# knights-lab/BURST

Hardware: AMD Instinct MI355X
Metric: aligned reads/sec (node), 100-bp synthetic reads @0.98 id vs RefSeq stand-in .edx/.acx (DB15), -m BEST; 1 GPU (higher is better)
Workload: dtype u32 bit-vectors (u8 edit distances)

## Files before the change

### burst_amd/capi.py

```python
import ctypes as C
import os

import numpy as np

_HERE = os.path.dirname(os.path.abspath(__file__))
LIB_PATH = os.path.join(os.environ.get("BURST_AMD_LIBDIR") or _HERE, "libburst_hip.so")

BHIP_OK, BHIP_E_ARG, BHIP_E_DEVICE, BHIP_E_CAPACITY, BHIP_E_QUERYLEN, BHIP_E_INTERNAL, BHIP_E_RESCORE = 0, -1, -2, -3, -4, -5, -6
BHIP_Q_PREFILTER, BHIP_Q_EXHAUSTIVE = 0, 1
BHIP_MAX_QLEN = 4095

HIT_DTYPE = np.dtype([("q", "<u4"), ("refIx", "<u4"), ("finalPos", "<u4"), ("score", "<f4"),
                      ("ed", "u1"), ("gapR", "u1"), ("gapQ", "u1"), ("rc", "u1")])
assert HIT_DTYPE.itemsize == 20


class BhipStats(C.Structure):
    _fields_ = [("n_queries", C.c_uint64), ("n_pairs", C.c_uint64), ("n_columns", C.c_uint64),
                ("n_raw_hits", C.c_uint64), ("n_hits", C.c_uint64), ("acx_entries_read", C.c_uint64),
                ("bytes_algorithmic", C.c_uint64), ("n_windows", C.c_uint64), ("n_window_columns", C.c_uint64),
                ("n_lane_tasks", C.c_uint64), ("n_task_columns", C.c_uint64), ("n_seed_words", C.c_uint64),
                ("ms_h2d", C.c_float), ("ms_prefilter", C.c_float), ("ms_peq", C.c_float), ("ms_myers", C.c_float),
                ("ms_rescore", C.c_float), ("ms_d2h", C.c_float), ("ms_total", C.c_float),
                ("ms_myers_prefix", C.c_float), ("ms_myers_window", C.c_float), ("ms_prefilter_hash", C.c_float), ("ms_seed", C.c_float),
                ("ms_stage_copy", C.c_float), ("ms_stage_route", C.c_float),
                ("myers_launches", C.c_uint32), ("prefix_words", C.c_uint32), ("prefilter_launches", C.c_uint32), ("prefilter_algo", C.c_uint32)]

    def as_dict(self):
        return {n: getattr(self, n) for n, _ in self._fields_}


class BhipQuerySpan(C.Structure):
    _fields_ = [("codes", C.c_void_p), ("codes4", C.c_void_p), ("off", C.c_void_p), ("emac", C.c_void_p), ("rc", C.c_void_p), ("flags", C.c_void_p),
                ("n", C.c_uint32), ("q_base", C.c_uint32), ("codes2", C.c_void_p), ("len", C.c_void_p)]


EXPORTS = ["bhip_init", "bhip_stage_queries", "bhip_align_staged", "bhip_align_batch", "bhip_align_pairs", "bhip_prefilter", "bhip_set_option", "bhip_get_stats",
           "bhip_device_info", "bhip_destroy", "bhip_last_error", "bhip_abi_version", "bhip_set_ref_order", "bhip_copy_hits_device", "bhip_sync_hits",
           "bhip_comm_create", "bhip_comm_unique_id", "bhip_comm_create_rank", "bhip_comm_allreduce_min", "bhip_comm_fetch_gathered", "bhip_comm_gather_hits", "bhip_comm_stage_device", "bhip_comm_gather_staged", "bhip_comm_stage_reset", "bhip_comm_destroy", "bhip_acx_export", "bhip_reserve", "bhip_reserve_symbols", "bhip_sort_queries", "bhip_stage_spans", "bhip_alloc_host", "bhip_free_host", "bhip_host_register", "bhip_host_unregister", "bhip_set_enqueued_hook", "bhip_acx_export_entries",
           "bhip_build_accelerator_shared", "bhip_comm_share", "bhip_team_create", "bhip_team_destroy", "bhip_team_share", "bhip_device_copy", "bhip_dna_marks",
           "bhip_cov_begin", "bhip_cov_add", "bhip_cov_sample_stats", "bhip_cov_dataset_stats", "bhip_cov_info", "bhip_cov_end", "bhip_lane_extents"]

COV_LINE_DTYPE = np.dtype([("ref", "<u4"), ("st", "<u4"), ("ed", "<u4"), ("w", "<u4")])
assert COV_LINE_DTYPE.itemsize == 16


class BurstHipError(RuntimeError):
    def __init__(self, code, msg):
        super().__init__("libburst_hip error %d: %s" % (code, msg))
        self.code = code


LOAD_LEGACY_PREFILTERS = False


def _load():
    if not os.path.exists(LIB_PATH):
        raise ImportError("%s is missing: the HIP extension has not been built (run __graft_entry__.build()); "
                          "burst_amd has no CPU fallback" % LIB_PATH)
    legacy = os.path.join(os.path.dirname(LIB_PATH), "libburst_hip_legacy.so")
    if LOAD_LEGACY_PREFILTERS and os.path.exists(legacy):
        globals()["_legacy_lib"] = C.CDLL(legacy, mode=C.RTLD_GLOBAL)
    lib = C.CDLL(LIB_PATH)
    vp, u32, u64, i32 = C.c_void_p, C.c_uint32, C.c_uint64, C.c_int
    lib.bhip_init.argtypes = [i32, vp, vp, u32, u32, vp, vp, i32, i32, vp, u32, vp, i32, C.POINTER(vp)]
    lib.bhip_init.restype = i32
    lib.bhip_dna_marks.argtypes = [i32, vp, u64, vp, vp, u64, u32, C.POINTER(u64), C.POINTER(u64), vp, vp]
    lib.bhip_dna_marks.restype = i32
    lib.bhip_align_batch.argtypes = [vp, vp, vp, vp, vp, vp, vp, u32, u32, i32, vp, u64, C.POINTER(u64)]
    lib.bhip_align_batch.restype = i32
    lib.bhip_stage_queries.argtypes = [vp, vp, vp, vp, vp, vp, vp, u32, u32]
    lib.bhip_stage_queries.restype = i32
    lib.bhip_align_staged.argtypes = [vp, i32, vp, u64, C.POINTER(u64)]
    lib.bhip_align_staged.restype = i32
    lib.bhip_align_pairs.argtypes = [vp, vp, vp, vp, u32, vp, vp, u64, vp]
    lib.bhip_align_pairs.restype = i32
    lib.bhip_prefilter.argtypes = [vp, vp, vp, vp, u32, vp, vp, vp, u64, C.POINTER(u64)]
    lib.bhip_prefilter.restype = i32
    lib.bhip_set_option.argtypes = [vp, C.c_char_p, C.c_longlong]
    lib.bhip_set_option.restype = i32
    lib.bhip_get_stats.argtypes = [vp, C.POINTER(BhipStats)]
    lib.bhip_get_stats.restype = i32
    lib.bhip_device_info.argtypes = [vp, C.c_char_p, i32, C.POINTER(i32), C.POINTER(u64)]
    lib.bhip_device_info.restype = i32
    lib.bhip_copy_hits_device.argtypes = [vp, vp, u64, C.POINTER(u64)]
    lib.bhip_copy_hits_device.restype = i32
    lib.bhip_sync_hits.argtypes = [vp]
    lib.bhip_sync_hits.restype = i32
    lib.bhip_destroy.argtypes = [vp]
    lib.bhip_destroy.restype = None
    lib.bhip_last_error.argtypes = []
    lib.bhip_last_error.restype = C.c_char_p
    lib.bhip_set_ref_order.argtypes = [vp, vp, u32]
    lib.bhip_set_ref_order.restype = i32
    lib.bhip_abi_version.argtypes = []
    lib.bhip_abi_version.restype = i32
    lib.bhip_stage_spans.argtypes = [vp, C.POINTER(BhipQuerySpan), u32, u32, u32]
    lib.bhip_reserve.argtypes = [vp, u32, u32]
    lib.bhip_reserve.restype = i32
    lib.bhip_stage_spans.restype = i32
    lib.bhip_reserve_symbols.argtypes = [vp, u32, u32, u64]
    lib.bhip_reserve_symbols.restype = i32
    lib.bhip_alloc_host.argtypes = [u64]
    lib.bhip_alloc_host.restype = vp
    lib.bhip_free_host.argtypes = [vp]
    lib.bhip_free_host.restype = None
    lib.bhip_host_register.argtypes = [vp, u64]
    lib.bhip_host_register.restype = i32
    lib.bhip_host_unregister.argtypes = [vp]
    lib.bhip_host_unregister.restype = i32
    lib.bhip_comm_unique_id.argtypes = [vp]
    lib.bhip_comm_unique_id.restype = i32
    lib.bhip_comm_create_rank.argtypes = [i32, i32, i32, vp, C.POINTER(vp)]
    lib.bhip_comm_create_rank.restype = i32
    lib.bhip_comm_destroy.argtypes = [vp]
    lib.bhip_comm_destroy.restype = None
    lib.bhip_acx_export.argtypes = [vp, vp, vp, vp, u64, C.POINTER(u64), vp, u32, C.POINTER(u32)]
    lib.bhip_acx_export.restype = i32
    lib.bhip_build_accelerator_shared.argtypes = [vp, i32, i32, i32, vp, vp]
    lib.bhip_build_accelerator_shared.restype = i32
    lib.bhip_team_create.argtypes = [i32, C.POINTER(vp)]
    lib.bhip_team_create.restype = i32
    lib.bhip_team_destroy.argtypes = [vp]
    lib.bhip_team_destroy.restype = None
    lib.bhip_device_copy.argtypes = [vp, vp, u64, i32]
    lib.bhip_device_copy.restype = i32
    lib.bhip_cov_begin.argtypes = [vp, u32, vp, u32]
    lib.bhip_cov_add.argtypes = [vp, u32, vp, u64]
    lib.bhip_cov_sample_stats.argtypes = [vp, u32, vp, vp]
    lib.bhip_cov_dataset_stats.argtypes = [vp, vp, vp]
    lib.bhip_cov_info.argtypes = [vp, vp]
    lib.bhip_cov_end.argtypes = [vp]
    lib.bhip_lane_extents.argtypes = [vp, vp]
    for f in (lib.bhip_cov_begin, lib.bhip_cov_add, lib.bhip_cov_sample_stats, lib.bhip_cov_dataset_stats, lib.bhip_cov_info, lib.bhip_cov_end, lib.bhip_lane_extents):
        f.restype = i32
    return lib


_lib = None


def _hits_mode(all_hits):
    return 2 if all_hits in (2, "best") else int(bool(all_hits))


def lib():
    global _lib
    if _lib is None:
        _lib = _load()
    return _lib


def _ptr(a):
    return None if a is None else a.ctypes.data_as(C.c_void_p)


def _chk(rc):
    if rc != BHIP_OK:
        raise BurstHipError(rc, lib().bhip_last_error().decode("utf-8", "replace"))


# ... 208 lines not shown
```

### burst_amd/csrc/bhip_align.hip

```cpp
#include "bhip_handle.h"
#include "bhip_pf_select.h"

__global__ void k_hit_count(const BhipHit *__restrict__ hits, uint32_t n, const uint32_t *__restrict__ n_dev, uint32_t *__restrict__ cnt, uint32_t *__restrict__ rank) {
	if (n_dev) n = *n_dev < n ? *n_dev : n;
	for (uint32_t i = blockIdx.x * blockDim.x + threadIdx.x; i < n; i += gridDim.x * blockDim.x) rank[i] = atomicAdd(&cnt[hits[i].q], 1u);
}
__global__ void k_hit_scatter(const BhipHit *__restrict__ in, uint32_t n, const uint32_t *__restrict__ n_dev, const uint32_t *__restrict__ off, const uint32_t *__restrict__ rank,
                              BhipHit *__restrict__ out, const uint32_t *__restrict__ qmap) {
	if (n_dev) n = *n_dev < n ? *n_dev : n;
	for (uint32_t i = blockIdx.x * blockDim.x + threadIdx.x; i < n; i += gridDim.x * blockDim.x) {
		BhipHit h = in[i];
		const uint32_t dst = off[h.q] + rank[i];
		if (qmap) h.q = qmap[h.q];
		out[dst] = h;
	}
}
__global__ void k_junk_adjust_raw(BhipRawHit *__restrict__ raw, const uint32_t *__restrict__ n_raw_dev, uint32_t raw_cap, const uint8_t *__restrict__ nx) {
	uint32_t n = *n_raw_dev;
	if (n > raw_cap) n = raw_cap;
	for (uint32_t i = blockIdx.x * blockDim.x + threadIdx.x; i < n; i += gridDim.x * blockDim.x) { const uint32_t x = nx[raw[i].q]; raw[i].ed += x; raw[i].m += x; }
}
__global__ void k_junk_adjust_best(uint32_t *__restrict__ best, const uint8_t *__restrict__ nx_six, uint32_t s0, uint32_t s1) {
	for (uint32_t s = s0 + blockIdx.x * blockDim.x + threadIdx.x; s < s1; s += gridDim.x * blockDim.x)
		if (nx_six[s] && best[s] != 0xFFFFFFFFu) best[s] += nx_six[s];
// ... 216 lines not shown
struct PfOverflow {
	uint32_t *fb1 = nullptr, *n_fb1 = nullptr;
	uint32_t *fb2 = nullptr, *n_fb2 = nullptr;
	int begin(Lane *L, Counters *dc, hipStream_t st, uint32_t n_list, bool lane_resolved) {
		int rc;
		if ((rc = L->fb_list.reserve(lane_resolved ? (size_t)n_list * 8 + 64 : (size_t)n_list * 4 + 16))) return rc;
		fb1 = L->fb_list.as<uint32_t>(); n_fb1 = &dc->n_fb;
		if (lane_resolved) {
			fb2 = fb1 + n_list + 8; n_fb2 = &dc->n_fb2;
			if (L->pf_launches || L->fb_dirty) HIPCHK(hipMemsetAsync(&dc->n_fb, 0, 8, st));
			L->fb_dirty = false;
		} else {
			HIPCHK(hipMemsetAsync(&dc->n_fb, 0, 4, st));
			L->fb_dirty = true;
		}
		return 0;
	}
};

static int launch_dense_fallback(Handle *h, Lane *L, hipStream_t st, const uint32_t *d_qlist, uint32_t n_list, const uint32_t *bad, uint32_t n_bad,
                                 uint2 *cand, uint32_t *candcnt, uint32_t *n_cand_dev, uint32_t cand_cap, Counters *dc, const uint32_t *fb, const uint32_t *n_fb) {
	const uint32_t *plan = h->cur->plan.as<uint32_t>();
	const bool narrow = h->cur->st_maxlen < 255u + (uint32_t)h->K;
	const size_t lds_w = ((size_t)(h->n_clumps + (narrow ? 3 : 1)) / (narrow ? 4 : 2)) * 4 + 1536u * 4 + 512u * 8 + 512u * 4 + 16;
	const uint32_t nw32 = (h->n_clumps + 1) / 2;
	if (lds_w <= 64 * 1024) {
		const uint32_t per_cu = (uint32_t)std::max<size_t>(1, std::min<size_t>(16, (160 * 1024) / lds_w));
		const uint32_t grid = std::min<uint32_t>(n_list, (uint32_t)h->n_cu * per_cu);
		if (narrow) hipLaunchKernelGGL(k_prefilter_wave<uint8_t>, dim3(grid), dim3(64), lds_w, st, h->s_codes(), h->s_off(),
			h->s_emac(), d_qlist, n_list, h->acx_view(), h->K, h->n_clumps, bad, n_bad, cand, candcnt,
			n_cand_dev, cand_cap, &dc->ent_read, plan, fb, n_fb);
		else hipLaunchKernelGGL(k_prefilter_wave<uint16_t>, dim3(grid), dim3(64), lds_w, st, h->s_codes(), h->s_off(),
			h->s_emac(), d_qlist, n_list, h->acx_view(), h->K, h->n_clumps, bad, n_bad, cand, candcnt,
			n_cand_dev, cand_cap, &dc->ent_read, plan, fb, n_fb);
	} else {
		int rc;
		const uint32_t grid = std::min<uint32_t>(n_list, (uint32_t)h->n_cu * 2);
		if ((rc = L->gcnt.reserve((size_t)grid * nw32 * 4))) return rc;
		hipLaunchKernelGGL(k_prefilter<false>, dim3(grid), dim3(256), 0, st, h->s_codes(), h->s_off(),
			h->s_emac(), d_qlist, n_list, h->acx_view(), h->K, h->n_clumps,
			L->gcnt.as<uint32_t>(), bad, n_bad, cand, candcnt, n_cand_dev, cand_cap, &dc->ent_read, fb, n_fb, plan);
	}
	HIPCHK(hipGetLastError());
	return 0;
}

static int launch_prefilter(Handle *h, Lane *L, hipStream_t st, const uint32_t *d_qlist, uint32_t n_list, uint2 *cand, uint32_t *candcnt, uint32_t cand_cap,
                            bool with_bad, uint32_t *n_cand_dev, Counters *dc) {
	const uint32_t *bad = with_bad ? h->bad.as<uint32_t>() : nullptr;
	const uint32_t n_bad = with_bad ? h->n_bad : 0;
	int rc;
	PfOverflow ov;
	if ((rc = ov.begin(L, dc, st, n_list, false))) return rc;
	{
		const uint32_t n_quads = (n_list + 3) / 4;
		const uint32_t grid = std::min<uint32_t>(n_quads, (uint32_t)h->n_cu * 6);
		hipLaunchKernelGGL(k_prefilter_hash, dim3(grid), dim3(64), 0, st, h->s_codes(), h->s_off(), h->s_emac(),
			d_qlist, n_list, h->acx_view(), h->K, bad, n_bad, cand, candcnt, n_cand_dev, cand_cap, &dc->ent_read,
			h->cur->plan.as<uint32_t>(), ov.fb1, ov.n_fb1);
		HIPCHK(hipGetLastError());
	}
	return launch_dense_fallback(h, L, st, d_qlist, n_list, bad, n_bad, cand, candcnt, n_cand_dev, cand_cap, dc, ov.fb1, ov.n_fb1);
}

static uint32_t seed_row_words(uint32_t maxwords) { return maxwords <= 8 ? 8u : std::max<uint32_t>(16u, (maxwords + 15u) & ~15u); }
static int class_prefix_words(const Handle *h, uint32_t maxE, int NW) {
	if (!h->opt_two_stage || NW > 32) return 0;
	const uint32_t want = (6 * maxE + 31) / 32;
	int NWP = want <= 1 ? 1 : (want <= 2 ? 2 : (want <= 3 ? 3 : (want <= 4 ? 4 : (want <= 6 ? 6 : 0))));
	if (NWP >= NW) NWP = 0;
	return NWP;
}
static int launch_peq(Handle *h, hipStream_t st, StageSlot *S, const uint32_t *d_qlist, uint32_t n_list, int NW, int NWP, DBuf &peq, DBuf &peqp, uint32_t blocks_per_cu = 16) {
	int rc;
	if ((rc = peq.reserve((size_t)n_list * 16 * NW * 4))) return rc;
	if ((rc = peqp.reserve((size_t)n_list * 16 * 6 * 4))) return rc;
	const bool junk = S->st_has_junk;
	const uint8_t *codes = junk ? S->qcodes_s.as<uint8_t>() : S->qcodes.as<uint8_t>();
	const uint64_t *off = junk ? S->qoff_s.as<uint64_t>() : S->qoff.as<uint64_t>();
	const uint32_t *pack = junk ? S->qpack_s.as<uint32_t>() : S->qpack.as<uint32_t>();
	{
		const uint32_t qb = 256u / (uint32_t)NW;
		const uint32_t grid = (uint32_t)std::min<uint64_t>(((uint64_t)n_list + qb - 1) / qb, (uint64_t)h->n_cu * blocks_per_cu);
		hipLaunchKernelGGL(k_build_peq, dim3(grid), dim3(256), 0, st, codes, off, d_qlist, n_list, NW, 0, h->mm, peq.as<uint32_t>(), pack, (S->st_maxlen + 7) / 8, h->peq_rows);
		HIPCHK(hipGetLastError());
	}
	if (NWP) {
		const uint32_t qb = 256u / (uint32_t)NWP;
		const uint32_t grid = (uint32_t)std::min<uint64_t>(((uint64_t)n_list + qb - 1) / qb, (uint64_t)h->n_cu * blocks_per_cu);
		hipLaunchKernelGGL(k_build_peq, dim3(grid), dim3(256), 0, st, codes, off, d_qlist, n_list, NWP, 32 * NWP, h->mm, peqp.as<uint32_t>(), pack, (S->st_maxlen + 7) / 8, h->peq_rows);
		HIPCHK(hipGetLastError());
	}
	return 0;
}
static uint32_t seed_min_need_for(const Handle *h, double mean_words, uint32_t W16) {
	return bhip_seed_min_need(h->opt_seed_min_need, h->opt_pf_cw, h->opt_pf_table, h->opt_pf_bytes, h->acx_wmean, mean_words, W16);
}
static int launch_seed(Handle *h, Lane *L, hipStream_t st, StageSlot *S, int cls, const uint32_t *d_qlist, uint32_t n_list, uint32_t maxwords, double mean_words, bool ahead = false) {
	int rc;
	const uint32_t W16 = seed_row_words(maxwords);
	L->seeded_ok[cls] = false;
	if ((rc = L->ranges_c[cls].reserve((size_t)n_list * W16 * 8 + 16))) return rc;
	if ((rc = L->hdr_c[cls].reserve((size_t)n_list * 8 + 16))) return rc;
	DBuf &qm = L->qmeta_c[S->seq & 1][cls];
	if ((rc = qm.reserve((size_t)n_list * 16 + 16))) return rc;
	L->qmeta_seq[S->seq & 1][cls] = 0;
	const uint64_t n_thr = (uint64_t)n_list * W16;
	hipEvent_t *ev = L->ev_seed[S->seq & 1][cls];
	const bool junk = S->st_has_junk;
	HIPCHK(hipEventRecord(ev[SPAN_START], st));
	const uint64_t full = (n_thr + 255) / 256;
	const uint32_t grid = (uint32_t)(ahead && h->opt_seed_ahead_blocks > 0 ? std::min<uint64_t>(full, (uint64_t)h->n_cu * (uint64_t)h->opt_seed_ahead_blocks) : full);
	hipLaunchKernelGGL(k_seed_ranges, dim3(grid), dim3(256), 0, st,
		junk ? S->qcodes_s.as<uint8_t>() : S->qcodes.as<uint8_t>(), junk ? S->qoff_s.as<uint64_t>() : S->qoff.as<uint64_t>(), d_qlist, n_list,
		h->acx_view(), h->K, S->plan.as<uint32_t>(), W16, L->ranges_c[cls].as<uint2>(), L->hdr_c[cls].as<uint2>(),
		junk ? S->qpack_s.as<uint32_t>() : S->qpack.as<uint32_t>(), (S->st_maxlen + 7) / 8, junk ? S->qemac_s.as<uint16_t>() : S->qemac.as<uint16_t>(), qm.as<uint4>(), S->st_has_six ? S->qsix.as<uint32_t>() : nullptr,
		seed_min_need_for(h, mean_words, W16), (uint32_t)h->opt_seed_drop_len, h->alt);
	HIPCHK(hipGetLastError());
	HIPCHK(hipEventRecord(ev[SPAN_DONE], st));
	L->qmeta_seq[S->seq & 1][cls] = S->seq + 1;
	L->seeded_ok[cls] = true; L->seeded_seq[cls] = S->seq; L->seeded_n[cls] = n_list; L->seeded_W16[cls] = W16;
	return 0;
}

static bhip_pf_kernel_t pf_kernel(const BhipPfChoice &c, int big) {
	if (c.legacy) return bhip_legacy_pf_kernel ? bhip_legacy_pf_kernel(c.kind, big ? 11 : c.htb, big ? 4 : c.rb, c.cw_mode, big) : nullptr;
	if (c.kind == BHIP_PF_CQ) return c.cw_mode == 0 ? (big ? k_prefilter_cq<0, 1> : k_prefilter_cq<0, 0>) : (big ? k_prefilter_cq<1, 1> : k_prefilter_cq<1, 0>);
	return big ? k_prefilter_cw<2, 1> : k_prefilter_cw<2, 0>;
}

static int launch_prefilter_mask(Handle *h, Lane *L, hipStream_t st, int cls, const uint32_t *d_qlist, uint32_t n_list, uint32_t maxwords, uint32_t *n_tasks_dev,
                                 uint32_t *n_cand_dev, Counters *dc, int algo, int prune) {
	int rc;
	PfOverflow ov;
	if ((rc = ov.begin(L, dc, st, n_list, true))) return rc;
	const uint32_t W16 = seed_row_words(maxwords);
	const double mean_words = n_list ? (double)L->seed_words[cls] / (double)n_list : (double)maxwords;
	if (!(L->seeded_ok[cls] && L->seeded_seq[cls] == h->cur->seq && L->seeded_n[cls] == n_list && L->seeded_W16[cls] == W16))
		if ((rc = launch_seed(h, L, st, h->cur, cls, d_qlist, n_list, maxwords, mean_words))) return rc;
	const BhipPfChoice c = bhip_pf_choose(algo, h->opt_pf_cw, h->opt_pf_table, h->opt_pf_rb, W16, mean_words * h->acx_wmean);
	const bool filter = c.kind != BHIP_PF_MASK, cw = c.kind == BHIP_PF_CW || c.kind == BHIP_PF_CQ;
	const bhip_pf_kernel_t fp = filter ? pf_kernel(c, 0) : nullptr, fp2 = filter && c.two_pass ? pf_kernel(c, 1) : nullptr;
	if (filter && (!fp || (c.two_pass && !fp2)))
		return fail(BHIP_E_ARG, "option prefilter_cw = %d selects a superseded prefilter kernel that is not part of libburst_hip.so (tests: libburst_hip_legacy.so is loaded first)", h->opt_pf_cw);
	hipFuncAttributes fa;
	const void *fn = filter ? (const void *)fp : c.htb == 9 ? (const void *)k_prefilter_mask<9> : c.htb == 10 ? (const void *)k_prefilter_mask<10> : (const void *)k_prefilter_mask<11>;
	const uint32_t fit = std::min<uint32_t>(cw ? 32u : 12u, blocks_per_cu(fn, 64u, 0, &fa));
	if (getenv("BHIP_DEBUG")) {
		if (cw) fprintf(stderr, "[bhip] prefilter kernel: %s, slot mode %d, %zu B LDS, %d VGPRs -> %u blocks per CU\n", c.kind == BHIP_PF_CQ ? "four queries per wave, streams by the whole wave" : "one query per wave", c.cw_mode, fa.sharedSizeBytes, fa.numRegs, fit);
		else fprintf(stderr, "[bhip] prefilter kernel: table 2^%d, %d record blocks in registers, %zu B LDS, %d VGPRs -> %u blocks per CU\n", c.htb, c.rb, fa.sharedSizeBytes, fa.numRegs, fit);
	}
	const uint32_t waves = h->opt_pf_waves ? std::min<uint32_t>((uint32_t)h->opt_pf_waves, fit) : fit;
	const uint32_t grid = std::min<uint32_t>(c.kind == BHIP_PF_CW ? n_list : (n_list + 3) / 4, (uint32_t)h->n_cu * waves);
	HIPCHK(hipEventRecord(L->ev_pf[cls][PF_HASH_START], st));
	const uint32_t *fb_dense = ov.fb1, *n_fb_dense = ov.n_fb1;
	if (filter) {
		auto launch = [&](bhip_pf_kernel_t k, uint32_t g, uint32_t *fb, uint32_t *n_fb, const uint32_t *sel, const uint32_t *n_sel) {
			hipLaunchKernelGGL(k, dim3(g), dim3(64), 0, st, L->ranges_c[cls].as<uint2>(), L->hdr_c[cls].as<uint2>(), W16, n_list,
				h->acx_view().rec, h->bad.as<uint32_t>(), h->n_bad,
				h->clump_len.as<uint32_t>(), h->tot_refs, L->tasks.as<uint2>(), n_tasks_dev, (uint32_t)L->task_cap, &dc->ent_read,
				fb, n_fb, &dc->unit_sum, &dc->col_sum, &dc->qlen_sum, &dc->surv_sum,
				L->tasks2.as<uint2>(), &dc->n_tasks2_cls[cls], prune, sel, n_sel, c.kind == BHIP_PF_CF ? h->opt_pf_bytes : 0);
		};
		launch(fp, grid, ov.fb1, ov.n_fb1, nullptr, nullptr);
		if (c.two_pass) {
			HIPCHK(hipGetLastError());
			const uint32_t g2 = (uint32_t)h->n_cu * (c.kind == BHIP_PF_CQ ? std::min<uint32_t>(4u, blocks_per_cu((const void *)fp2, 64u, 0)) : 1u);
			launch(fp2, g2, ov.fb2, ov.n_fb2, ov.fb1, ov.n_fb1);
			fb_dense = ov.fb2; n_fb_dense = ov.n_fb2;
		}
	} else {
		dispatch_int(HtbList{}, c.htb, [&](auto htb) {
			hipLaunchKernelGGL(k_prefilter_mask<decltype(htb)::value>, dim3(grid), dim3(64), 0, st, L->ranges_c[cls].as<uint2>(), L->hdr_c[cls].as<uint2>(), W16, n_list,
				h->acx_view().rec, h->bad.as<uint32_t>(), h->n_bad,
				h->clump_len.as<uint32_t>(), h->tot_refs, L->tasks.as<uint2>(), n_tasks_dev, (uint32_t)L->task_cap, &dc->ent_read,
				ov.fb1, ov.n_fb1, &dc->unit_sum, &dc->col_sum, &dc->qlen_sum, L->cand.as<uint2>(), n_cand_dev, (uint32_t)L->cand_cap);
		});
	}
	HIPCHK(hipGetLastError());
	HIPCHK(hipEventRecord(L->ev_pf[cls][PF_HASH_DONE], st));
	++L->pf_launches;
	L->pf_algo_used = c.kind;
	return launch_dense_fallback(h, L, st, d_qlist, n_list, h->bad.as<uint32_t>(), h->n_bad, L->cand.as<uint2>(), nullptr, n_cand_dev, (uint32_t)L->cand_cap, dc, fb_dense, n_fb_dense);
}

static int lane_reserve_work(Lane *L) {
	int rc;
	if ((rc = L->cand.reserve(L->cand_cap * sizeof(uint2))) || (rc = L->raw.reserve(L->raw_cap * sizeof(BhipRawHit))) || (rc = L->wide.reserve(L->raw_cap * sizeof(uint32_t))) ||
	    (rc = L->rs_lists.reserve(L->raw_cap * sizeof(uint32_t) * 10)) || (rc = L->scratch.reserve(L->scratch_cap * sizeof(uint32_t))) || (rc = L->wins.reserve(L->win_cap * sizeof(BhipWin))) ||
	    (rc = L->tasks.reserve(L->task_cap * sizeof(uint2))) || (rc = L->tasks2.reserve(L->task_cap * sizeof(uint2))) || (rc = L->tasks2k.reserve(L->task_cap * sizeof(uint2))) ||
	    (rc = L->wins2.reserve(L->win_cap * sizeof(BhipWin)))) return rc;
	return 0;
}
extern "C" int bhip_reserve(void *handle, uint32_t n_entries, uint32_t max_len) { return bhip_reserve_symbols(handle, n_entries, max_len, 0); }
extern "C" int bhip_reserve_symbols(void *handle, uint32_t n_entries, uint32_t max_len, uint64_t total_symbols) {
	Handle *h = (Handle *)handle;
	if (!h) return fail(BHIP_E_ARG, "null handle");
	if (!n_entries) return BHIP_OK;
	if (!max_len || max_len > BHIP_MAX_QLEN) max_len = BHIP_MAX_QLEN;
	HIPCHK(hipSetDevice(h->device));
	int rc;
	if (getenv("BHIP_DEBUG")) { size_t f_ = 0, t_ = 0; if (hipMemGetInfo(&f_, &t_) == hipSuccess) fprintf(stderr, "[bhip] reserve for %u entries of up to %u symbols: %.2f GB of the device's %.2f free\n", n_entries, max_len, f_ / 1e9, t_ / 1e9); }
	const size_t n = n_entries, nb = total_symbols ? (size_t)std::min<uint64_t>(total_symbols + 64, (uint64_t)n * max_len) : n * max_len, qw = (max_len + 7) / 8;
	const size_t cw = (size_t)class_words(class_of_len(max_len), max_len);
	const size_t peq_words = total_symbols ? std::min<size_t>(n * cw, 2 * (nb / 32 + n)) : n * cw;
	for (StageSlot &S : h->slots) {
		if ((rc = slot_init(&S))) return rc;
		if ((rc = S.qcodes4.reserve(nb / 2 + 128)) || (rc = S.qcodes.reserve(nb + 128)) || (rc = S.qoff.reserve((n + 1) * 8)) || (rc = S.qemac.reserve((n + 1) * 2)) ||
		    (rc = S.qsix.reserve((n + 1) * 4)) || (rc = S.qrc.reserve(n + 1)) || (rc = S.qflags.reserve(n + 1)) || (rc = S.qmap.reserve((n + 1) * 4)) ||
		    (rc = S.off_raw.reserve((n + 8) * 8)) || (rc = S.plan.reserve(n * 4 + 16)) || (rc = S.qpack.reserve(n * qw * 4 + 64)) || (rc = S.key.reserve(n + 16)) ||
		    (rc = S.key_sorted.reserve(n + 16)) || (rc = S.idx.reserve(n * 4 + 16)) || (rc = S.idx_sorted.reserve(n * 4 + 16))) return rc;
		size_t tb = 0;
		HIPCHK(hipcub::DeviceRadixSort::SortPairs(nullptr, tb, S.key.as<uint8_t>(), S.key_sorted.as<uint8_t>(), S.idx.as<uint32_t>(), S.idx_sorted.as<uint32_t>(), (int)n, 0, 8, h->stage_stream));
		if ((rc = S.sort_tmp.reserve(tb + 16))) return rc;
	}
	if (getenv("BHIP_DEBUG")) { size_t f_ = 0, t_ = 0; if (hipMemGetInfo(&f_, &t_) == hipSuccess) fprintf(stderr, "[bhip] ... staging slots reserved: %.2f GB free\n", f_ / 1e9); }
	if ((rc = ensure_lanes(h, 1))) return rc;
	Lane *L = h->lanes[0];
	lane_capacity_floor(h, L, n);
	const int cls = class_of_len(max_len);
	if ((rc = lane_reserve_work(L)) || (rc = L->peq.reserve(peq_words * 16 * 4)) || (rc = L->peqp.reserve(n * 16 * 6 * 4)) ||
	    (rc = L->peq_alt.reserve(peq_words * 16 * 4)) || (rc = L->peqp_alt.reserve(n * 16 * 6 * 4)) ||
	    (rc = L->fb_list.reserve(n * 8 + 64)) || (rc = L->ranges_c[cls].reserve(n * 16 * 8 + 16)) || (rc = L->hdr_c[cls].reserve(n * 8 + 16))) return rc;
	if (h->n_order) { if ((rc = h->best_key.reserve((n + 1) * 8)) || (rc = h->sort_idx.reserve(std::max<size_t>((size_t)h->out_cap, n + 1) * 4))) return rc; if (!h->nsel_pinned) HIPCHK(hipHostMalloc((void **)&h->nsel_pinned, 64, hipHostMallocDefault)); }
	if ((rc = h->best.reserve((n + 1) * 4)) || (rc = h->out.reserve(h->out_cap * sizeof(BhipHit))) || (rc = h->shared_ctr.reserve(sizeof(SharedCtr))) ||
	    (rc = h->sort_idx.reserve(h->out_cap * 4)) || (rc = h->sort_keys.reserve((n + 1) * 4)) || (rc = h->sort_keys2.reserve((n + 1) * 4)) ||
	    (rc = h->out_sorted.reserve(h->out_cap * sizeof(BhipHit))) || (rc = h->out_sorted2.reserve(h->out_cap * sizeof(BhipHit)))) return rc;
	{
		size_t tb = 0;
		HIPCHK(hipcub::DeviceScan::ExclusiveSum(nullptr, tb, h->sort_keys.as<uint32_t>(), h->sort_keys2.as<uint32_t>(), (int)(n + 1), h->stream));
		if ((rc = h->sort_tmp.reserve(tb))) return rc;
	}
	if (getenv("BHIP_DEBUG")) { size_t f_ = 0, t_ = 0; if (hipMemGetInfo(&f_, &t_) == hipSuccess) fprintf(stderr, "[bhip] ... lane and record buffers reserved: %.2f GB free\n", f_ / 1e9); }
	if (!h->copy_stream) { HIPCHK(hipStreamCreateWithFlags(&h->copy_stream, hipStreamNonBlocking)); HIPCHK(hipEventCreateWithFlags(&h->ev_sorted, hipEventDisableTiming));
		for (auto &e : h->ev_copied) HIPCHK(hipEventCreateWithFlags(&e, hipEventDisableTiming)); }
	{
		const uint32_t nw = std::min<uint32_t>(n_entries, 1u << 17), len = std::min<uint32_t>(max_len, 100u);
		const size_t nb_w = (size_t)nw * len + 16;
		uint8_t *pin = nullptr;
		const size_t bytes = nb_w + nb_w / 2 + 16 + ((size_t)nw + 1) * 8 + (size_t)nw * 2 + 64 + (size_t)nw * 4 * sizeof(BhipHit);
		HIPCHK(hipHostMalloc((void **)&pin, bytes, hipHostMallocPortable));
		uint8_t *codes = pin, *codes4 = pin + nb_w;
		uint64_t *off = (uint64_t *)(pin + ((nb_w + nb_w / 2 + 16 + 7) & ~(size_t)7));
		uint16_t *emac = (uint16_t *)(off + nw + 1);
		BhipHit *hbuf = (BhipHit *)(((uintptr_t)(emac + nw) + 63) & ~(uintptr_t)63);
		uint64_t x = 88172645463325252ull;
		for (size_t i = 0; i < nb_w; ++i) { x ^= x << 13; x ^= x >> 7; x ^= x << 17; codes[i] = (uint8_t)(1 + (x & 3)); }
		for (size_t i = 0; i < nb_w / 2; ++i) codes4[i] = (uint8_t)(codes[2 * i] | codes[2 * i + 1] << 4);
		for (uint32_t i = 0; i <= nw; ++i) off[i] = (uint64_t)i * len;
		for (uint32_t i = 0; i < nw; ++i) emac[i] = (uint16_t)(len / 40);
		BhipQuerySpan sp;
		memset(&sp, 0, sizeof sp);
		sp.codes = codes; sp.codes4 = codes4; sp.off = off; sp.emac = emac; sp.n = nw;
		uint64_t n_out = 0;
		const int async = h->opt_async_d2h;
		h->opt_async_d2h = 1;
		for (StageSlot &S : h->slots) { S.state = 0; S.st_valid = false; }
		rc = 0;
		for (int rep = 0; rep < 4 && !rc; ++rep) {
			rc = bhip_stage_spans(h, &sp, 1, nw, len);
			if (!rc) rc = bhip_align_staged(h, 0, hbuf, (uint64_t)nw * 4, &n_out);
		}
		(void)bhip_sync_hits(h);
		{
			const size_t big = std::min<size_t>(64u << 20, std::min(h->out_sorted.cap, h->out_sorted2.cap));
			void *tmp = nullptr;
			if (big && hipHostMalloc(&tmp, 2 * big, hipHostMallocPortable) == hipSuccess) {
				(void)hipMemcpyAsync(tmp, h->out_sorted.p, big, hipMemcpyDeviceToHost, h->copy_stream);
				(void)hipMemcpyAsync((char *)tmp + big, h->out_sorted2.p, big, hipMemcpyDeviceToHost, h->copy_stream);
				(void)hipMemcpyAsync(tmp, h->out_sorted.p, big, hipMemcpyDeviceToHost, h->copy_stream);
				(void)hipStreamSynchronize(h->copy_stream);
				(void)hipMemcpyAsync(h->out_sorted.p, tmp, big, hipMemcpyHostToDevice, h->stage_stream);
				(void)hipMemcpyAsync(h->out_sorted2.p, (char *)tmp + big, big, hipMemcpyHostToDevice, h->stage_stream);
				(void)hipMemcpyAsync(h->out_sorted.p, tmp, big, hipMemcpyHostToDevice, h->stage_stream);
				(void)hipStreamSynchronize(h->stage_stream);
				const size_t piece = big / 16;
				if (piece) {
					for (int i = 0; i < 12; ++i) (void)hipMemcpyAsync((char *)h->out_sorted.p + (size_t)i * piece, (char *)tmp + (size_t)i * piece, piece, hipMemcpyHostToDevice, h->stage_stream);
					(void)hipMemcpyAsync((char *)tmp + big, h->out_sorted2.p, big, hipMemcpyDeviceToHost, h->copy_stream);
					(void)hipStreamSynchronize(h->copy_stream);
					(void)hipStreamSynchronize(h->stage_stream);
				}
				(void)hipHostFree(tmp);
			}
			(void)hipGetLastError();
		}
// ... 17 lines not shown
	SharedCtr hsc = {};
	uint32_t n_deliver = 0;
	bool sorted_ahead = false; int o_ahead = 0;
	size_t tmp_bytes = 0;
	std::chrono::steady_clock::time_point t0; double t_host[4] = {0, 0, 0, 0};
	void mark(int i) { t_host[i] = std::chrono::duration<double, std::milli>(std::chrono::steady_clock::now() - t0).count(); }
};

static int enqueue_class(Handle *h, Lane *L, int cls, int all_hits) {
	int rc;
	hipStream_t pf = h->pf_stream, sw = h->sweep_stream, po = h->post_stream;
	Counters *dc = L->counters.as<Counters>();
	const uint32_t n_pf = L->npf[cls], n_ex = L->nex[cls], n_list = n_pf + n_ex;
	const uint32_t grid_my = (uint32_t)h->n_cu * (uint32_t)h->opt_sweep_blocks;
	const uint32_t grid_task = (uint32_t)h->n_cu * 4u * (uint32_t)h->opt_sweep_blocks * (uint32_t)h->opt_oversub;
	const int NW = class_words(cls, L->maxlen);
	const uint32_t *qlist = L->qlist[cls];
	hipEvent_t *ce = L->ev_cls[cls];
	if (L->launches) { HIPCHK(hipStreamWaitEvent(pf, L->ev_rs[RS_START], 0)); HIPCHK(hipStreamWaitEvent(sw, L->ev_rs[RS_START], 0)); }
	const int NWP = class_prefix_words(h, L->maxE[cls], NW);
	HIPCHK(hipEventRecord(ce[CE_START], sw));
	L->peq_ahead[cls] = false;
	if (L->alt_ok && L->alt_seq == h->cur->seq && L->alt_cls == cls && L->alt_n == n_list && L->alt_nwp == NWP && !L->launches) {
		std::swap(L->peq, L->peq_alt); std::swap(L->peqp, L->peqp_alt);
		std::swap(L->ev_peq_cur[SPAN_START], L->ev_peq_alt[SPAN_START]); std::swap(L->ev_peq_cur[SPAN_DONE], L->ev_peq_alt[SPAN_DONE]);
		L->alt_ok = false; L->peq_ahead[cls] = true;
	} else if ((rc = launch_peq(h, sw, h->cur, qlist, n_list, NW, NWP, L->peq, L->peqp))) return rc;
	L->prefix_words = (uint32_t)NWP;
	HIPCHK(hipEventRecord(ce[CE_PEQ_DONE], sw));
	HIPCHK(hipEventRecord(ce[CE_PF_START], pf));
	const bool masked = NWP && n_pf && h->has_masks && h->opt_lane_masks;
	const int pf_algo = bhip_pf_algo(h->opt_pf_algo, L->pf_algo);
	const int prune = masked && !all_hits && h->opt_prune && n_list < (1u << 24) && pf_algo == 0;
	if (n_pf) {
		if (masked) { if ((rc = launch_prefilter_mask(h, L, pf, cls, qlist, n_pf, L->maxwords[cls], &dc->n_tasks_cls[cls], &dc->n_cand_cls[cls], dc, pf_algo, prune))) return rc; }
		else if ((rc = launch_prefilter(h, L, pf, qlist, n_pf, L->cand.as<uint2>(), nullptr, (uint32_t)L->cand_cap, true, &dc->n_cand_cls[cls], dc))) return rc;
	}
	const uint4 *qmeta_cls = (masked && L->qmeta_seq[h->cur->seq & 1][cls] == h->cur->seq + 1) ? L->qmeta_c[h->cur->seq & 1][cls].as<uint4>() : nullptr;
	L->masked = masked;
	L->pf_masked[cls] = masked && n_pf;
	HIPCHK(hipEventRecord(ce[CE_PF_DONE], pf));
	HIPCHK(hipStreamWaitEvent(sw, ce[CE_PF_DONE], 0));
	HIPCHK(hipEventRecord(ce[CE_SWEEP_START], sw));
	if (n_pf) {
		if (masked) launch_prefix_task(h, L, sw, NWP, grid_task, L->tasks.as<uint2>(), &dc->n_tasks_cls[cls], qlist, L->wins.as<BhipWin>(), &dc->n_wins_cls[cls], dc, qmeta_cls);
		if (NWP) launch_prefix(h, L, sw, NWP, masked ? std::min<uint32_t>(grid_my, (uint32_t)h->n_cu) : grid_my, L->cand.as<uint2>(), &dc->n_cand_cls[cls], L->cand_cap, 0, qlist, &dc->n_wins_cls[cls], dc);
		else launch_myers(h, L, sw, NW, grid_my, L->cand.as<uint2>(), &dc->n_cand_cls[cls], L->cand_cap, 0, qlist, L->raw.as<BhipRawHit>(),
			&dc->n_raw, (uint32_t)L->raw_cap, h->best.as<uint32_t>(), nullptr, dc);
		HIPCHK(hipGetLastError());
		++L->launches;
	}
	HIPCHK(hipEventRecord(ce[CE_SWEEP_PF_DONE], sw));
	if (n_ex) {
		const uint64_t np = (uint64_t)n_ex * h->n_clumps;
		const uint32_t g = (uint32_t)std::min<uint64_t>((np + 15) / 16, grid_my);
		if (NWP) launch_prefix(h, L, sw, NWP, g, nullptr, nullptr, np, n_pf, qlist, &dc->n_wins_cls[cls], dc);
		else launch_myers(h, L, sw, NW, g, nullptr, nullptr, np, n_pf, qlist, L->raw.as<BhipRawHit>(), &dc->n_raw, (uint32_t)L->raw_cap,
			h->best.as<uint32_t>(), nullptr, dc);
		HIPCHK(hipGetLastError());
		++L->launches;
		L->n_pairs_ex += np;
	}
	HIPCHK(hipEventRecord(ce[CE_SWEEP_EX_DONE], sw));
	HIPCHK(hipStreamWaitEvent(po, ce[CE_SWEEP_EX_DONE], 0));
	if (NWP) { launch_window(h, L, po, cls, NWP, grid_my, L->wins.as<BhipWin>(), &dc->n_wins_cls[cls], dc); HIPCHK(hipGetLastError()); }
	L->pruned[cls] = masked && prune && n_pf;
	if (L->pruned[cls]) {
		HIPCHK(hipEventRecord(L->ev_ph[cls][PH_WIN_DONE], po));
		HIPCHK(hipStreamWaitEvent(sw, L->ev_ph[cls][PH_WIN_DONE], 0));
		hipLaunchKernelGGL(k_task_filter, dim3((uint32_t)h->n_cu * 8), dim3(256), 0, sw, L->tasks2.as<uint2>(), &dc->n_tasks2_cls[cls], (uint32_t)L->task_cap, qlist,
			six_or_null(h), h->best.as<uint32_t>(), L->tasks2k.as<uint2>(), &dc->n_tasks2k_cls[cls]);
		launch_prefix_task(h, L, sw, NWP, grid_task, L->tasks2k.as<uint2>(), &dc->n_tasks2k_cls[cls], qlist, L->wins2.as<BhipWin>(), &dc->n_wins2_cls[cls], dc, qmeta_cls);
		HIPCHK(hipGetLastError());
		HIPCHK(hipEventRecord(L->ev_ph[cls][PH_SWEEP2_DONE], sw));
		HIPCHK(hipStreamWaitEvent(po, L->ev_ph[cls][PH_SWEEP2_DONE], 0));
		launch_window(h, L, po, cls, NWP, grid_my, L->wins2.as<BhipWin>(), &dc->n_wins2_cls[cls], dc);
		HIPCHK(hipGetLastError());
	}
	HIPCHK(hipEventRecord(ce[CE_WIN_DONE], po));
	HIPCHK(hipEventRecord(L->ev_rs[RS_START], po));
	return 0;
}

static int enqueue_rescore(Handle *h, Lane *L, const BatchCall &b) {
	hipStream_t po = h->post_stream;
	Counters *dc = L->counters.as<Counters>();
	SharedCtr *sc = h->shared_ctr.as<SharedCtr>();
	const RefArgs R = ref_args(h);
	HIPCHK(hipEventRecord(L->ev_rs[RS_START], po));
	if (h->cur->st_has_junk) {
		const uint32_t nl_ = h->cur->st_lanes, nsh_ = h->cur->st_nshared;
		uint32_t li_ = 0;
		for (uint32_t l = 0; l < nl_; ++l) if (h->lanes[l] == L) li_ = l;
		const uint32_t s0 = (uint32_t)(((uint64_t)li_ * nsh_ + nl_ - 1) / nl_), s1 = (uint32_t)(((uint64_t)(li_ + 1) * nsh_ + nl_ - 1) / nl_);
		hipLaunchKernelGGL(k_junk_adjust_raw, dim3((uint32_t)h->n_cu * 4), dim3(256), 0, po, L->raw.as<BhipRawHit>(), &dc->n_raw, (uint32_t)L->raw_cap, h->cur->nx.as<uint8_t>());
		if (s1 > s0) hipLaunchKernelGGL(k_junk_adjust_best, dim3(std::min<uint32_t>((s1 - s0 + 255) / 256, (uint32_t)h->n_cu * 4)), dim3(256), 0, po, h->best.as<uint32_t>(), h->cur->nx_six.as<uint8_t>(), s0, s1);
		HIPCHK(hipGetLastError());
	}
	const uint32_t qw_g = (h->cur->st_maxlen + 7) / 8;
	hipLaunchKernelGGL(k_rescore_classify, dim3((uint32_t)h->n_cu * 8), dim3(256), 0, po, L->raw.as<BhipRawHit>(), &dc->n_raw, (uint32_t)L->raw_cap,
		h->best.as<uint32_t>(), b.all_hits, h->cur->qoff.as<uint64_t>(), six_or_null(h), rc_or_null(h),
		R.len, h->out.as<BhipHit>(), &sc->n_out, (uint32_t)h->out_cap, L->rs_lists.as<uint32_t>(), dc->n_rs, L->wide.as<uint32_t>(), &dc->n_wide,
		b.band_rows, h->opt_rescore_reg);
	HIPCHK(hipGetLastError());
	if (h->opt_rescore_reg) {
		for_each_int(SetList{}, [&](auto set) {
			constexpr int SET = decltype(set)::value;
			const uint32_t grid = (uint32_t)h->n_cu * std::min<uint32_t>(32u, blocks_per_cu((const void *)k_rescore_reg<SET>, 64, 0)) * (uint32_t)h->opt_oversub;
			hipLaunchKernelGGL(k_rescore_reg<SET>, dim3(grid), dim3(64), 0, po, L->raw.as<BhipRawHit>(), L->rs_lists.as<uint32_t>(), dc->n_rs, (uint32_t)L->raw_cap,
				h->cur->qoff.as<uint64_t>(), rc_or_null(h), h->cur->qpack.as<uint32_t>(), qw_g,
				R.bytes(), R.off, R.len, h->lut.as<uint8_t>(), h->out.as<BhipHit>(), &sc->n_out, (uint32_t)h->out_cap, &sc->err);
		});
		HIPCHK(hipGetLastError());
	}
	const uint32_t grid_rs = (uint32_t)h->n_cu * (h->opt_rescore_reg ? 4 : 16);
	const size_t lds_rs = (size_t)(b.band_rows + 1 + b.qw + b.rw) * 256;
	hipLaunchKernelGGL(k_rescore<false>, dim3(grid_rs), dim3(64), lds_rs, po, L->raw.as<BhipRawHit>(), &dc->n_raw, (uint32_t)L->raw_cap,
		L->rs_lists.as<uint32_t>() + (size_t)9 * L->raw_cap, &dc->n_rs[9], h->best.as<uint32_t>(), b.all_hits, h->cur->qcodes.as<uint8_t>(), h->cur->qoff.as<uint64_t>(),
		six_or_null(h), rc_or_null(h), R.bytes(), R.off, R.len, h->lut.as<uint8_t>(), h->out.as<BhipHit>(), &sc->n_out, (uint32_t)h->out_cap, L->wide.as<uint32_t>(),
		&dc->n_wide, (uint32_t *)nullptr, &dc->scratch_used, 0ull, &sc->err, b.qw ? h->cur->qpack.as<uint32_t>() : nullptr, b.band_rows, b.qw, b.rw);
	HIPCHK(hipGetLastError());
	HIPCHK(hipEventRecord(L->ev_rs[RS_DONE], po));
	HIPCHK(hipMemcpyAsync(L->hc_pinned, dc, sizeof(Counters), hipMemcpyDeviceToHost, po));
	return 0;
}

static int enqueue_lane(Handle *h, Lane *L, const BatchCall &b) {
	int rc;
	if ((rc = lane_reserve_work(L))) return rc;
	HIPCHK(hipMemsetAsync(L->counters.p, 0, sizeof(Counters), h->pf_stream));
	L->launches = 0; L->prefix_words = 0; L->n_pairs_ex = 0; L->pf_launches = 0; L->fb_dirty = false;
	for (int c = 0; c < kNumClasses; ++c) { L->pf_masked[c] = false; L->pruned[c] = false; }
	for (int cls = 0; cls < kNumClasses; ++cls) if (L->npf[cls] + L->nex[cls]) if ((rc = enqueue_class(h, L, cls, b.all_hits))) return rc;
	return enqueue_rescore(h, L, b);
}

static void seed_next_batch(Handle *h, StageSlot *cur, hipEvent_t cur_done) {
	if (!h->opt_seed_ahead || !h->has_acx || !h->has_masks || !h->opt_lane_masks || h->opt_host_routing) return;
	StageSlot *N = nullptr;
	for (StageSlot &S : h->slots) if (&S != cur && S.state == 1 && (!N || S.seq < N->seq)) N = &S;
	if (!N || !N->st_nq) return;
	if (!N->resolved) {
		for (;;) {
			const hipError_t e = hipEventQuery(N->ev_done);
			if (e == hipSuccess) break;
			if (e != hipErrorNotReady) { (void)hipGetLastError(); return; }
			if (hipEventQuery(cur_done) != hipErrorNotReady) { (void)hipGetLastError(); return; }
			std::this_thread::yield();
		}
		(void)hipGetLastError();
		const BhipStageInfo &I = *N->info_pinned;
		if (I.err || I.junk) return;
		if (resolve_slot(h, N)) return;
	}
	if (N->st_has_junk || ensure_lanes(h, N->st_lanes)) return;
	for (uint32_t l = 0; l < N->st_lanes && l < h->lanes.size(); ++l) {
		Lane *L = h->lanes[l];
		for (int cls = 0; cls < kNumClasses; ++cls) {
			const uint32_t n_pf = N->npf[l][cls];
			if (!n_pf || !class_prefix_words(h, N->maxE[l][cls], class_words(cls, N->maxlen_lane[l]))) continue;
			if (L->seeded_ok[cls] && L->seeded_seq[cls] == N->seq) continue;
			if (launch_seed(h, L, h->pf_stream, N, cls, N->idx_sorted.as<uint32_t>() + N->qlist_off[l][cls], n_pf, N->maxwords[l][cls], (double)N->seed_words[l][cls] / (double)n_pf, true)) { (void)hipGetLastError(); return; }
		}
		int only = -1, n_cls = 0;
		for (int cls = 0; cls < kNumClasses; ++cls) if (N->npf[l][cls] + N->nex[l][cls]) { only = cls; ++n_cls; }
		if (n_cls == 1 && !(L->alt_ok && L->alt_seq == N->seq)) {
			const uint32_t n_list = N->npf[l][only] + N->nex[l][only];
			const int NW = class_words(only, N->maxlen_lane[l]), NWP = class_prefix_words(h, N->maxE[l][only], NW);
			L->alt_ok = false;
			if (hipEventRecord(L->ev_peq_alt[SPAN_START], h->pf_stream) != hipSuccess ||
			    launch_peq(h, h->pf_stream, N, N->idx_sorted.as<uint32_t>() + N->qlist_off[l][only], n_list, NW, NWP, L->peq_alt, L->peqp_alt, (uint32_t)h->opt_peq_ahead_blocks) ||
			    hipEventRecord(L->ev_peq_alt[SPAN_DONE], h->pf_stream) != hipSuccess) { (void)hipGetLastError(); return; }
			L->alt_ok = true; L->alt_seq = N->seq; L->alt_cls = only; L->alt_nwp = NWP; L->alt_n = n_list;
		}
	}
}

extern "C" int bhip_set_enqueued_hook(void *handle, void (*fn)(void *), void *ctx) {
	Handle *h = (Handle *)handle;
	if (!h) return fail(BHIP_E_ARG, "null handle");
	h->enqueued_hook = fn; h->enqueued_ctx = ctx;
	return BHIP_OK;
}

static bool grow_cap(uint64_t &cap, uint64_t seen, bool eighth, int lane, const char *what) {
	if (seen <= cap) return false;
	const uint64_t to = seen + (eighth ? seen / 8 : 0) + 1024;
	if (getenv("BHIP_DEBUG")) {
		if (lane >= 0) fprintf(stderr, "[bhip] redo: lane %d %s %llu -> %llu\n", lane, what, (unsigned long long)cap, (unsigned long long)to);
		else fprintf(stderr, "[bhip] redo: %s %llu -> %llu\n", what, (unsigned long long)cap, (unsigned long long)to);
	}
	cap = to;
	return true;
}

static int pick_batch(Handle *h, BatchCall &b) {
	StageSlot *slot = nullptr;
	for (StageSlot &S : h->slots) if (S.state == 1 && (!slot || S.seq < slot->seq)) slot = &S;
	if (!slot) for (StageSlot &S : h->slots) if (S.state == 2 && (!slot || S.seq > slot->seq)) slot = &S;
	if (!slot) return fail(BHIP_E_ARG, "no staged queries (call bhip_stage_queries first)");
	{ int rcs = resolve_slot(h, slot); if (rcs) { slot->state = 0; return rcs; } }
	apply_slot(h, slot);
	b.slot = slot; b.n_q = h->cur->st_nq; b.n_shared = h->cur->st_nshared; b.nl = h->cur->st_lanes;
	return BHIP_OK;
}
static int plan_batch(Handle *h, BatchCall &b) {
	b.band_rows = std::min<uint32_t>(BHIP_RESCORE_WMAX, 2 * h->cur->st_maxE + 1 + 9);
	b.qw = (h->cur->st_maxlen + 7) / 8; b.rw = (h->cur->st_maxlen + b.band_rows + 24) / 8 + 2;
	if ((size_t)(b.band_rows + 1 + b.qw + b.rw) * 256 > 40 * 1024) { b.qw = 0; b.rw = 0; }
	if (!b.sel_best) return BHIP_OK;
	int rc;
	if ((rc = h->best_key.reserve((size_t)(b.n_q + 1) * 8)) || (rc = h->sort_idx.reserve(std::max<size_t>((size_t)h->out_cap, (size_t)b.n_q + 1) * 4))) return rc;
	if (!h->nsel_pinned) HIPCHK(hipHostMalloc((void **)&h->nsel_pinned, 64, hipHostMallocDefault));
	return BHIP_OK;
}
static bool records_resident(const Handle *h, const BatchCall &b) { return h->res_valid && h->res_seq == b.slot->seq && h->res_all_hits == b.mode; }
static void take_resident(Handle *h, BatchCall &b) {
	b.hsc.n_out = h->res_n_raw; b.hsc.err = 0; h->stats = h->res_stats; b.n_deliver = h->res_n; *b.n_hits = b.n_deliver; b.sorted_ahead = false;
}

static int plan_scan(Handle *h, BatchCall &b, hipStream_t st) {
	b.tmp_bytes = 0;
	HIPCHK(hipcub::DeviceScan::ExclusiveSum(nullptr, b.tmp_bytes, h->sort_keys.as<uint32_t>(), h->sort_keys2.as<uint32_t>(), (int)(b.n_q + 1), st));
	return h->sort_tmp.reserve(b.tmp_bytes);
}
static int enqueue_grouping(Handle *h, const BatchCall &b, hipStream_t st, uint32_t n_host, const uint32_t *n_dev, DBuf &sorted) {
	uint32_t *cnt = h->sort_keys.as<uint32_t>(), *off = h->sort_keys2.as<uint32_t>(), *rank = h->sort_idx.as<uint32_t>();
	const uint32_t n_q = b.n_q, g = (uint32_t)h->n_cu * 8;
	const uint32_t *qmap = h->cur->has_qmap ? h->cur->qmap.as<uint32_t>() : (const uint32_t *)nullptr;
	size_t tmp_bytes = b.tmp_bytes;
	if (b.sel_best) {
		hipLaunchKernelGGL(k_best_key, dim3(g), dim3(256), 0, st, h->out.as<BhipHit>(), n_host, n_dev, h->ref_order.as<uint32_t>(), cnt, h->best_key.as<unsigned long long>());
		hipLaunchKernelGGL(k_best_flag, dim3(std::min<uint32_t>((n_q + 256) / 256, g)), dim3(256), 0, st, cnt, n_q, rank);
		HIPCHK(hipcub::DeviceScan::ExclusiveSum(h->sort_tmp.p, tmp_bytes, rank, off, (int)(n_q + 1), st));
		hipLaunchKernelGGL(k_best_emit, dim3(g), dim3(256), 0, st, h->out.as<BhipHit>(), n_host, n_dev, h->ref_order.as<uint32_t>(), cnt, h->best_key.as<unsigned long long>(), off, sorted.as<BhipHit>(), qmap);
		HIPCHK(hipGetLastError());
		HIPCHK(hipMemcpyAsync(h->nsel_pinned, off + n_q, 4, hipMemcpyDeviceToHost, st));
		return 0;
	}
	HIPCHK(hipcub::DeviceScan::ExclusiveSum(h->sort_tmp.p, tmp_bytes, cnt, off, (int)(n_q + 1), st));
	hipLaunchKernelGGL(k_hit_scatter, dim3(g), dim3(256), 0, st, h->out.as<BhipHit>(), n_host, n_dev, off, rank, sorted.as<BhipHit>(), qmap);
	hipLaunchKernelGGL(k_hit_fix, dim3(std::min<uint32_t>((n_q + 255) / 256, (uint32_t)h->n_cu * 8)), dim3(256), 0, st, sorted.as<BhipHit>(), off, cnt, n_q, h->sort_scratch.as<BhipHit>(), (uint32_t)(h->sort_scratch.cap / sizeof(BhipHit)));
	HIPCHK(hipGetLastError());
	return 0;
}
static int enqueue_grouping_ahead(Handle *h, BatchCall &b) {
	int rc;
	b.o_ahead = (h->opt_async_d2h && b.hits) ? (h->out_idx ^ 1) : 0;
	DBuf &sorted = b.o_ahead ? h->out_sorted2 : h->out_sorted;
	if ((rc = h->sort_idx.reserve((size_t)h->out_cap * 4)) || (rc = h->sort_keys.reserve((size_t)(b.n_q + 1) * 4)) || (rc = h->sort_keys2.reserve((size_t)(b.n_q + 1) * 4)) ||
	    (rc = sorted.reserve((size_t)h->out_cap * sizeof(BhipHit))) || (rc = h->sort_scratch.reserve((size_t)h->out_cap * sizeof(BhipHit)))) return rc;
	if ((rc = plan_scan(h, b, h->post_stream))) return rc;
	if (h->copy_pending[b.o_ahead]) HIPCHK(hipStreamWaitEvent(h->post_stream, h->ev_copied[b.o_ahead], 0));
	HIPCHK(hipEventRecord(h->ev[EV_GROUP_START], h->post_stream));
	if ((rc = enqueue_grouping(h, b, h->post_stream, (uint32_t)h->out_cap, &h->shared_ctr.as<SharedCtr>()->n_out, sorted))) return rc;
	HIPCHK(hipEventRecord(h->ev[EV_GROUP_DONE], h->post_stream));
	b.sorted_ahead = true;
	return BHIP_OK;
}

static int enqueue_chain(Handle *h, BatchCall &b, int attempt) {
	int rc;
	const uint32_t n_q = b.n_q;
	b.sorted_ahead = false;
	if ((rc = h->best.reserve((size_t)(b.n_shared + 1) * 4)) || (rc = h->out.reserve(h->out_cap * sizeof(BhipHit))) || (rc = h->shared_ctr.reserve(sizeof(SharedCtr)))) return rc;
	HIPCHK(hipEventRecord(h->ev[EV_BEGIN], h->stream));
	HIPCHK(hipMemsetAsync(h->best.p, 0xFF, (size_t)b.n_shared * 4, h->stream));
	HIPCHK(hipMemsetAsync(h->shared_ctr.p, 0, 2 * sizeof(uint32_t), h->stream));
	if ((rc = h->sort_idx.reserve((size_t)h->out_cap * 4)) || (rc = h->sort_keys.reserve((size_t)(n_q + 1) * 4))) return rc;
	HIPCHK(hipMemsetAsync(h->sort_keys.p, 0, (size_t)(n_q + 1) * 4, h->stream));
	if (b.sel_best) HIPCHK(hipMemsetAsync(h->best_key.p, 0xFF, (size_t)(n_q + 1) * 8, h->stream));
	hipLaunchKernelGGL(k_set_rank_ptrs, dim3(1), dim3(1), 0, h->stream, h->shared_ctr.as<SharedCtr>(), h->sort_keys.as<uint32_t>(), h->sort_idx.as<uint32_t>());
	HIPCHK(hipEventRecord(h->ev[EV_RESET_DONE], h->stream));
	HIPCHK(hipStreamWaitEvent(h->sweep_stream, h->ev[EV_RESET_DONE], 0));
	HIPCHK(hipStreamWaitEvent(h->post_stream, h->ev[EV_RESET_DONE], 0));
	for (uint32_t l = 0; l < b.nl; ++l) if (h->lanes[l]->n_entries) if ((rc = enqueue_lane(h, h->lanes[l], b))) return rc;
	HIPCHK(hipEventRecord(h->ev[EV_PF_DONE], h->pf_stream));
	if ((rc = enqueue_grouping_ahead(h, b))) return rc;
	if (!h->hsc_pinned) HIPCHK(hipHostMalloc((void **)&h->hsc_pinned, sizeof(SharedCtr), hipHostMallocDefault));
	HIPCHK(hipMemcpyAsync(h->hsc_pinned, h->shared_ctr.p, 2 * sizeof(uint32_t), hipMemcpyDeviceToHost, h->post_stream));
	HIPCHK(hipEventRecord(h->ev[EV_CHAIN_DONE], h->post_stream));
	seed_next_batch(h, b.slot, h->ev[EV_CHAIN_DONE]);
	if (h->enqueued_hook && attempt == 0) h->enqueued_hook(h->enqueued_ctx);
	return BHIP_OK;
}
static int wait_chain(Handle *h, const BatchCall &b) {
	HIPCHK(hipEventSynchronize(h->ev[EV_PF_DONE]));
	HIPCHK(hipStreamSynchronize(h->sweep_stream));
	HIPCHK(hipStreamSynchronize(h->post_stream));
	for (uint32_t l = 0; l < b.nl; ++l) if (h->lanes[l]->n_entries) h->lanes[l]->hc = *h->lanes[l]->hc_pinned;
	return BHIP_OK;
// ... 214 lines not shown
	}
	return deliver(h, b);
}

extern "C" int bhip_align_batch(void *handle, const uint8_t *q_codes, const uint64_t *q_off, const uint16_t *q_emac,
                                const uint32_t *q_six, const uint8_t *q_rc, const uint8_t *q_flags,
                                uint32_t n_q, uint32_t n_shared, int all_hits,
                                BhipHit *hits, uint64_t cap, uint64_t *n_hits) {
	if (!n_hits) return fail(BHIP_E_ARG, "null argument");
	*n_hits = 0;
	int rc = bhip_stage_queries(handle, q_codes, q_off, q_emac, q_six, q_rc, q_flags, n_q, n_shared);
	if (rc) return rc;
	return bhip_align_staged(handle, all_hits, hits, cap, n_hits);
}

extern "C" int bhip_align_pairs(void *handle, const uint8_t *q_codes, const uint64_t *q_off, const uint16_t *q_emac,
                                uint32_t n_q, const uint32_t *pair_q, const uint32_t *pair_clump, uint64_t n_pairs, uint8_t *mins) {
	Handle *h = (Handle *)handle;
	if (!h || !q_codes || !q_off || !q_emac || !pair_q || !pair_clump || !mins) return fail(BHIP_E_ARG, "null argument");
	memset(&h->stats, 0, sizeof h->stats);
	for (StageSlot &S : h->slots) { S.state = 0; S.st_valid = false; }
	h->cur = &h->slots[0];
	if (!n_pairs || !n_q) return BHIP_OK;
	HIPCHK(hipSetDevice(h->device));
	int rc;
	if ((rc = ensure_lanes(h, 1))) return rc;
	Lane *L = h->lanes[0];
	uint32_t maxlen = 0;
	for (uint32_t i = 0; i < n_q; ++i) maxlen = std::max<uint32_t>(maxlen, (uint32_t)(q_off[i + 1] - q_off[i]));
	if (maxlen > BHIP_MAX_QLEN) return fail(BHIP_E_QUERYLEN, "query longer than %d", BHIP_MAX_QLEN);
	const int cls = class_of_len(std::max<uint32_t>(maxlen, 1)), NW = class_words(cls, maxlen);
	std::vector<uint2> pr(n_pairs);
	for (uint64_t p = 0; p < n_pairs; ++p) {
		if (pair_q[p] >= n_q || pair_clump[p] >= h->n_clumps) return fail(BHIP_E_ARG, "pair %llu out of range", (unsigned long long)p);
		pr[p] = make_uint2(pair_q[p], pair_clump[p]);
	}
	h->cur->st_has_six = false; h->cur->st_has_rc = false;
	if ((rc = upload_queries(h, q_codes, q_off, q_emac, nullptr, nullptr, n_q))) return rc;
	if ((rc = L->peq.reserve((size_t)n_q * 16 * NW * 4))) return rc;
	if ((rc = h->pairs.reserve(n_pairs * sizeof(uint2)))) return rc;
	if ((rc = h->mins.reserve(n_pairs * 16))) return rc;
	hipStream_t st = h->stream;
	HIPCHK(hipMemcpyAsync(h->pairs.p, pr.data(), n_pairs * sizeof(uint2), hipMemcpyHostToDevice, st));
	HIPCHK(hipMemsetAsync(L->counters.p, 0, sizeof(Counters), st));
	Counters *dc = L->counters.as<Counters>();
	const uint32_t qb = 256u / (uint32_t)NW;
	hipLaunchKernelGGL(k_build_peq, dim3((uint32_t)std::min<uint64_t>(((uint64_t)n_q + qb - 1) / qb, (uint64_t)h->n_cu * 16)), dim3(256), 0, st,
		h->cur->qcodes.as<uint8_t>(), h->cur->qoff.as<uint64_t>(), (const uint32_t *)nullptr, n_q, NW, 0, h->mm, L->peq.as<uint32_t>(), (const uint32_t *)nullptr, 0u, h->peq_rows);
	HIPCHK(hipGetLastError());
	HIPCHK(hipEventRecord(h->ev[EV_BEGIN], st));
	launch_myers(h, L, st, NW, (uint32_t)std::min<uint64_t>((n_pairs + 15) / 16, (uint64_t)h->n_cu * 8), h->pairs.as<uint2>(), nullptr, n_pairs, 0, nullptr,
		nullptr, nullptr, 0, nullptr, h->mins.as<uint8_t>(), dc);
	HIPCHK(hipGetLastError());
	HIPCHK(hipEventRecord(h->ev[EV_KERNEL_DONE], st));
	HIPCHK(hipMemcpyAsync(mins, h->mins.p, n_pairs * 16, hipMemcpyDeviceToHost, st));
	Counters hc;
	HIPCHK(hipMemcpyAsync(&hc, dc, sizeof hc, hipMemcpyDeviceToHost, st));
	HIPCHK(hipStreamSynchronize(st));
	h->stats.n_queries = n_q; h->stats.n_pairs = n_pairs; h->stats.n_columns = hc.col_sum; h->stats.myers_launches = 1;
	h->stats.bytes_algorithmic = 8ull * hc.col_sum + hc.qlen_sum / 2 + 192ull * n_pairs;
	h->stats.ms_myers = ev_ms(h->ev[EV_BEGIN], h->ev[EV_KERNEL_DONE]); h->stats.ms_total = h->stats.ms_myers;
	return BHIP_OK;
}

extern "C" int bhip_prefilter(void *handle, const uint8_t *q_codes, const uint64_t *q_off, const uint16_t *q_emac, uint32_t n_q,
                              uint32_t *out_q, uint32_t *out_clump, uint32_t *out_count, uint64_t cap, uint64_t *n_out) {
	Handle *h = (Handle *)handle;
	if (!h || !q_codes || !q_off || !q_emac || !n_out) return fail(BHIP_E_ARG, "null argument");
	if (!h->has_acx) return fail(BHIP_E_ARG, "handle has no accelerator");
	*n_out = 0;
	for (StageSlot &S : h->slots) { S.state = 0; S.st_valid = false; }
	h->cur = &h->slots[0];
	if (!n_q) return BHIP_OK;
	HIPCHK(hipSetDevice(h->device));
	int rc;
	if ((rc = ensure_lanes(h, 1))) return rc;
	Lane *L = h->lanes[0];
	for (int attempt = 0; attempt < 4; ++attempt) {
		if ((rc = upload_queries(h, q_codes, q_off, q_emac, nullptr, nullptr, n_q))) return rc;
		{
			std::vector<uint32_t> plan(n_q, 1u);
			for (uint32_t i = 0; i < n_q; ++i) plan[i] = make_seed_plan(q_codes + q_off[i], (uint32_t)(q_off[i + 1] - q_off[i]), q_emac[i], (uint32_t)h->K, h->opt_prefilter_stride, h->alt);
			if ((rc = upload_plan(h, n_q, plan))) return rc;
			const uint32_t qw_g = (h->cur->st_maxlen + 7) / 8;
			if ((rc = h->cur->qpack.reserve((size_t)n_q * qw_g * 4 + 16))) return rc;
			const uint64_t total = (uint64_t)n_q * qw_g;
			if (total) hipLaunchKernelGGL(k_pack_queries, dim3((uint32_t)std::min<uint64_t>((total + 255) / 256, (uint64_t)h->n_cu * 16)), dim3(256), 0, h->stream,
				h->cur->qcodes.as<uint8_t>(), h->cur->qoff.as<uint64_t>(), n_q, qw_g, h->cur->qpack.as<uint32_t>());
			HIPCHK(hipGetLastError());
		}
		if ((rc = L->cand.reserve(L->cand_cap * sizeof(uint2)))) return rc;
		if ((rc = L->candcnt.reserve(L->cand_cap * sizeof(uint32_t)))) return rc;
		HIPCHK(hipStreamSynchronize(h->stream));
		HIPCHK(hipMemsetAsync(L->counters.p, 0, sizeof(Counters), L->stream));
		Counters *dc = L->counters.as<Counters>();
		HIPCHK(hipEventRecord(h->ev[EV_BEGIN], L->stream));
		if ((rc = launch_prefilter(h, L, L->stream, nullptr, n_q, L->cand.as<uint2>(), L->candcnt.as<uint32_t>(), (uint32_t)L->cand_cap, false, &dc->n_cand, dc))) return rc;
		HIPCHK(hipEventRecord(h->ev[EV_KERNEL_DONE], L->stream));
		Counters hc;
		HIPCHK(hipMemcpyAsync(&hc, dc, sizeof hc, hipMemcpyDeviceToHost, L->stream));
		HIPCHK(hipStreamSynchronize(L->stream));
		if (hc.n_cand > L->cand_cap) { L->cand_cap = (uint64_t)hc.n_cand + 1024; continue; }
		*n_out = hc.n_cand;
		memset(&h->stats, 0, sizeof h->stats);
		h->stats.n_queries = n_q; h->stats.n_pairs = hc.n_cand; h->stats.acx_entries_read = hc.ent_read; h->stats.ms_prefilter = ev_ms(h->ev[EV_BEGIN], h->ev[EV_KERNEL_DONE]);
		if (hc.n_cand > cap) return fail(BHIP_E_CAPACITY, "candidate buffer holds %llu, %u needed", (unsigned long long)cap, hc.n_cand);
		std::vector<uint2> c(hc.n_cand); std::vector<uint32_t> cc(hc.n_cand);
		if (hc.n_cand) {
			HIPCHK(hipMemcpy(c.data(), L->cand.p, hc.n_cand * sizeof(uint2), hipMemcpyDeviceToHost));
			HIPCHK(hipMemcpy(cc.data(), L->candcnt.p, hc.n_cand * sizeof(uint32_t), hipMemcpyDeviceToHost));
		}
		std::vector<uint32_t> ord(hc.n_cand);
		for (uint32_t i = 0; i < hc.n_cand; ++i) ord[i] = i;
		std::sort(ord.begin(), ord.end(), [&](uint32_t a, uint32_t b) { return c[a].x != c[b].x ? c[a].x < c[b].x : c[a].y < c[b].y; });
		for (uint32_t i = 0; i < hc.n_cand; ++i) {
			if (out_q) out_q[i] = c[ord[i]].x;
			if (out_clump) out_clump[i] = c[ord[i]].y;
			if (out_count) out_count[i] = cc[ord[i]];
		}
		return BHIP_OK;
	}
	return fail(BHIP_E_INTERNAL, "candidate buffer kept overflowing");
}

extern "C" int bhip_copy_hits_device(void *handle, void *dst_device, uint64_t cap_records, uint64_t *n_records) {
	Handle *h = (Handle *)handle;
	if (!h || !n_records) return fail(BHIP_E_ARG, "null argument");
	*n_records = h->last_n_out;
	if (!h->last_n_out) return BHIP_OK;
	if (!dst_device && cap_records) return fail(BHIP_E_ARG, "null destination");
	if (h->last_n_out > cap_records) return fail(BHIP_E_CAPACITY, "device buffer holds %llu records, %llu needed", (unsigned long long)cap_records, (unsigned long long)h->last_n_out);
	HIPCHK(hipSetDevice(h->device));
	HIPCHK(hipMemcpyAsync(dst_device, (h->last_out ? h->out_sorted2 : h->out_sorted).p, (size_t)h->last_n_out * sizeof(BhipHit), hipMemcpyDeviceToDevice, h->stream));
	HIPCHK(hipStreamSynchronize(h->stream));
	return BHIP_OK;
}

extern "C" int bhip_sync_hits(void *handle) {
	Handle *h = (Handle *)handle;
	if (!h) return fail(BHIP_E_ARG, "null handle");
	HIPCHK(hipSetDevice(h->device));
	for (int o = 0; o < 2; ++o) if (h->copy_pending[o]) { HIPCHK(hipEventSynchronize(h->ev_copied[o])); h->copy_pending[o] = false; }
	return BHIP_OK;
}
```

### burst_amd/csrc/bhip_handle.h

```cpp
#ifndef BHIP_HANDLE_H
#define BHIP_HANDLE_H
#include <hip/hip_runtime.h>
#include <hipcub/hipcub.hpp>
#include <string>
#include <stdint.h>
#include <stdio.h>
#include <stdarg.h>
#include <stdlib.h>
#include <string.h>
#include <algorithm>
#include <vector>
#include <mutex>
#include <atomic>
#include <chrono>
#include <thread>
#include "burst_hip.h"
#include "bhip_internal.h"

__global__ void k_acx_offsets(const uint32_t *, uint64_t, int, uint32_t *, unsigned long long *);
__global__ void k_acx_lines(const uint32_t *, uint64_t, int, unsigned long long *, uint4 *);
__global__ void k_acx_decode(const uint8_t *, const unsigned long long *, const uint32_t *, BhipAcxView, uint64_t, int, uint32_t, uint32_t *, uint32_t *);
__global__ void k_transpose_refs(const uint8_t *, const uint64_t *, const uint32_t *, const uint64_t *, uint32_t, uint4 *);
__global__ void k_build_peq(const uint8_t *, const uint64_t *, const uint32_t *, uint32_t, int, int, BhipMatchMask, uint32_t *, const uint32_t *, uint32_t, uint32_t);
template <bool LDS_CNT> __global__ void k_prefilter(const uint8_t *, const uint64_t *, const uint16_t *, const uint32_t *, uint32_t,
	BhipAcxView, int, uint32_t, uint32_t *, const uint32_t *, uint32_t, uint2 *, uint32_t *, uint32_t *, uint32_t,
	unsigned long long *, const uint32_t *, const uint32_t *, const uint32_t *);
__global__ void k_prefilter_hash(const uint8_t *, const uint64_t *, const uint16_t *, const uint32_t *, uint32_t, BhipAcxView, int,
	const uint32_t *, uint32_t, uint2 *, uint32_t *, uint32_t *, uint32_t, unsigned long long *, const uint32_t *, uint32_t *, uint32_t *);
template <typename CNT> __global__ void k_prefilter_wave(const uint8_t *, const uint64_t *, const uint16_t *, const uint32_t *, uint32_t,
	BhipAcxView, int, uint32_t, const uint32_t *, uint32_t, uint2 *, uint32_t *, uint32_t *, uint32_t, unsigned long long *, const uint32_t *,
	const uint32_t *, const uint32_t *);
template <int NW> __global__ void k_myers(const uint2 *, const uint32_t *, uint64_t, uint32_t, uint32_t, const uint32_t *, const uint32_t *,
	const uint64_t *, const uint16_t *, const uint32_t *, const uint4 *, const uint64_t *, const uint32_t *, uint32_t,
	BhipRawHit *, uint32_t *, uint32_t, uint32_t *, uint8_t *, unsigned long long *, unsigned long long *);
__global__ void k_myers_long(const uint2 *, const uint32_t *, uint64_t, uint32_t, uint32_t, const uint32_t *, const uint32_t *,
	const uint64_t *, const uint16_t *, const uint32_t *, const uint4 *, const uint64_t *, const uint32_t *, uint32_t,
	BhipRawHit *, uint32_t *, uint32_t, uint32_t *, uint8_t *, unsigned long long *, unsigned long long *, uint32_t);
template <int NWP> __global__ void k_myers_prefix(const uint2 *, const uint32_t *, uint64_t, uint32_t, uint32_t, const uint32_t *, const uint32_t *,
	const uint64_t *, const uint16_t *, const uint4 *, const uint64_t *, const uint32_t *, uint32_t, BhipWin *, uint32_t *, uint32_t,
	unsigned long long *, unsigned long long *, uint32_t *, const uint32_t *);
template <int NW> __global__ void k_myers_window(const BhipWin *, const uint32_t *, uint32_t, int, int, const uint32_t *, const uint32_t *,
	const uint4 *, BhipRawHit *, uint32_t *, uint32_t, uint32_t *, unsigned long long *, const uint32_t *);
template <int BW> __global__ void k_myers_window_band(const BhipWin *, const uint32_t *, uint32_t, int, int, const uint32_t *, const uint32_t *,
	const uint4 *, BhipRawHit *, uint32_t *, uint32_t, uint32_t *, unsigned long long *, const uint32_t *);
__global__ void k_extract_kmers(const uint4 *, const uint64_t *, const uint32_t *, const uint64_t *, uint32_t, uint32_t, int, unsigned long long *, uint16_t *, uint32_t *);
__global__ void k_attach_masks(BhipAcxView, uint64_t, const unsigned long long *, const uint16_t *, uint32_t, const uint32_t *, uint32_t *, uint32_t, uint32_t);
template <int HTB> __global__ void k_prefilter_mask(const uint2 *, const uint2 *, uint32_t, uint32_t, const uint32_t *, const uint32_t *, uint32_t, const uint32_t *, uint32_t,
	uint2 *, uint32_t *, uint32_t, unsigned long long *, uint32_t *, uint32_t *, unsigned long long *, unsigned long long *, unsigned long long *,
	uint2 *, uint32_t *, uint32_t);
template <int MODE, int BIG> __global__ void k_prefilter_cq(const uint2 *, const uint2 *, uint32_t, uint32_t, const uint32_t *, const uint32_t *, uint32_t, const uint32_t *, uint32_t,
	uint2 *, uint32_t *, uint32_t, unsigned long long *, uint32_t *, uint32_t *, unsigned long long *, unsigned long long *, unsigned long long *, unsigned long long *,
	uint2 *, uint32_t *, int, const uint32_t *, const uint32_t *, int);
template <int MODE, int BIG> __global__ void k_prefilter_cw(const uint2 *, const uint2 *, uint32_t, uint32_t, const uint32_t *, const uint32_t *, uint32_t, const uint32_t *, uint32_t,
	uint2 *, uint32_t *, uint32_t, unsigned long long *, uint32_t *, uint32_t *, unsigned long long *, unsigned long long *, unsigned long long *, unsigned long long *,
	uint2 *, uint32_t *, int, const uint32_t *, const uint32_t *, int);
__global__ void k_task_filter(const uint2 *, const uint32_t *, uint32_t, const uint32_t *, const uint32_t *, const uint32_t *, uint2 *, uint32_t *);
__global__ void k_seed_ranges(const uint8_t *, const uint64_t *, const uint32_t *, uint32_t, BhipAcxView, int, const uint32_t *, uint32_t, uint2 *, uint2 *, const uint32_t *, uint32_t, const uint16_t *, uint4 *, const uint32_t *, uint32_t, uint32_t, BhipAlt);
template <int NWP> __global__ void k_myers_prefix_task(const uint2 *, const uint32_t *, uint32_t, const uint32_t *, const uint32_t *, const uint64_t *,
	const uint16_t *, const uint4 *, const uint64_t *, const uint32_t *, BhipWin *, uint32_t *, uint32_t, unsigned long long *, uint32_t *, const uint4 *, const uint32_t *);
template <bool WIDE> __global__ void k_rescore(const BhipRawHit *, const uint32_t *, uint32_t, const uint32_t *, const uint32_t *,
	const uint32_t *, int, const uint8_t *, const uint64_t *, const uint32_t *, const uint8_t *, const uint8_t *, const uint64_t *,
	const uint32_t *, const uint8_t *, BhipHit *, uint32_t *, uint32_t, uint32_t *, uint32_t *, uint32_t *, unsigned long long *,
	unsigned long long, uint32_t *, const uint32_t *, uint32_t, uint32_t, uint32_t);
__global__ void k_pack_queries(const uint8_t *, const uint64_t *, uint32_t, uint32_t, uint32_t *);
__global__ void k_unpack4(const uint8_t *, uint64_t, uint64_t, uint8_t *);
__global__ void k_unpack2(const uint8_t *, uint64_t, uint64_t, uint8_t *);
__global__ void k_span_fill(const uint64_t *, uint32_t, uint32_t, uint64_t, uint32_t, uint64_t *, uint32_t *, uint32_t *);
__global__ void k_route(const uint64_t *, const uint32_t *, uint32_t, const uint16_t *, const uint32_t *, const uint8_t *, uint32_t, uint32_t, uint32_t, int, int, int,
	uint32_t *, uint8_t *, uint32_t *, BhipStageInfo *, BhipAlt);
__global__ void k_rescore_classify(const BhipRawHit *, const uint32_t *, uint32_t, const uint32_t *, int, const uint64_t *, const uint32_t *, const uint8_t *,
	const uint32_t *, BhipHit *, uint32_t *, uint32_t, uint32_t *, uint32_t *, uint32_t *, uint32_t *, uint32_t, int);
template <int SET> __global__ void k_rescore_reg(const BhipRawHit *, const uint32_t *, const uint32_t *, uint32_t, const uint64_t *, const uint8_t *, const uint32_t *, uint32_t,
	const uint8_t *, const uint64_t *, const uint32_t *, const uint8_t *, BhipHit *, uint32_t *, uint32_t, uint32_t *);
int bhip_fail_msg(int code, const char *fmt, ...) __attribute__((format(printf, 2, 3)));
#define fail(...) bhip_fail_msg(__VA_ARGS__)
inline bool bhip_trace_sync() { static const bool on = getenv("BHIP_TRACE_SYNC") != nullptr; return on; }
#define HIPCHK(x) do { hipError_t e_ = (x); if (e_ != hipSuccess) \
	return fail(BHIP_E_DEVICE, "%s:%d %s: %s", __FILE__, __LINE__, #x, hipGetErrorString(e_)); \
	if (bhip_trace_sync()) { fprintf(stderr, "[bhip sync] %s:%d\n", __FILE__, __LINE__); (void)hipDeviceSynchronize(); } } while (0)

inline std::mutex &bhip_vmm_mutex() { static std::mutex m; return m; }
inline std::atomic<int> &bhip_vmm_peer_access() { static std::atomic<int> f(0); return f; }
struct DBuf {
	void *p = nullptr; size_t cap = 0;
	bool vmm = false; size_t va_size = 0; int vmm_device = 0;
	std::vector<hipMemGenericAllocationHandle_t> chunks;
	size_t n_mapped = 0;
	static constexpr size_t kChunk = 1ull << 30;
	static hipError_t malloc_patiently(void **q, size_t want) {
		hipError_t e = hipMalloc(q, want);
		if (e != hipErrorOutOfMemory) return e;
		(void)hipGetLastError();
		size_t last_free = 0, total = 0;
		(void)hipMemGetInfo(&last_free, &total);
		const bool dbg = getenv("BHIP_DEBUG") != nullptr;
		if (dbg) fprintf(stderr, "[bhip] hipMalloc(%zu) found no memory with %.2f GB reported free: waiting for memory that is on its way back\n", want, last_free / 1e9);
		for (int tries = 0; tries < 80; ++tries) {
			std::this_thread::sleep_for(std::chrono::milliseconds(100));
			e = hipMalloc(q, want);
			if (e != hipErrorOutOfMemory) { if (dbg) fprintf(stderr, "[bhip] ... there after %d ms\n", 100 * (tries + 1)); return e; }
			(void)hipGetLastError();
			if (dbg && tries % 10 == 9) { size_t f = 0; (void)hipMemGetInfo(&f, &total); fprintf(stderr, "[bhip] ... %d ms: %.2f GB reported free\n", 100 * (tries + 1), f / 1e9); }
		}
		return e;
	}
	static void poison(void *q, size_t n) {
		static const char *ev = getenv("BHIP_POISON");
		if (ev && q) { (void)hipMemset(q, atoi(ev) & 255, n); (void)hipDeviceSynchronize(); if (getenv("BHIP_DEBUG")) fprintf(stderr, "[bhip] buffer %p .. %p (%zu bytes)\n", q, (void *)((char *)q + n), n); }
	}
	int reserve(size_t bytes) {
		if (bytes <= cap) return 0;
		release();
		size_t want = bytes + bytes / 4 + 256;
		hipError_t e = malloc_patiently(&p, want);
		if (e != hipSuccess) { p = nullptr; return fail(BHIP_E_DEVICE, "hipMalloc(%zu): %s", want, hipGetErrorString(e)); }
		poison(p, want);
		cap = want; return 0;
	}
	int reserve_exact(size_t bytes) {
		if (bytes <= cap) return 0;
		release();
		hipError_t e = malloc_patiently(&p, bytes);
		if (e != hipSuccess) { p = nullptr; return fail(BHIP_E_DEVICE, "hipMalloc(%zu): %s", bytes, hipGetErrorString(e)); }
		poison(p, bytes);
		cap = bytes; return 0;
	}
	int reserve_growable(size_t max_bytes, int device) {
		release();
		std::lock_guard<std::mutex> lk(bhip_vmm_mutex());
		int ok = 0;
		if (hipDeviceGetAttribute(&ok, hipDeviceAttributeVirtualMemoryManagementSupported, device) != hipSuccess || !ok) { (void)hipGetLastError(); return 1; }
		const size_t sz = ((max_bytes + kChunk - 1) / kChunk + 1) * kChunk;
		if (hipMemAddressReserve(&p, sz, kChunk, nullptr, 0) != hipSuccess) { (void)hipGetLastError(); p = nullptr; return 1; }
		vmm = true; va_size = sz; vmm_device = device; cap = 0; n_mapped = 0;
		chunks.assign(sz / kChunk, nullptr);
		peers.clear();
		int n_dev = 0;
		if (bhip_vmm_peer_access().load() && hipGetDeviceCount(&n_dev) == hipSuccess) for (int d = 0; d < n_dev; ++d) { int can = 0; if (d != device && hipDeviceCanAccessPeer(&can, d, device) == hipSuccess && can) peers.push_back(d); }
		(void)hipGetLastError();
		return 0;
	}
	std::vector<int> peers;
	int map_chunks(size_t c0, size_t c1) {
		if (!vmm) return fail(BHIP_E_INTERNAL, "map_chunks on a fixed buffer");
		if (c1 > chunks.size()) return fail(BHIP_E_DEVICE, "record area: chunk %zu wanted, %zu reserved", c1, chunks.size());
		hipMemAllocationProp prop = {};
		prop.type = hipMemAllocationTypePinned; prop.location.type = hipMemLocationTypeDevice; prop.location.id = vmm_device;
		hipMemAccessDesc acc = {};
		acc.location.type = hipMemLocationTypeDevice; acc.location.id = vmm_device; acc.flags = hipMemAccessFlagsProtReadWrite;
		for (size_t c = c0; c < c1; ++c) {
			if (chunks[c]) continue;
			std::lock_guard<std::mutex> lk(bhip_vmm_mutex());
			hipMemGenericAllocationHandle_t hnd;
			hipError_t e = hipMemCreate(&hnd, kChunk, &prop, 0);
			if (e != hipSuccess) return fail(BHIP_E_DEVICE, "hipMemCreate(%zu) with %zu chunks mapped: %s", kChunk, n_mapped, hipGetErrorString(e));
			e = hipMemMap((char *)p + c * kChunk, kChunk, 0, hnd, 0);
// ... 119 lines not shown
	DBuf ranges_c[kNumClasses], hdr_c[kNumClasses];
	DBuf qmeta_c[2][kNumClasses];
	uint64_t qmeta_seq[2][kNumClasses] = {};
	bool seeded_ok[kNumClasses] = {false};
	uint64_t seeded_seq[kNumClasses] = {0};
	uint32_t seeded_n[kNumClasses] = {0}, seeded_W16[kNumClasses] = {0};
	hipEvent_t ev_seed[2][kNumClasses][2];
	DBuf peq_alt, peqp_alt;
	bool alt_ok = false; uint64_t alt_seq = 0; int alt_cls = 0, alt_nwp = 0; uint32_t alt_n = 0;
	hipEvent_t ev_peq_alt[2], ev_peq_cur[2];
	bool peq_ahead[kNumClasses] = {false};
	uint64_t task_cap = 1 << 20;
	uint64_t cand_cap = 1 << 18, raw_cap = 1 << 18, win_cap = 1 << 20, scratch_cap = 1 << 18;
	uint32_t npf[kNumClasses] = {0}, nex[kNumClasses] = {0}, maxE[kNumClasses] = {0}, maxwords[kNumClasses] = {0}, maxlen = 0, n_entries = 0;
	Counters *hc_pinned = nullptr;
	Counters hc;
	uint32_t launches = 0, prefix_words = 0;
	uint64_t n_pairs_ex = 0;
	bool masked = false;
};

struct SharedCtr { uint32_t n_out, err; uint32_t *cnt; uint32_t *rank; };
__global__ void k_set_rank_ptrs(SharedCtr *sc, uint32_t *cnt, uint32_t *rank);
struct Handle {
	int device = 0, n_cu = 0;
	char dev_name[256];
	uint64_t hbm = 0;
	hipStream_t stream = nullptr;
	hipStream_t pf_stream = nullptr;
	hipStream_t sweep_stream = nullptr;
	hipStream_t post_stream = nullptr;
	hipEvent_t ev[EV_COUNT];
	uint32_t n_clumps = 0, tot_refs = 0, max_clump_len = 0;
	DBuf ref_lane, ref_off, clump_len, lut;
	BhipMatchMask mm;
	BhipAlt alt;
	bool has_acx = false; int K = 0;
	int acx_z = 0;
	DBuf acx_lines, acx_rec, bad; uint32_t n_bad = 0; uint64_t n_ent = 0, acx_bias = 0;
	BhipAcxView acx_view() const {
		BhipAcxView v; v.lines = acx_lines.as<uint4>();
		v.rec = acx_rec.as<uint32_t>() - acx_bias; return v;
	}
	bool has_masks = false;
	int opt_lane_masks = 1;
	StageSlot slots[3];
	StageSlot *cur = &slots[0];
	uint64_t stage_seq = 0;
	hipStream_t stage_stream = nullptr;
	bool res_valid = false; uint64_t res_seq = 0; int res_all_hits = 0; uint32_t res_n = 0; BhipStats res_stats;
	int opt_host_routing = 0;
	DBuf best, out, shared_ctr, mins, pairs;
	DBuf ref_order, best_key; uint32_t n_order = 0;
	uint32_t *nsel_pinned = nullptr;
	uint32_t res_n_raw = 0;
	SharedCtr *hsc_pinned = nullptr;
	const uint8_t *s_codes() const { return cur->st_has_junk ? cur->qcodes_s.as<uint8_t>() : cur->qcodes.as<uint8_t>(); }
	const uint64_t *s_off() const { return cur->st_has_junk ? cur->qoff_s.as<uint64_t>() : cur->qoff.as<uint64_t>(); }
	const uint16_t *s_emac() const { return cur->st_has_junk ? cur->qemac_s.as<uint16_t>() : cur->qemac.as<uint16_t>(); }
	const uint32_t *s_pack() const { return cur->st_has_junk ? cur->qpack_s.as<uint32_t>() : cur->qpack.as<uint32_t>(); }
	DBuf sort_keys, sort_keys2, sort_idx, sort_tmp, out_sorted, out_sorted2, sort_scratch;
	uint64_t out_cap = 1 << 20;
	std::vector<uint32_t> h_clump_len;
	BhipStats stats;
	std::vector<Lane *> lanes;
	int opt_two_stage = 1;
	int opt_prefilter_stride = 0;
	int opt_lanes = 1;
	int opt_sweep_blocks = 8;
	uint32_t peq_rows = 16;
	int opt_oversub = 2;
	int opt_band_blocks = 0;
	int opt_no_band = 0;
	int opt_async_d2h = 0, out_idx = 0;
	hipStream_t copy_stream = nullptr;
	hipEvent_t ev_sorted = nullptr, ev_copied[2] = {nullptr, nullptr};
	bool copy_pending[2] = {false, false};
	void *reg_ptr[2] = {nullptr, nullptr}; size_t reg_bytes[2] = {0, 0};
	int last_out = 0;
	uint64_t last_n_out = 0;
	int opt_prune = 1;
	int opt_lane_min = 32768;
	int opt_rescore_reg = 1;
	int opt_pf_waves = 0;
	int opt_pf_algo = -1;
	int opt_pf_table = 0;
	int opt_pf_cw = 2;
	int opt_pf_bytes = 1;
	int opt_pf_rb = 0;
	int opt_seed_ahead = 1;
	int opt_seed_ahead_blocks = 2;
	int opt_peq_ahead_blocks = 16;
	void (*enqueued_hook)(void *) = nullptr; void *enqueued_ctx = nullptr;
	int opt_seed_min_need = -1;
	int opt_seed_drop_len = 8;
	double acx_wmean = 0.0;
	void *cov = nullptr;
	long long opt_cov_event_cap = 0;
};

static inline float ev_ms(hipEvent_t a, hipEvent_t b) { float ms = 0; (void)hipEventElapsedTime(&ms, a, b); return ms; }

int  ensure_lanes(Handle *h, uint32_t n);
uint32_t make_seed_plan(const uint8_t *s, uint32_t len, uint32_t E, uint32_t K, int stride_opt, const BhipAlt &A);
int  slot_init(StageSlot *S);
int  resolve_slot(Handle *h, StageSlot *S);
void apply_slot(Handle *h, StageSlot *S);
void lane_capacity_floor(Handle *h, Lane *L, uint64_t n);
int  bhip_load_accelerator(Handle *h, const uint32_t *acx_lens, const void *acx_lists, int acx_fmt, int K, const uint32_t *badlist, uint32_t n_bad);
int  bhip_build_accelerator(Handle *h, int K, int z);
void bhip_cov_release(Handle *h);
#endif
```

### burst_amd/csrc/bhip_init.hip

```cpp
#include "bhip_handle.h"

static thread_local char g_err[512] = "";

__global__ void k_ref_symbol_scan(const uint32_t *__restrict__ w, uint64_t n_words, uint32_t *__restrict__ flag) {
	uint32_t any = 0;
	for (uint64_t i = blockIdx.x * (uint64_t)blockDim.x + threadIdx.x; i < n_words; i += (uint64_t)gridDim.x * blockDim.x) {
		const uint32_t d = w[i];
		any |= (d | ((d << 1) & ((d << 2) | (d << 3)))) & 0x88888888u;
	}
	if (any) *flag = 1u;
}
int bhip_fail_msg(int code, const char *fmt, ...) {
	va_list ap; va_start(ap, fmt); vsnprintf(g_err, sizeof g_err, fmt, ap); va_end(ap);
	return code;
}

extern "C" const char *bhip_last_error(void) { return g_err; }
extern "C" int bhip_abi_version(void) { return BHIP_ABI_VERSION; }
std::atomic<int> &bhip_vmm_peer_access_flag() { return bhip_vmm_peer_access(); }

static void lane_destroy(Lane *L) {
	if (!L) return;
	DBuf *all[] = {&L->peq, &L->peqp, &L->cand, &L->candcnt, &L->wins, &L->raw, &L->wide, &L->scratch, &L->fb_list, &L->gcnt, &L->counters, &L->tasks, &L->tasks2, &L->tasks2k, &L->wins2, &L->rs_lists};
	for (DBuf *b : all) b->release();
// ... 114 lines not shown
		if (clump_len[c] > h->max_clump_len) h->max_clump_len = clump_len[c];
	}
	{
		DBuf d_src, d_srcoff;
		INITRC(d_src.reserve(src_off[n_clumps] * 16 + 16));
		INITRC(d_srcoff.reserve((n_clumps + 1) * sizeof(uint64_t)));
		INITRC(h->ref_lane.reserve_exact(dst_off[n_clumps] * 256 + 256));
		INITRC(h->ref_off.reserve((n_clumps + 1) * sizeof(uint64_t)));
		INITRC(h->clump_len.reserve(n_clumps * sizeof(uint32_t)));
		INITRC(h->lut.reserve(256));
		INITCHK(hipMemcpyAsync(d_src.p, edx_packed, src_off[n_clumps] * 16, hipMemcpyHostToDevice, h->stream));
		INITCHK(hipMemcpyAsync(d_srcoff.p, src_off.data(), (n_clumps + 1) * sizeof(uint64_t), hipMemcpyHostToDevice, h->stream));
		INITCHK(hipMemcpyAsync(h->ref_off.p, dst_off.data(), (n_clumps + 1) * sizeof(uint64_t), hipMemcpyHostToDevice, h->stream));
		INITCHK(hipMemcpyAsync(h->clump_len.p, clump_len, n_clumps * sizeof(uint32_t), hipMemcpyHostToDevice, h->stream));
		INITCHK(hipMemcpyAsync(h->lut.p, score_lut, 256, hipMemcpyHostToDevice, h->stream));
		const uint32_t grid = std::min<uint32_t>(n_clumps, (uint32_t)h->n_cu * 8);
		hipLaunchKernelGGL(k_transpose_refs, dim3(grid), dim3(256), 0, h->stream, d_src.as<uint8_t>(), d_srcoff.as<uint64_t>(),
			h->clump_len.as<uint32_t>(), h->ref_off.as<uint64_t>(), n_clumps, h->ref_lane.as<uint4>());
		INITCHK(hipGetLastError());
		DBuf d_flag;
		INITRC(d_flag.reserve(sizeof(uint32_t)));
		INITCHK(hipMemsetAsync(d_flag.p, 0, sizeof(uint32_t), h->stream));
		hipLaunchKernelGGL(k_ref_symbol_scan, dim3((uint32_t)h->n_cu * 8), dim3(256), 0, h->stream, d_src.as<uint32_t>(), src_off[n_clumps] * 4, d_flag.as<uint32_t>());
		INITCHK(hipGetLastError());
		uint32_t any_other = 1;
		INITCHK(hipMemcpyAsync(&any_other, d_flag.p, sizeof(uint32_t), hipMemcpyDeviceToHost, h->stream));
		INITCHK(hipStreamSynchronize(h->stream));
		h->peq_rows = any_other ? 16u : 5u;
		d_src.release(); d_srcoff.release(); d_flag.release();
	}
	if (getenv("BHIP_DEBUG")) { size_t f_ = 0, t_ = 0; if (hipMemGetInfo(&f_, &t_) == hipSuccess) fprintf(stderr, "[bhip] references on the device (%.2f GB, upload buffer released): %.2f GB of the device's %.2f free\n", h->ref_lane.cap / 1e9, f_ / 1e9, t_ / 1e9); }
	h->acx_z = score_lut[16 * 5 + 5] != 0;
	if (acx_lens) INITRC(bhip_load_accelerator(h, acx_lens, acx_lists, acx_fmt, K, badlist, n_bad));
	else if (K) INITRC(bhip_build_accelerator(h, K, h->acx_z));
	INITRC(ensure_lanes(h, 1));
	if (const char *ev = getenv("BHIP_OPTS")) {
		std::string all(ev);
		for (size_t a = 0; a < all.size();) {
			size_t b = all.find(',', a); if (b == std::string::npos) b = all.size();
			const std::string kv = all.substr(a, b - a); a = b + 1;
			const size_t eq = kv.find('=');
			char *end = nullptr;
			const long long v = eq == std::string::npos ? 0 : strtoll(kv.c_str() + eq + 1, &end, 0);
			if (eq == std::string::npos || eq == 0 || !end || end == kv.c_str() + eq + 1 || *end) { fprintf(stderr, "[bhip] BHIP_OPTS: '%s' is not name=<integer>: ignored\n", kv.c_str()); continue; }
			if (bhip_set_option(h, kv.substr(0, eq).c_str(), v)) fprintf(stderr, "[bhip] BHIP_OPTS: %s: ignored\n", bhip_last_error());
		}
	}
	*handle = h;
	return BHIP_OK;
}


extern "C" int bhip_device_info(void *handle, char *name, int name_cap, int *n_cu, uint64_t *hbm_bytes) {
	Handle *h = (Handle *)handle;
	if (!h) return fail(BHIP_E_ARG, "null handle");
	if (name && name_cap > 0) snprintf(name, (size_t)name_cap, "%s", h->dev_name);
	if (n_cu) *n_cu = h->n_cu;
	if (hbm_bytes) *hbm_bytes = h->hbm;
	return BHIP_OK;
}

extern "C" int bhip_set_option(void *handle, const char *name, long long value) {
	Handle *h = (Handle *)handle;
	if (!h || !name) return fail(BHIP_E_ARG, "null argument");
	if (!strcmp(name, "prefilter_stride")) {
		if (value < 0 || value > 64) return fail(BHIP_E_ARG, "prefilter_stride must be 0 (auto) .. 64");
		h->opt_prefilter_stride = (int)value; return BHIP_OK;
	}
	if (!strcmp(name, "two_stage")) { h->opt_two_stage = value != 0; return BHIP_OK; }
	if (!strcmp(name, "host_routing")) { h->opt_host_routing = value != 0; return BHIP_OK; }
	if (!strcmp(name, "discard_staged")) { for (StageSlot &S : h->slots) if (S.state == 1) S.state = 0; h->res_valid = false; return BHIP_OK; }
	if (!strcmp(name, "lane_masks")) { h->opt_lane_masks = value != 0; return BHIP_OK; }
	if (!strcmp(name, "sweep_blocks")) { if (value < 1 || value > 8) return fail(BHIP_E_ARG, "sweep_blocks must be 1 .. 8"); h->opt_sweep_blocks = (int)value; return BHIP_OK; }
	if (!strcmp(name, "lane_min_entries")) { if (value < 1) return fail(BHIP_E_ARG, "lane_min_entries must be >= 1"); h->opt_lane_min = (int)value; return BHIP_OK; }
	if (!strcmp(name, "async_d2h")) { h->opt_async_d2h = value != 0; return BHIP_OK; }
	if (!strcmp(name, "seed_ahead")) { h->opt_seed_ahead = value != 0; return BHIP_OK; }
	if (!strcmp(name, "peq_ahead_blocks")) { if (value < 1 || value > 16) return fail(BHIP_E_ARG, "peq_ahead_blocks must be 1 .. 16"); h->opt_peq_ahead_blocks = (int)value; return BHIP_OK; }
	if (!strcmp(name, "seed_ahead_blocks")) { if (value < 0 || value > 64) return fail(BHIP_E_ARG, "seed_ahead_blocks must be 0 .. 64"); h->opt_seed_ahead_blocks = (int)value; return BHIP_OK; }
	if (!strcmp(name, "band_blocks")) { if (value < 0 || value > 1024) return fail(BHIP_E_ARG, "band_blocks must be 0 .. 1024"); h->opt_band_blocks = (int)value; return BHIP_OK; }
	if (!strcmp(name, "oversub")) { if (value < 1 || value > 16) return fail(BHIP_E_ARG, "oversub must be 1 .. 16"); h->opt_oversub = (int)value; return BHIP_OK; }
	if (!strcmp(name, "band")) { h->opt_no_band = value == 0; return BHIP_OK; }
	if (!strcmp(name, "prune")) { h->opt_prune = value != 0; return BHIP_OK; }
	if (!strcmp(name, "rescore_reg")) { h->opt_rescore_reg = value != 0; return BHIP_OK; }
	if (!strcmp(name, "seed_min_need")) { if (value < -1 || value > 255) return fail(BHIP_E_ARG, "seed_min_need must be -1 (by rule) or 0 .. 255"); h->opt_seed_min_need = (int)value; return BHIP_OK; }
	if (!strcmp(name, "seed_drop_len")) { if (value < 0 || value > (1 << 24)) return fail(BHIP_E_ARG, "seed_drop_len must be 0 .. 2^24"); h->opt_seed_drop_len = (int)value; return BHIP_OK; }
	if (!strcmp(name, "prefilter_waves")) { if (value < 0 || value > 16) return fail(BHIP_E_ARG, "prefilter_waves must be 0 .. 16"); h->opt_pf_waves = (int)value; return BHIP_OK; }
	if (!strcmp(name, "prefilter_algo")) { if (value < -1 || value > 1) return fail(BHIP_E_ARG, "prefilter_algo must be -1, 0 or 1"); h->opt_pf_algo = (int)value; return BHIP_OK; }
	if (!strcmp(name, "prefilter_table")) { if (value != 0 && (value < 9 || value > 11)) return fail(BHIP_E_ARG, "prefilter_table must be 0, 9, 10 or 11"); h->opt_pf_table = (int)value; return BHIP_OK; }
	if (!strcmp(name, "prefilter_cw")) { if (value < 0 || value > 2) return fail(BHIP_E_ARG, "prefilter_cw must be 0, 1 or 2"); h->opt_pf_cw = (int)value; return BHIP_OK; }
	if (!strcmp(name, "prefilter_bytes")) { h->opt_pf_bytes = value != 0; return BHIP_OK; }
	if (!strcmp(name, "prefilter_rb")) { if (value != 0 && (value < 2 || value > 4)) return fail(BHIP_E_ARG, "prefilter_rb must be 0, 2, 3 or 4"); h->opt_pf_rb = (int)value; return BHIP_OK; }
	if (!strcmp(name, "cov_event_cap")) { if (value < 0) return fail(BHIP_E_ARG, "cov_event_cap must be >= 0 bytes (0 = a fifth of the free memory)"); h->opt_cov_event_cap = value; return BHIP_OK; }
	if (!strcmp(name, "lanes")) {
		if (value < 1 || value > BHIP_MAX_LANES) return fail(BHIP_E_ARG, "lanes must be 1 .. %d", BHIP_MAX_LANES);
		h->opt_lanes = (int)value; for (StageSlot &S : h->slots) { S.state = 0; S.st_valid = false; } return BHIP_OK;
	}
	return fail(BHIP_E_ARG, "unknown option '%s'", name);
}

extern "C" int bhip_get_stats(void *handle, BhipStats *out) {
	Handle *h = (Handle *)handle;
	if (!h || !out) return fail(BHIP_E_ARG, "null argument");
	*out = h->stats;
	return BHIP_OK;
}

int ensure_lanes(Handle *h, uint32_t n) {
	while (h->lanes.size() < n) { Lane *L = nullptr; int rc = lane_create(h, &L); if (rc) return rc; h->lanes.push_back(L); }
	return 0;
}
```

### burst_amd/csrc/bhip_internal.h

```cpp
#ifndef BHIP_INTERNAL_H
#define BHIP_INTERNAL_H
#include <stdint.h>

struct BhipMatchMask { uint16_t m[16]; };

struct BhipRawHit {
	uint32_t q;
	uint32_t refIx;
	uint32_t ed;
	uint32_t e_first;
	uint32_t e_last;
	uint32_t m;
	uint32_t L;
	uint32_t six;
	uint64_t rbase;
};

#define BHIP_WIN_GMASK 0x3FFFFFFFu
struct BhipWin {
	uint32_t li;
	uint32_t refIx;
	uint32_t g_first, g_last;
	uint32_t q;
	uint32_t mE;
	uint32_t nchunks;
	uint32_t L;
	uint64_t rbase;
	uint32_t six;
	uint32_t pad2;
};
__host__ __device__ inline uint32_t bhip_win_class(uint32_t g_first, uint32_t g_last, uint32_t E) {
	const uint64_t diags = 8ull * (g_last - g_first) + 8u + 2u * E;
	return diags <= 26 ? 0u : diags <= 58 ? 1u : diags <= 90 ? 2u : 3u;
}

#define BHIP_PLAN_STRIDE(p) ((p) & 255u)
#define BHIP_PLAN_NEED(p)   (((p) >> 8) & 0xFFFFu)
#define BHIP_PLAN_X(p)      (((p) >> 24) & 15u)
#define BHIP_PLAN_USED(p)   ((p) >> 28)
#define BHIP_EXPAND_SLOTS 8u
struct BhipAlt { uint8_t n[16]; uint8_t base[16]; };

template <class Sym>
__host__ __device__ inline uint32_t bhip_word_class(Sym sym, uint32_t p, uint32_t K, const BhipAlt &A, uint32_t &amb_k, uint32_t &extra) {
	uint32_t namb = 0, bad = 0;
	amb_k = 0; extra = 0;
	for (uint32_t k = 0; k < K; ++k) {
		const uint32_t n = A.n[sym(p + k) & 15u];
		if (n == 0u) bad = 1u;
		else if (n > 1u) { ++namb; amb_k = k; extra = n - 1u; }
	}
	return (bad || namb > 1u) ? 0u : (namb ? 2u : 1u);
}
template <class Sym>
__host__ __device__ inline void bhip_expand_walk(Sym sym, uint32_t K, uint32_t upto, const BhipAlt &A, uint32_t &w_strict, uint32_t &x, uint32_t &used) {
	w_strict = 0; x = 0; used = 0;
	for (uint32_t j = 0; j < upto; ++j) {
		uint32_t ak, ex;
		const uint32_t c = bhip_word_class(sym, j * K, K, A, ak, ex);
		if (c == 1u) ++w_strict;
		else if (c == 2u && used + ex <= BHIP_EXPAND_SLOTS) { ++x; used += ex; }
	}
}

#define BHIP_N_CLASSES  8
#define BHIP_MAX_LANES  15
#define BHIP_ROUTE_KEYS 240
#define BHIP_ROUTE_SKIP 255
struct BhipStageInfo {
	uint32_t count[256];
	uint32_t maxE[BHIP_ROUTE_KEYS / 2], maxwords[BHIP_ROUTE_KEYS / 2];
	unsigned long long seed_words[BHIP_ROUTE_KEYS / 2];
	uint32_t maxlen_lane[16], n_entries_lane[16];
	uint32_t junk;
	uint32_t err, err_i, err_len;
	uint32_t maxE_all, maxlen_all;
};

typedef void (*bhip_pf_kernel_t)(const uint2 *, const uint2 *, uint32_t, uint32_t, const uint32_t *, const uint32_t *, uint32_t, const uint32_t *, uint32_t,
	uint2 *, uint32_t *, uint32_t, unsigned long long *, uint32_t *, uint32_t *, unsigned long long *, unsigned long long *, unsigned long long *, unsigned long long *,
	uint2 *, uint32_t *, int, const uint32_t *, const uint32_t *, int);
extern "C" bhip_pf_kernel_t bhip_legacy_pf_kernel(int kind, int htb, int rb, int cw_mode, int big) __attribute__((weak));

#define BHIP_RESCORE_WMAX 48

#define BHIP_ACX_LINE_WORDS 14u
#define BHIP_REC_BYTES 4
#define BHIP_REC_PAD 0xFFFFFFFFu
struct BhipAcxView {
	const uint4 *lines;
	const uint32_t *rec;
};

#include "bhip_lanecode.h"

#ifdef __HIPCC__
typedef const uint32_t __attribute__((address_space(1))) *bhip_gptr_t;
__device__ __forceinline__ void bhip_acx_range(const BhipAcxView &a, uint32_t w, unsigned long long &beg, uint32_t &n) {
	const uint32_t blk = w / BHIP_ACX_LINE_WORDS, j = w - blk * BHIP_ACX_LINE_WORDS;
	const uint32_t *L = (const uint32_t *)(a.lines + 4ull * blk);
	const unsigned long long b0 = (unsigned long long)L[0] | (unsigned long long)L[1] << 32;
	const uint32_t hi = L[2 + j], lo_raw = L[1 + j];
	const uint32_t lo = j ? lo_raw : 0u;
	beg = b0 + lo;
	n = hi - lo;
}
__device__ __forceinline__ uint2 bhip_acx_rec(const uint32_t *rec, unsigned long long e) {
	const uint32_t v = rec[e];
	return make_uint2(v & 0xFFFFFFu, bhip_lane_code_mask(v >> 24));
}
__device__ __forceinline__ uint32_t bhip_acx_clump(const uint32_t *rec, unsigned long long e) { return rec[e] & 0xFFFFFFu; }
__device__ __forceinline__ uint32_t bhip_acx_raw_issue(const uint32_t *rec, unsigned long long e, bool valid, const void *dummy) {
	const uintptr_t addr = valid ? (uintptr_t)(rec + e) : (uintptr_t)dummy;
	return ((bhip_gptr_t)addr)[0];
}
__device__ __forceinline__ uint32_t bhip_acx_raw_finish(uint32_t raw, bool valid, uint32_t &sink) {
	sink ^= raw;
	return valid ? raw : BHIP_REC_PAD;
}
__device__ __forceinline__ uint32_t bhip_acx_raw_or_pad(const uint32_t *rec, unsigned long long e, bool valid, const void *dummy, uint32_t &sink) {
	return bhip_acx_raw_finish(bhip_acx_raw_issue(rec, e, valid, dummy), valid, sink);
}
__device__ __forceinline__ void bhip_hit_rank(uint32_t *n_out, uint32_t pos, uint32_t q) {
	uint32_t *const *pp = (uint32_t *const *)(n_out + 2);
	uint32_t *cnt = pp[0], *rank = pp[1];
	if (cnt) rank[pos] = atomicAdd(&cnt[q], 1u);
}
#endif

#endif
```

### burst_amd/csrc/bhip_kernels.hip

```cpp
#include <hip/hip_runtime.h>
#include <stdint.h>
#include <type_traits>
#include "burst_hip.h"
#include "bhip_internal.h"

__global__ void k_transpose_refs(const uint8_t *__restrict__ src, const uint64_t *__restrict__ src_off,
                                 const uint32_t *__restrict__ clump_len, const uint64_t *__restrict__ dst_off,
                                 uint32_t n_clumps, uint4 *__restrict__ dst_lane) {
	const uint32_t z = threadIdx.x & 15, g = threadIdx.x >> 4, gpb = blockDim.x >> 4;
	for (uint32_t c = blockIdx.x; c < n_clumps; c += gridDim.x) {
		const uint32_t L = clump_len[c], nrows = (L + 1) >> 1, nchunks = (L + 31) >> 5;
		const uint8_t *s = src + src_off[c] * 16;
		for (uint32_t t = g; t < nchunks; t += gpb) {
			uint32_t w[4] = {0, 0, 0, 0};
			#pragma unroll
			for (int i = 0; i < 16; ++i) {
				uint32_t row = 16 * t + i;
				uint32_t b = row < nrows ? s[(uint64_t)row * 16 + z] : 0u;
				w[i >> 2] |= b << (8 * (i & 3));
			}
			dst_lane[dst_off[c] * 16 + (uint64_t)z * nchunks + t] = make_uint4(w[0], w[1], w[2], w[3]);
		}
	}
}
// ... 1062 lines not shown
			const int x = m + dlo + k;
			if (x < 1 || x > (int)L) continue;
			const uint32_t cell = band[(uint32_t)k * stride], key = cell >> GS;
			if (key < bkey) { bkey = key; bv = cell & 255u; }
		}
		for (int k = 0; k < Wd; ++k) {
			const int x = m + dlo + k;
			if (x < 1 || x > (int)L) continue;
			if ((band[(uint32_t)k * stride] >> GS) == bkey) fin = (uint32_t)x;
		}
		const uint32_t bs = bkey >> 8, bh = 255u - (bkey & 255u);
		if (bs != B) { atomicOr(err_flags, 1u); continue; }
		const uint32_t pos = atomicAdd(n_out, 1u);
		if (pos < out_cap) {
			BhipHit o;
			o.q = q; o.refIx = h.refIx; o.finalPos = fin;
			o.score = 1.0f - (float)bs / ((float)m + (float)bh);
			o.ed = (uint8_t)B; o.gapR = (uint8_t)bv; o.gapQ = (uint8_t)bh; o.rc = qrc ? qrc[q] : 0;
			out[pos] = o;
			bhip_hit_rank(n_out, pos, q);
		}
	}
}

__global__ __launch_bounds__(256) void k_rescore_classify(
		const BhipRawHit *__restrict__ raw, const uint32_t *__restrict__ n_raw_dev, uint32_t raw_cap,
		const uint32_t *__restrict__ best, int all_hits, const uint64_t *__restrict__ qoff,
		const uint32_t *__restrict__ qsix, const uint8_t *__restrict__ qrc, const uint32_t *__restrict__ clump_len,
		BhipHit *__restrict__ out, uint32_t *__restrict__ n_out, uint32_t out_cap,
		uint32_t *__restrict__ lists, uint32_t *__restrict__ counts, uint32_t *__restrict__ wide, uint32_t *__restrict__ n_wide,
		uint32_t band_rows, int use_reg) {
	__shared__ uint32_t s_cnt[12], s_base[12];
	uint32_t n = *n_raw_dev;
	if (n > raw_cap) n = raw_cap;
	const uint32_t tid = threadIdx.x;
	for (uint32_t chunk = blockIdx.x * 1024u; chunk < n; chunk += gridDim.x * 1024u) {
		if (tid < 12) s_cnt[tid] = 0;
		__syncthreads();
		int bucket[4]; uint32_t rank[4], e2v[4], mv[4], qv[4], rv[4];
		#pragma unroll
		for (int t = 0; t < 4; ++t) {
			const uint32_t i = chunk + (uint32_t)t * 256u + tid;
			bucket[t] = -1; rank[t] = 0; e2v[t] = 0; mv[t] = 0; qv[t] = 0; rv[t] = 0;
			if (i < n) {
				const BhipRawHit h = raw[i];
				if (all_hits || h.ed == best[h.six]) {
					const uint32_t L = h.L;
					const uint32_t e2 = h.e_last < L ? h.e_last : L;
					qv[t] = h.q; rv[t] = h.refIx; e2v[t] = e2;
					if (h.ed == 0) { bucket[t] = 11; mv[t] = h.m; }
					else {
						const uint32_t Wd = e2 - h.e_first + 2 * h.ed + 1;
						int bk = !use_reg || h.ed > 254u ? 9 : Wd <= 4 ? 0 : Wd <= 6 ? 1 : Wd <= 8 ? 2 : Wd <= 12 ? 3 : Wd <= 16 ? 4 : Wd <= 24 ? 5 : Wd <= 32 ? 6 : Wd <= 40 ? 7 : Wd <= 48 ? 8 : 9;
						if (Wd > band_rows && bk == 9) bk = 10;
						bucket[t] = bk;
					}
					rank[t] = atomicAdd(&s_cnt[bucket[t]], 1u);
				}
			}
		}
		__syncthreads();
		if (tid < 12 && s_cnt[tid]) s_base[tid] = atomicAdd(tid == 11 ? n_out : tid == 10 ? n_wide : &counts[tid], s_cnt[tid]);
		__syncthreads();
		#pragma unroll
		for (int t = 0; t < 4; ++t) {
			const uint32_t i = chunk + (uint32_t)t * 256u + tid;
			const int bk = bucket[t];
			if (bk < 0) continue;
			const uint32_t pos = s_base[bk] + rank[t];
			if (bk == 11) {
				if (pos < out_cap) {
					BhipHit o; o.q = qv[t]; o.refIx = rv[t]; o.finalPos = e2v[t]; o.score = 1.0f - 0.0f / (float)mv[t];
					o.ed = 0; o.gapR = 0; o.gapQ = 0; o.rc = qrc ? qrc[qv[t]] : 0;
					out[pos] = o;
					bhip_hit_rank(n_out, pos, qv[t]);
				}
			} else if (bk == 10) wide[pos] = i;
			else lists[(size_t)bk * raw_cap + pos] = i;
		}
		__syncthreads();
	}
}

template <int WB>
__device__ __forceinline__ void rescore_reg_one(
		const BhipRawHit *__restrict__ hp, bool live, uint32_t *s_mm, uint32_t fastq, uint32_t lane,
		const uint64_t *__restrict__ qoff, const uint8_t *__restrict__ qrc, const uint32_t *__restrict__ qpack, uint32_t qw,
		const uint32_t *__restrict__ refw, const uint64_t *__restrict__ ref_off, const uint32_t *__restrict__ clump_len,
		BhipHit *__restrict__ out, uint32_t *__restrict__ n_out, uint32_t out_cap, uint32_t *__restrict__ err_flags) {
	constexpr int NW = (WB + 7) / 8 + 1;
	constexpr uint32_t SS = 18, GS = 10;
	const uint32_t INVALID = (512u << SS) | (255u << GS), Z0 = 255u << GS;
	const uint32_t STEP_U = (1u << SS) + 1u + (1u << 8), STEP_L = (1u << SS) - (1u << GS) + (2u << 8);
	uint32_t bkey = 0xFFFFFFFFu, bv = 0, fin = 0xFFFFFFFFu, m = 0, B = 0, hq = 0, hrefIx = 0;
	if (live) {
		const uint32_t q = hp->q;
		hq = q; hrefIx = hp->refIx;
		B = hp->ed;
		const uint32_t h_first = hp->e_first, h_last = hp->e_last;
		const uint32_t L = hp->L, nchunks = (L + 31) >> 5;
		m = hp->m;
		const int e2 = (int)(h_last < L ? h_last : L), e1 = (int)h_first;
		const int dlo = e1 - (int)m - (int)B, Wd = e2 - e1 + 2 * (int)B + 1;
		const uint64_t rbase = hp->rbase;
		const uint32_t LIM = (B + 1) << SS;
		uint32_t bd[WB + 1];
		#pragma unroll
		for (int k = 0; k < WB; ++k) { const int x = dlo + k; bd[k] = (k < Wd && x >= 0 && x <= (int)L) ? Z0 : INVALID; }
		bd[WB] = INVALID;
		int p = dlo, j8 = dlo >> 3;
		uint32_t d[NW];
		#pragma unroll
		for (int i = 0; i < NW; ++i) d[i] = ref_dword_at(refw, rbase, j8 + i, nchunks);
		auto all_acgt = [&]() { uint32_t bad = 0;
			#pragma unroll
			for (int i = 0; i < NW; ++i) bad |= (d[i] - 0x11111111u) & 0xCCCCCCCCu;
			return bad == 0; };
		bool dclean = all_acgt();
		int jn = j8 + NW;
		uint4 ahead = ref_chunk_at(refw, rbase, jn >> 2, nchunks);
		const uint32_t *qp = qpack + (uint64_t)q * qw;
		uint32_t qd = qp[0], q_next = qw > 1 ? qp[1] : 0u;
		uint32_t prev_sym = (ref_dword_at(refw, rbase, (p - 1) >> 3, nchunks) >> (4 * ((p - 1) & 7))) & 15u;
		for (int y = 1; y <= (int)m; ++y) {
			const uint32_t qi = (uint32_t)(y - 1);
			if ((qi & 7u) == 0 && qi) { qd = q_next; q_next = (qi >> 3) + 1 < qw ? qp[(qi >> 3) + 1] : 0u; }
			const uint32_t qc = (qd >> (4 * (qi & 7u))) & 15u;
			const uint32_t col0 = (uint32_t)y <= B ? (((uint32_t)y << SS) | Z0 | (uint32_t)y) : INVALID;
			const int x0 = y + dlo;
			const bool fast_row = y > 1 && x0 >= 1 && dclean && ((fastq >> qc) & 1u);
			const uint32_t mrow = fast_row ? 0u : s_mm[qc];
			const uint32_t m1 = mrow >> 16;
			uint32_t dd[NW - 1];
			{
				const uint32_t sh = 4u * ((uint32_t)p & 7u);
				#pragma unroll
				for (int i = 0; i < NW - 1; ++i) dd[i] = __builtin_amdgcn_alignbit(d[i + 1], d[i], sh);
			}
			const int kmax = (Wd - 1) < ((int)L - x0) ? (Wd - 1) : ((int)L - x0);
			if (y == 1) {
				#pragma unroll
				for (int k = 0; k < WB; ++k) {
					const int x = x0 + k;
					const uint32_t r = (dd[k >> 3] >> (4 * (k & 7))) & 15u;
					const uint32_t cst = ((mrow >> r) & 1u) ? 0u : (((m1 >> r) & 1u) ? 1u : 255u);
					uint32_t hh = 0;
					if (cst == 1 && x >= 2) hh = (mrow >> prev_sym) & 1u;
					uint32_t cell = cst == 255u ? INVALID : ((cst << SS) | ((255u - hh) << GS));
					if (x < 1) cell = x == 0 ? col0 : INVALID;
					if (k > kmax) cell = INVALID;
					prev_sym = r;
					bd[k] = cell;
				}
			} else if (fast_row) {
				uint32_t nz[NW - 1];
				#pragma unroll
				for (int i = 0; i < NW - 1; ++i) { const uint32_t x = dd[i] ^ (qc * 0x11111111u); nz[i] = ((x & 0x77777777u) + 0x77777777u) | x; }
				uint32_t left = (x0 - 1 == 0) ? col0 : INVALID;
				uint32_t dg = bd[0];
				#pragma unroll
				for (int k = 0; k < WB; ++k) {
					const uint32_t up = bd[k + 1];
					const uint32_t cD = dg + (((nz[k >> 3] >> (4 * (k & 7) + 3)) & 1u) << SS), cU = up + STEP_U, cL = left + STEP_L;
					uint32_t cm = cD < cU ? cD : cU;
					cm = cm < cL ? cm : cL;
					cm &= ~0x300u;
					uint32_t cell = cm >= LIM ? INVALID : cm;
					if (k > kmax) cell = INVALID;
					bd[k] = cell;
					left = cell;
					dg = up;
				}
			} else {
				uint32_t left = (x0 - 1 == 0) ? col0 : INVALID;
				uint32_t dg = bd[0];
				#pragma unroll
				for (int k = 0; k < WB; ++k) {
					const uint32_t r = (dd[k >> 3] >> (4 * (k & 7))) & 15u;
					const uint32_t up = bd[k + 1];
					const uint32_t cstS = ((mrow >> r) & 1u) ? 0u : (((m1 >> r) & 1u) ? (1u << SS) : (255u << SS));
					const uint32_t cD = dg + cstS, cU = up + STEP_U, cL = left + STEP_L;
					uint32_t cm = cD < cU ? cD : cU;
					cm = cm < cL ? cm : cL;
					cm &= ~0x300u;
					uint32_t cell = cm >= LIM ? INVALID : cm;
					if (x0 < 1) { const int x = x0 + k; if (x < 1) cell = x == 0 ? col0 : INVALID; }
					if (k > kmax) cell = INVALID;
					bd[k] = cell;
					left = cell;
					dg = up;
				}
			}
			++p;
			if ((p & 7) == 0) {
				#pragma unroll
				for (int i = 0; i < NW - 1; ++i) d[i] = d[i + 1];
				d[NW - 1] = pick4(ahead, (uint32_t)jn & 3u);
				dclean = all_acgt();
				++j8; ++jn;
				if ((jn & 3) == 0) ahead = ref_chunk_at(refw, rbase, jn >> 2, nchunks);
			}
		}
		#pragma unroll
		for (int k = 0; k < WB; ++k) {
			const int x = (int)m + dlo + k;
			if (k < Wd && x >= 1 && x <= (int)L) { const uint32_t key = bd[k] >> GS; if (key < bkey) { bkey = key; bv = bd[k] & 255u; } }
		}
		#pragma unroll
		for (int k = 0; k < WB; ++k) {
			const int x = (int)m + dlo + k;
			if (k < Wd && x >= 1 && x <= (int)L && (bd[k] >> GS) == bkey) fin = (uint32_t)x;
		}
	}
	const uint32_t bs = bkey >> 8, bh = 255u - (bkey & 255u);
	const bool ok = live && bs == B;
	if (live && !ok) atomicOr(err_flags, 1u);
	const unsigned long long bm = __ballot(ok);
	if (bm) {
		uint32_t base = 0;
		if (lane == (uint32_t)__builtin_ctzll(bm)) base = atomicAdd(n_out, (uint32_t)__popcll(bm));
		base = __shfl(base, __builtin_ctzll(bm));
		if (ok) {
			const uint32_t pos = base + __popcll(bm & ((1ull << lane) - 1ull));
			if (pos < out_cap) {
				BhipHit o;
				o.q = hq; o.refIx = hrefIx; o.finalPos = fin;
				o.score = 1.0f - (float)bs / ((float)m + (float)bh);
				o.ed = (uint8_t)B; o.gapR = (uint8_t)bv; o.gapQ = (uint8_t)bh; o.rc = qrc ? qrc[hq] : 0;
				out[pos] = o;
				bhip_hit_rank(n_out, pos, hq);
			}
		}
	}
}

template <int SET>
__global__ __launch_bounds__(64) void k_rescore_reg(
		const BhipRawHit *__restrict__ raw, const uint32_t *__restrict__ lists, const uint32_t *__restrict__ counts, uint32_t raw_cap,
		const uint64_t *__restrict__ qoff, const uint8_t *__restrict__ qrc, const uint32_t *__restrict__ qpack, uint32_t qw,
		const uint8_t *__restrict__ refb, const uint64_t *__restrict__ ref_off, const uint32_t *__restrict__ clump_len,
		const uint8_t *__restrict__ lut,
		BhipHit *__restrict__ out, uint32_t *__restrict__ n_out, uint32_t out_cap, uint32_t *__restrict__ err_flags) {
	__shared__ uint32_t s_mm[16];
	const uint32_t tid = threadIdx.x;
	if (tid < 16) { uint32_t mm = 0; for (int r = 0; r < 16; ++r) mm |= (lut[16 * tid + r] == 0 ? 1u : 0u) << r | (lut[16 * tid + r] != 255 ? 1u : 0u) << (16 + r); s_mm[tid] = mm; }
	__syncthreads();
	uint32_t fastq = 0;
	for (uint32_t qc = 1; qc <= 4; ++qc) if ((s_mm[qc] & 0x1Eu) == (1u << qc)) fastq |= 1u << qc;
	const uint32_t *refw = (const uint32_t *)refb;
#define BHIP_RS_RUN(b, WB) { \
		uint32_t n = counts[b]; if (n > raw_cap) n = raw_cap; \
		const uint32_t *lst = lists + (size_t)(b) * raw_cap; \
		const uint32_t n_round = (n + 63u) & ~63u; \
		for (uint32_t i = blockIdx.x * 64 + tid; i < n_round; i += gridDim.x * 64) { \
			const bool live = i < n; \
			rescore_reg_one<WB>(raw + (live ? lst[i] : 0u), live, s_mm, fastq, tid, qoff, qrc, qpack, qw, refw, ref_off, clump_len, out, n_out, out_cap, err_flags); \
		} }
	if (SET == 0) { BHIP_RS_RUN(0, 4) BHIP_RS_RUN(1, 6) BHIP_RS_RUN(2, 8) }
	else if (SET == 3) { BHIP_RS_RUN(3, 12) }
	else if (SET == 1) { BHIP_RS_RUN(4, 16) BHIP_RS_RUN(5, 24) }
	else { BHIP_RS_RUN(6, 32) BHIP_RS_RUN(7, 40) BHIP_RS_RUN(8, 48) }
#undef BHIP_RS_RUN
}
template __global__ void k_rescore_reg<0>(const BhipRawHit *, const uint32_t *, const uint32_t *, uint32_t, const uint64_t *, const uint8_t *, const uint32_t *, uint32_t,
	const uint8_t *, const uint64_t *, const uint32_t *, const uint8_t *, BhipHit *, uint32_t *, uint32_t, uint32_t *);
template __global__ void k_rescore_reg<1>(const BhipRawHit *, const uint32_t *, const uint32_t *, uint32_t, const uint64_t *, const uint8_t *, const uint32_t *, uint32_t,
	const uint8_t *, const uint64_t *, const uint32_t *, const uint8_t *, BhipHit *, uint32_t *, uint32_t, uint32_t *);
template __global__ void k_rescore_reg<2>(const BhipRawHit *, const uint32_t *, const uint32_t *, uint32_t, const uint64_t *, const uint8_t *, const uint32_t *, uint32_t,
	const uint8_t *, const uint64_t *, const uint32_t *, const uint8_t *, BhipHit *, uint32_t *, uint32_t, uint32_t *);
template __global__ void k_rescore_reg<3>(const BhipRawHit *, const uint32_t *, const uint32_t *, uint32_t, const uint64_t *, const uint8_t *, const uint32_t *, uint32_t,
	const uint8_t *, const uint64_t *, const uint32_t *, const uint8_t *, BhipHit *, uint32_t *, uint32_t, uint32_t *);

template __global__ void k_rescore<false>(const BhipRawHit *, const uint32_t *, uint32_t, const uint32_t *, const uint32_t *, const uint32_t *, int,
	const uint8_t *, const uint64_t *, const uint32_t *, const uint8_t *, const uint8_t *, const uint64_t *, const uint32_t *, const uint8_t *,
	BhipHit *, uint32_t *, uint32_t, uint32_t *, uint32_t *, uint32_t *, unsigned long long *, unsigned long long, uint32_t *,
	const uint32_t *, uint32_t, uint32_t, uint32_t);
template __global__ void k_rescore<true>(const BhipRawHit *, const uint32_t *, uint32_t, const uint32_t *, const uint32_t *, const uint32_t *, int,
	const uint8_t *, const uint64_t *, const uint32_t *, const uint8_t *, const uint8_t *, const uint64_t *, const uint32_t *, const uint8_t *,
	BhipHit *, uint32_t *, uint32_t, uint32_t *, uint32_t *, uint32_t *, unsigned long long *, unsigned long long, uint32_t *,
	const uint32_t *, uint32_t, uint32_t, uint32_t);
```

### burst_amd/csrc/bhip_stage.hip

```cpp
#include "bhip_handle.h"

uint32_t make_seed_plan(const uint8_t *s, uint32_t len, uint32_t E, uint32_t K, int stride_opt, const BhipAlt &A) {
	if (len < K) return 1u;
	const uint32_t npos = len - K + 1;
	bool clean = true;
	for (uint32_t i = 0; i < len; ++i) if ((uint32_t)(s[i] - 1u) >= 4u) { clean = false; break; }
	std::vector<uint8_t> valid;
	if (!clean) {
		valid.assign(npos, 0);
		uint32_t run = 0;
		for (uint32_t i = 0; i < len; ++i) { run = ((uint32_t)(s[i] - 1u) < 4u) ? run + 1 : 0; if (i + 1 >= K && run >= K) valid[i + 1 - K] = 1; }
	}
	uint32_t xk = 0, usedk = 0;
	auto sym = [&](uint32_t i) -> uint32_t { return s[i]; };
	auto need_of = [&](uint32_t st) -> int {
		uint32_t W = 0;
		if (clean) W = (len - K) / st + 1;
		else if (st == K) { uint32_t ws; bhip_expand_walk(sym, K, (len - K) / K + 1, A, ws, xk, usedk); W = ws + xk; }
		else for (uint32_t p = 0; p < npos; p += st) W += valid[p];
		return (int)W - (int)(E * ((K + st - 1) / st));
	};
	const uint32_t smin = (len - K) / 254 + 1;
	uint32_t best_s = 0; int best_n = 0;
	if (stride_opt > 0) { best_s = std::max<uint32_t>((uint32_t)stride_opt, smin); best_n = need_of(best_s); }
	else {
		for (uint32_t st = std::max(K, smin); st >= smin; --st) { const int n = need_of(st); if (n >= 3) { best_s = st; best_n = n; break; } if (st == smin) break; }
		if (!best_s) for (uint32_t st = smin; st <= std::max(K, smin); ++st) { const int n = need_of(st); if (n > best_n) { best_n = n; best_s = st; } }
		if (!best_s) { best_s = smin; best_n = need_of(smin); }
	}
	if (best_n < 1) best_n = 0;
	if (best_n > 0xFFFF) best_n = 0xFFFF;
	const bool ex = !clean && best_s == K && best_n > 0 && xk > 0;
	return (best_s & 255u) | ((uint32_t)best_n << 8) | (ex ? xk << 24 | usedk << 28 : 0u);
}

int slot_init(StageSlot *S) {
	if (S->ev_done) return 0;
	if (hipEventCreate(&S->ev_begin) != hipSuccess || hipEventCreate(&S->ev_done) != hipSuccess || hipEventCreate(&S->ev_copied) != hipSuccess) return fail(BHIP_E_DEVICE, "hipEventCreate failed");
	if (hipHostMalloc((void **)&S->info_pinned, sizeof(BhipStageInfo), hipHostMallocDefault) != hipSuccess) return fail(BHIP_E_DEVICE, "hipHostMalloc failed");
	int rc = S->info.reserve(sizeof(BhipStageInfo));
	return rc;
}

static uint32_t lanes_for(const Handle *h, uint32_t n_q) {
	uint32_t nl = (uint32_t)h->opt_lanes;
	while (nl > 1 && n_q / nl < (uint32_t)h->opt_lane_min) --nl;
	return nl;
}

static int stage_enqueue(Handle *h, StageSlot *S, const BhipQuerySpan *spans, uint32_t n_spans, const uint32_t *six_explicit, bool share_by_position,
                         uint32_t n_shared, uint32_t max_len) {
	int rc;
	if ((rc = slot_init(S))) return rc;
	hipStream_t st = h->stage_stream;
	uint64_t n_q64 = 0, nb = 0;
	bool any_rc = false, any_flags = false, all_flags = true, any_qbase = false, all_packed = true, all_packed2 = true, all_len = true;
	for (uint32_t k = 0; k < n_spans; ++k) {
		const BhipQuerySpan &sp = spans[k];
		if (!sp.n) continue;
		if (!sp.codes || !sp.off || !sp.emac) return fail(BHIP_E_ARG, "null query arrays");
		if (share_by_position && sp.n > n_shared) return fail(BHIP_E_ARG, "span %u has %u entries for %u shared slots", k, sp.n, n_shared);
		n_q64 += sp.n; nb += sp.off[sp.n] - sp.off[0];
		all_packed &= sp.codes4 != nullptr; all_packed2 &= sp.codes2 != nullptr; all_len &= sp.len != nullptr;
		any_rc |= sp.rc != nullptr; any_flags |= sp.flags != nullptr; all_flags &= sp.flags != nullptr; any_qbase |= sp.q_base != 0 || k > 0;
	}
	if (n_q64 > 0xFFFFFFF0ull) return fail(BHIP_E_ARG, "too many entries in one batch");
	if (any_flags && !all_flags) return fail(BHIP_E_ARG, "q_flags given for some spans only");
	const uint32_t n_q = (uint32_t)n_q64;
	S->spans.assign(spans, spans + n_spans);
	S->six_explicit = six_explicit;
	S->resolved = false; S->st_valid = false; S->st_has_junk = false;
	S->st_nq = n_q; S->st_has_six = six_explicit != nullptr || share_by_position; S->st_has_rc = any_rc; S->has_flags = any_flags; S->has_qmap = any_qbase;
	S->st_nshared = S->st_has_six ? n_shared : n_q;
	S->st_lanes = n_q ? lanes_for(h, n_q) : 0;
	S->seq = ++h->stage_seq;
	if (!n_q) { S->st_maxlen = 0; return 0; }
	if ((rc = ensure_lanes(h, S->st_lanes))) return rc;
	if (!max_len) {
		for (uint32_t k = 0; k < n_spans; ++k) for (uint32_t j = 0; j < spans[k].n; ++j) {
			const uint64_t len = spans[k].off[j + 1] - spans[k].off[j];
			if (len > BHIP_MAX_QLEN) return fail(BHIP_E_QUERYLEN, "query %u has %llu symbols (max %d)", j, (unsigned long long)len, BHIP_MAX_QLEN);
			max_len = std::max<uint32_t>(max_len, (uint32_t)len);
		}
	}
	if (max_len > BHIP_MAX_QLEN) return fail(BHIP_E_QUERYLEN, "queries of up to %u symbols (max %d)", max_len, BHIP_MAX_QLEN);
	S->st_maxlen = max_len;
	const uint32_t qw = (max_len + 7) / 8;
	if (all_packed2) all_packed = false;
	if ((all_packed || all_packed2) && (rc = S->qcodes4.reserve(nb / 2 + 2 * (size_t)n_spans + 64))) return rc;
	if (all_len && (rc = S->qlen16.reserve(((size_t)n_q + n_spans + 1) * 2 + 64))) return rc;
	if ((rc = S->qcodes.reserve(nb + 2 * (size_t)n_spans + 64)) || (rc = S->qoff.reserve(((size_t)n_q + 1) * 8)) || (rc = S->qemac.reserve(((size_t)n_q + 1) * 2)) ||
	    (rc = S->qsix.reserve(((size_t)n_q + 1) * 4)) || (rc = S->qrc.reserve((size_t)n_q + 1)) || (rc = S->qflags.reserve((size_t)n_q + 1)) ||
	    (rc = S->qmap.reserve(((size_t)n_q + 1) * 4)) || (rc = S->off_raw.reserve(((size_t)n_q + n_spans + 1) * 8)) || (rc = S->plan.reserve((size_t)n_q * 4 + 16)) ||
	    (rc = S->qpack.reserve((size_t)n_q * qw * 4 + 64)) || (rc = S->key.reserve((size_t)n_q + 16)) || (rc = S->key_sorted.reserve((size_t)n_q + 16)) ||
	    (rc = S->idx.reserve((size_t)n_q * 4 + 16)) || (rc = S->idx_sorted.reserve((size_t)n_q * 4 + 16))) return rc;
	HIPCHK(hipEventRecord(S->ev_begin, st));
	uint32_t ebase = 0; uint64_t pos = 0, pos4 = 0;
	for (uint32_t k = 0; k < n_spans; ++k) {
		const BhipQuerySpan &sp = spans[k];
		if (!sp.n) continue;
		const uint64_t bytes = sp.off[sp.n] - sp.off[0];
		if (all_packed2) {
			pos4 = ((pos4 + 3) & ~3ull) + (sp.off[0] & 3ull);
			if (bytes) {
				HIPCHK(hipMemcpyAsync(S->qcodes4.as<uint8_t>() + (pos4 >> 2), sp.codes2 + (sp.off[0] >> 2), ((sp.off[sp.n] + 3) >> 2) - (sp.off[0] >> 2), hipMemcpyHostToDevice, st));
				hipLaunchKernelGGL(k_unpack2, dim3((uint32_t)std::min<uint64_t>((bytes / 4 + 256) / 256, (uint64_t)h->n_cu * 16)), dim3(256), 0, st, S->qcodes4.as<uint8_t>(), pos4, bytes,
					S->qcodes.as<uint8_t>() + pos);
				HIPCHK(hipGetLastError());
			}
			pos4 += bytes;
		} else if (all_packed) {
			pos4 = ((pos4 + 1) & ~1ull) + (sp.off[0] & 1ull);
			if (bytes) {
				HIPCHK(hipMemcpyAsync(S->qcodes4.as<uint8_t>() + (pos4 >> 1), sp.codes4 + (sp.off[0] >> 1), ((sp.off[sp.n] + 1) >> 1) - (sp.off[0] >> 1), hipMemcpyHostToDevice, st));
				hipLaunchKernelGGL(k_unpack4, dim3((uint32_t)std::min<uint64_t>((bytes / 4 + 256) / 256, (uint64_t)h->n_cu * 16)), dim3(256), 0, st, S->qcodes4.as<uint8_t>(), pos4, bytes,
					S->qcodes.as<uint8_t>() + pos);
				HIPCHK(hipGetLastError());
			}
			pos4 += bytes;
		} else if (bytes) HIPCHK(hipMemcpyAsync(S->qcodes.as<uint8_t>() + pos, sp.codes + sp.off[0], bytes, hipMemcpyHostToDevice, st));
		uint64_t *raw = S->off_raw.as<uint64_t>() + ebase + k;
		if (all_len) {
			uint16_t *dl = S->qlen16.as<uint16_t>() + ebase + k;
			HIPCHK(hipMemcpyAsync(dl, sp.len, (size_t)sp.n * 2, hipMemcpyHostToDevice, st));
			HIPCHK(hipMemsetAsync(dl + sp.n, 0, 2, st));
			auto widen = [] __host__ __device__(uint16_t v) -> unsigned long long { return (unsigned long long)v; };
			hipcub::TransformInputIterator<unsigned long long, decltype(widen), const uint16_t *> it(dl, widen);
			size_t tb = 0;
			HIPCHK(hipcub::DeviceScan::ExclusiveSum(nullptr, tb, it, (unsigned long long *)raw, (int)(sp.n + 1), st));
			if ((rc = S->sort_tmp.reserve(tb + 16))) return rc;
			HIPCHK(hipcub::DeviceScan::ExclusiveSum(S->sort_tmp.p, tb, it, (unsigned long long *)raw, (int)(sp.n + 1), st));
		} else HIPCHK(hipMemcpyAsync(raw, sp.off, ((size_t)sp.n + 1) * 8, hipMemcpyHostToDevice, st));
		HIPCHK(hipMemcpyAsync(S->qemac.as<uint16_t>() + ebase, sp.emac, (size_t)sp.n * 2, hipMemcpyHostToDevice, st));
		if (sp.rc) HIPCHK(hipMemcpyAsync(S->qrc.as<uint8_t>() + ebase, sp.rc, sp.n, hipMemcpyHostToDevice, st));
		else if (any_rc) HIPCHK(hipMemsetAsync(S->qrc.as<uint8_t>() + ebase, 0, sp.n, st));
		if (sp.flags) HIPCHK(hipMemcpyAsync(S->qflags.as<uint8_t>() + ebase, sp.flags, sp.n, hipMemcpyHostToDevice, st));
		if (six_explicit) HIPCHK(hipMemcpyAsync(S->qsix.as<uint32_t>() + ebase, six_explicit + ebase, (size_t)sp.n * 4, hipMemcpyHostToDevice, st));
		hipLaunchKernelGGL(k_span_fill, dim3(std::min<uint32_t>((sp.n + 256) / 256, (uint32_t)h->n_cu * 4)), dim3(256), 0, st, raw, sp.n, ebase, pos, sp.q_base,
			S->qoff.as<uint64_t>(), share_by_position ? S->qsix.as<uint32_t>() : (uint32_t *)nullptr, S->qmap.as<uint32_t>());
		HIPCHK(hipGetLastError());
		ebase += sp.n; pos += bytes;
	}
	HIPCHK(hipEventRecord(S->ev_copied, st));
	{
		const uint64_t total = (uint64_t)n_q * qw;
		if (total) hipLaunchKernelGGL(k_pack_queries, dim3((uint32_t)std::min<uint64_t>((total + 255) / 256, (uint64_t)h->n_cu * 16)), dim3(256), 0, st,
			S->qcodes.as<uint8_t>(), S->qoff.as<uint64_t>(), n_q, qw, S->qpack.as<uint32_t>());
		HIPCHK(hipGetLastError());
	}
	HIPCHK(hipMemsetAsync(S->info.p, 0, sizeof(BhipStageInfo), st));
	hipLaunchKernelGGL(k_route, dim3(std::min<uint32_t>((n_q + 255) / 256, (uint32_t)h->n_cu * 8)), dim3(256), 0, st, S->qoff.as<uint64_t>(), S->qpack.as<uint32_t>(), qw,
		S->qemac.as<uint16_t>(), S->st_has_six ? S->qsix.as<uint32_t>() : (const uint32_t *)nullptr, any_flags ? S->qflags.as<uint8_t>() : (const uint8_t *)nullptr,
		n_q, S->st_nshared, S->st_lanes, h->has_acx ? 1 : 0, h->K, h->opt_prefilter_stride, S->plan.as<uint32_t>(), S->key.as<uint8_t>(), S->idx.as<uint32_t>(),
		S->info.as<BhipStageInfo>(), h->alt);
	HIPCHK(hipGetLastError());
	{
		size_t tb = 0;
		HIPCHK(hipcub::DeviceRadixSort::SortPairs(nullptr, tb, S->key.as<uint8_t>(), S->key_sorted.as<uint8_t>(), S->idx.as<uint32_t>(), S->idx_sorted.as<uint32_t>(), (int)n_q, 0, 8, st));
		if ((rc = S->sort_tmp.reserve(tb + 16))) return rc;
		HIPCHK(hipcub::DeviceRadixSort::SortPairs(S->sort_tmp.p, tb, S->key.as<uint8_t>(), S->key_sorted.as<uint8_t>(), S->idx.as<uint32_t>(), S->idx_sorted.as<uint32_t>(), (int)n_q, 0, 8, st));
	}
	HIPCHK(hipMemcpyAsync(S->info_pinned, S->info.p, sizeof(BhipStageInfo), hipMemcpyDeviceToHost, st));
	HIPCHK(hipEventRecord(S->ev_done, st));
	return 0;
}

static void slot_take_info(StageSlot *S, const BhipStageInfo &I) {
	uint32_t off = 0;
	for (uint32_t l = 0; l < 16; ++l) {
		for (int c = 0; c < kNumClasses; ++c) {
// ... 63 lines not shown
				clean.clear();
				for (uint64_t k = 0; k < len_all; ++k) if (codes_i[k]) clean.push_back(codes_i[k]);
				const uint64_t nx_i = len_all - clean.size();
				P.junk = true;
				nxv[i] = (uint8_t)std::min<uint64_t>(nx_i, 255);
				if (nx_i > E_i || clean.empty()) { nxv[i] = 255; continue; }
				E_i -= (uint32_t)nx_i; len = clean.size(); codes_i = clean.data();
			}
			const uint32_t six = q_six ? q_six[i] : i;
			const uint32_t l = (uint32_t)(((uint64_t)six * nl) / nsh);
			const int cls = class_of_len((uint32_t)len);
			int ex = q_flags ? (q_flags[i] == BHIP_Q_EXHAUSTIVE) : !h->has_acx;
			if (!h->has_acx) ex = 1;
			if (!ex) {
				plan[i] = make_seed_plan(codes_i, (uint32_t)len, E_i, (uint32_t)h->K, h->opt_prefilter_stride, h->alt);
				if (BHIP_PLAN_NEED(plan[i]) == 0) ex = 1;
			}
			const size_t lc = (size_t)l * kNumClasses + cls;
			P.lists[lc * 2 + ex].push_back(i);
			P.maxE[lc] = std::max<uint32_t>(P.maxE[lc], E_i);
			if (!ex && len >= (uint64_t)h->K) {
				const uint32_t nwd = (uint32_t)((len - h->K) / (plan[i] & 255u) + 1) + BHIP_PLAN_USED(plan[i]);
				P.maxwords[lc] = std::max<uint32_t>(P.maxwords[lc], nwd);
				P.seed_words[lc] += nwd;
			}
			P.maxlen[l] = std::max<uint32_t>(P.maxlen[l], (uint32_t)len_all);
			++P.n_entries[l];
		}
	};
	if (n_thr == 1) work(0);
	else {
		std::vector<std::thread> th;
		for (uint32_t t = 0; t < n_thr; ++t) th.emplace_back(work, t);
		for (auto &x : th) x.join();
	}
	for (const Part &P : parts) {
		if (P.err == 1) return fail(BHIP_E_QUERYLEN, "query %u has %llu symbols (max %d)", P.err_i, (unsigned long long)P.err_len, BHIP_MAX_QLEN);
		if (P.err == 2) return fail(BHIP_E_ARG, "q_six[%u] out of range", P.err_i);
	}
	BhipStageInfo I;
	memset(&I, 0, sizeof I);
	std::vector<uint32_t> sorted; sorted.reserve(n_q);
	for (uint32_t l = 0; l < nl; ++l) for (int c = 0; c < kNumClasses; ++c) for (int ex = 0; ex < 2; ++ex) {
		const size_t lc = (size_t)l * kNumClasses + c, k = lc * 2 + ex;
		for (const Part &P : parts) { sorted.insert(sorted.end(), P.lists[k].begin(), P.lists[k].end()); I.count[(l * BHIP_N_CLASSES + c) * 2 + ex] += (uint32_t)P.lists[k].size(); }
		if (!ex) for (const Part &P : parts) {
			I.maxE[l * BHIP_N_CLASSES + c] = std::max(I.maxE[l * BHIP_N_CLASSES + c], P.maxE[lc]); I.maxwords[l * BHIP_N_CLASSES + c] = std::max(I.maxwords[l * BHIP_N_CLASSES + c], P.maxwords[lc]);
			I.seed_words[l * BHIP_N_CLASSES + c] += P.seed_words[lc];
		}
	}
	for (uint32_t l = 0; l < nl; ++l) for (const Part &P : parts) { I.maxlen_lane[l] = std::max(I.maxlen_lane[l], P.maxlen[l]); I.n_entries_lane[l] += P.n_entries[l]; }
	for (uint32_t i = 0; i < n_q; ++i) I.maxE_all = std::max<uint32_t>(I.maxE_all, q_emac[i]);
	slot_take_info(S, I);
	hipStream_t st = h->stage_stream;
	HIPCHK(hipMemcpyAsync(S->plan.p, plan.data(), (size_t)n_q * 4, hipMemcpyHostToDevice, st));
	if (!sorted.empty()) HIPCHK(hipMemcpyAsync(S->idx_sorted.p, sorted.data(), sorted.size() * 4, hipMemcpyHostToDevice, st));
	S->st_has_junk = false;
	for (const Part &P : parts) S->st_has_junk |= P.junk;
	if (S->st_has_junk) {
		std::vector<uint64_t> off_s((size_t)n_q + 1, 0);
		std::vector<uint16_t> emac_s(n_q);
		std::vector<uint8_t> codes_s; codes_s.reserve(q_off[n_q] + 16);
		std::vector<uint8_t> nxs(nsh + 1, 0);
		for (uint32_t i = 0; i < n_q; ++i) {
			const uint8_t *c = q_codes + q_off[i]; const uint64_t len = q_off[i + 1] - q_off[i];
			if (!nxv[i]) codes_s.insert(codes_s.end(), c, c + len);
			else if (nxv[i] != 255) for (uint64_t k = 0; k < len; ++k) { if (c[k]) codes_s.push_back(c[k]); }
			off_s[i + 1] = codes_s.size();
			emac_s[i] = (uint16_t)(nxv[i] == 255 ? 0 : q_emac[i] - nxv[i]);
			if (nxv[i] == 255) nxv[i] = 0;
			nxs[q_six ? q_six[i] : i] = nxv[i];
		}
		codes_s.resize(codes_s.size() + 16, 0);
		if ((rc = S->qcodes_s.reserve(codes_s.size()))) return rc;
		if ((rc = S->qoff_s.reserve(((size_t)n_q + 1) * 8))) return rc;
		if ((rc = S->qemac_s.reserve(((size_t)n_q + 1) * 2))) return rc;
		if ((rc = S->nx.reserve((size_t)n_q + 16))) return rc;
		if ((rc = S->nx_six.reserve((size_t)nsh + 16))) return rc;
		HIPCHK(hipMemcpyAsync(S->qcodes_s.p, codes_s.data(), codes_s.size(), hipMemcpyHostToDevice, st));
		HIPCHK(hipMemcpyAsync(S->qoff_s.p, off_s.data(), ((size_t)n_q + 1) * 8, hipMemcpyHostToDevice, st));
		HIPCHK(hipMemcpyAsync(S->qemac_s.p, emac_s.data(), (size_t)n_q * 2, hipMemcpyHostToDevice, st));
		HIPCHK(hipMemcpyAsync(S->nx.p, nxv.data(), n_q, hipMemcpyHostToDevice, st));
		HIPCHK(hipMemcpyAsync(S->nx_six.p, nxs.data(), nsh, hipMemcpyHostToDevice, st));
		const uint32_t qw_g = (S->st_maxlen + 7) / 8;
		if ((rc = S->qpack_s.reserve((size_t)n_q * qw_g * 4 + 64))) return rc;
		const uint64_t total = (uint64_t)n_q * qw_g;
		if (total) hipLaunchKernelGGL(k_pack_queries, dim3((uint32_t)std::min<uint64_t>((total + 255) / 256, (uint64_t)h->n_cu * 16)), dim3(256), 0, st,
			S->qcodes_s.as<uint8_t>(), S->qoff_s.as<uint64_t>(), n_q, qw_g, S->qpack_s.as<uint32_t>());
		HIPCHK(hipGetLastError());
	}
	HIPCHK(hipStreamSynchronize(st));
	return 0;
}

int resolve_slot(Handle *h, StageSlot *S) {
	if (S->resolved) return 0;
	if (!S->st_nq) { S->resolved = true; S->st_valid = true; S->st_lanes = 0; return 0; }
	HIPCHK(hipEventSynchronize(S->ev_done));
	const BhipStageInfo &I = *S->info_pinned;
	if (I.err == 1) return fail(BHIP_E_QUERYLEN, "query %u has %u symbols (max %d)", I.err_i, I.err_len, BHIP_MAX_QLEN);
	if (I.err == 2) return fail(BHIP_E_ARG, "q_six[%u] out of range", I.err_i);
	S->st_ms_h2d = ev_ms(S->ev_begin, S->ev_done);
	S->st_ms_copy = ev_ms(S->ev_begin, S->ev_copied); S->st_ms_route = ev_ms(S->ev_copied, S->ev_done);
	if (I.junk || h->opt_host_routing) { int rc = host_route(h, S); if (rc) return rc; }
	else slot_take_info(S, I);
	S->resolved = true; S->st_valid = true;
	if (getenv("BHIP_DEBUG")) fprintf(stderr, "[bhip] stage: %u entries, %s routing, copies + routing %.2f ms on the staging stream\n", S->st_nq,
		(I.junk || h->opt_host_routing) ? "host" : "device", S->st_ms_h2d);
	return 0;
}

void lane_capacity_floor(Handle *h, Lane *L, uint64_t n) {
	L->task_cap = std::max<uint64_t>(L->task_cap, 3 * n + 4096); L->win_cap = std::max<uint64_t>(L->win_cap, 2 * n + 4096);
	L->raw_cap = std::max<uint64_t>(L->raw_cap, 2 * n + 4096); L->cand_cap = std::max<uint64_t>(L->cand_cap, n / 4 + 4096);
	h->out_cap = std::max<uint64_t>(h->out_cap, 2 * n + 4096);
}

void apply_slot(Handle *h, StageSlot *S) {
	h->cur = S;
	for (uint32_t l = 0; l < S->st_lanes && l < h->lanes.size(); ++l) {
		Lane *L = h->lanes[l];
		for (int c = 0; c < kNumClasses; ++c) {
			L->npf[c] = S->npf[l][c]; L->nex[c] = S->nex[l][c]; L->maxE[c] = S->maxE[l][c]; L->maxwords[c] = S->maxwords[l][c]; L->seed_words[c] = S->seed_words[l][c];
			L->qlist[c] = S->idx_sorted.as<uint32_t>() + S->qlist_off[l][c];
		}
		L->maxlen = S->maxlen_lane[l]; L->n_entries = S->n_entries_lane[l];
		lane_capacity_floor(h, L, L->n_entries);
	}
}

static StageSlot *free_slot(Handle *h) {
	for (StageSlot &S : h->slots) if (S.state == 0) return &S;
	for (StageSlot &S : h->slots) if (S.state == 2) return &S;
	return nullptr;
}

extern "C" int bhip_stage_spans(void *handle, const BhipQuerySpan *spans, uint32_t n_spans, uint32_t n_shared, uint32_t max_len) {
	Handle *h = (Handle *)handle;
	if (!h || (!spans && n_spans)) return fail(BHIP_E_ARG, "null argument");
	HIPCHK(hipSetDevice(h->device));
	StageSlot *S = free_slot(h);
	if (!S) return fail(BHIP_E_ARG, "every staging slot holds a batch that has not been aligned yet: align one first");
	S->state = 0;
	int rc = stage_enqueue(h, S, spans, n_spans, nullptr, true, n_shared, max_len);
	if (rc) return rc;
	S->state = 1;
	return BHIP_OK;
}

extern "C" int bhip_stage_queries(void *handle, const uint8_t *q_codes, const uint64_t *q_off, const uint16_t *q_emac,
                                  const uint32_t *q_six, const uint8_t *q_rc, const uint8_t *q_flags, uint32_t n_q, uint32_t n_shared) {
	Handle *h = (Handle *)handle;
	if (!h) return fail(BHIP_E_ARG, "null handle");
	if (n_q && (!q_codes || !q_off || !q_emac)) return fail(BHIP_E_ARG, "null query arrays");
	HIPCHK(hipSetDevice(h->device));
	for (StageSlot &S : h->slots) if (S.state == 1) S.state = 0;
	StageSlot *S = free_slot(h);
	S->state = 0;
	BhipQuerySpan sp;
	memset(&sp, 0, sizeof sp);
	sp.codes = q_codes; sp.off = q_off; sp.emac = q_emac; sp.rc = q_rc; sp.flags = q_flags; sp.n = n_q; sp.q_base = 0;
	int rc = stage_enqueue(h, S, &sp, n_q ? 1u : 0u, q_six, false, n_shared, 0);
	if (rc) return rc;
	if ((rc = resolve_slot(h, S))) return rc;
	S->spans.clear(); S->six_explicit = nullptr;
	S->state = 1;
	return BHIP_OK;
// ... 36 lines not shown
```

### include/burst_hip.h

```cpp
#ifndef BURST_HIP_H
#define BURST_HIP_H
#include <stdint.h>
#ifdef __cplusplus
extern "C" {
#endif
#define BHIP_API __attribute__((visibility("default")))

#define BHIP_OK            0
#define BHIP_E_ARG        -1
#define BHIP_E_DEVICE     -2
#define BHIP_E_CAPACITY   -3
#define BHIP_E_QUERYLEN   -4
#define BHIP_E_INTERNAL   -5
#define BHIP_E_RESCORE    -6

#define BHIP_MAX_QLEN   4095

typedef struct BhipHit {
	uint32_t q;
	uint32_t refIx;
	uint32_t finalPos;
	float    score;
	uint8_t  ed;
	uint8_t  gapR;
// ... 45 lines not shown
BHIP_API int bhip_align_staged(void *handle, int all_hits, BhipHit *hits, uint64_t cap, uint64_t *n_hits);
#define BHIP_HITS_MIN   0
#define BHIP_HITS_ALL   1
#define BHIP_HITS_BEST  2
BHIP_API int bhip_set_ref_order(void *handle, const uint32_t *order, uint32_t n);

typedef struct BhipQuerySpan {
	const uint8_t  *codes;
	const uint8_t  *codes4;
	const uint64_t *off;
	const uint16_t *emac;
	const uint8_t  *rc;
	const uint8_t  *flags;
	uint32_t n;
	uint32_t q_base;
	const uint8_t  *codes2;
	const uint16_t *len;
} BhipQuerySpan;
BHIP_API int bhip_stage_spans(void *handle, const BhipQuerySpan *spans, uint32_t n_spans, uint32_t n_shared, uint32_t max_len);

BHIP_API int bhip_set_enqueued_hook(void *handle, void (*fn)(void *ctx), void *ctx);

BHIP_API int bhip_reserve(void *handle, uint32_t n_entries, uint32_t max_len);
BHIP_API int bhip_reserve_symbols(void *handle, uint32_t n_entries, uint32_t max_len, uint64_t total_symbols);

BHIP_API void *bhip_alloc_host(uint64_t bytes);
BHIP_API void  bhip_free_host(void *p);
BHIP_API int   bhip_host_register(void *p, uint64_t bytes);
BHIP_API int   bhip_host_unregister(void *p);

BHIP_API int  bhip_comm_create(int n_ranks, const int *devices, void **comm);
BHIP_API int  bhip_comm_unique_id(void *id128);
BHIP_API int  bhip_comm_create_rank(int n_ranks, int rank, int device, const void *id128, void **comm);
BHIP_API int  bhip_comm_gather_hits(void *comm, int rank, const BhipHit *hits, uint64_t n, BhipHit *out, uint64_t cap, uint64_t *n_total, uint64_t *counts);
BHIP_API int  bhip_comm_stage_device(void *comm, int rank, void *handle, uint64_t first_record, uint64_t *n_records);
BHIP_API int  bhip_comm_gather_staged(void *comm, int rank, uint64_t n, BhipHit *out, uint64_t cap, uint64_t *n_total, uint64_t *counts);
BHIP_API void bhip_comm_stage_reset(void *comm, int rank);
BHIP_API int  bhip_comm_fetch_gathered(void *comm, BhipHit *out, uint64_t cap, uint64_t *n_total);
BHIP_API int  bhip_comm_allreduce_min(void *comm, int rank, uint8_t *buf, uint64_t n);
BHIP_API void bhip_comm_destroy(void *comm);

typedef int (*bhip_share_fn)(void *ctx, void *device_base, const uint64_t *byte_off, int part, int n_parts, int status);
typedef struct { void *comm; int rank; } BhipCommRank;
BHIP_API int  bhip_build_accelerator_shared(void *handle, int K, int part, int n_parts, bhip_share_fn share, void *ctx);
BHIP_API int  bhip_comm_share(void *comm_rank, void *device_base, const uint64_t *byte_off, int part, int n_parts, int status);
BHIP_API int  bhip_team_create(int n_ranks, void **team);
BHIP_API void bhip_team_destroy(void *team);
BHIP_API int  bhip_team_share(void *team, void *device_base, const uint64_t *byte_off, int part, int n_parts, int status);
BHIP_API int  bhip_device_copy(void *dst, const void *src, uint64_t bytes, int to_device);

BHIP_API int bhip_acx_export(void *handle, uint32_t *lens, uint32_t *clumps, uint16_t *masks, uint64_t cap_entries, uint64_t *n_entries,
                    uint32_t *badlist, uint32_t cap_bad, uint32_t *n_bad);
BHIP_API int bhip_acx_export_entries(void *handle, uint64_t first, uint64_t n_entries, uint32_t *clumps, uint16_t *masks);

BHIP_API int bhip_align_pairs(void *handle, const uint8_t *q_codes, const uint64_t *q_off, const uint16_t *q_emac,
                     uint32_t n_q, const uint32_t *pair_q, const uint32_t *pair_clump, uint64_t n_pairs,
                     uint8_t *mins);

BHIP_API int bhip_prefilter(void *handle, const uint8_t *q_codes, const uint64_t *q_off, const uint16_t *q_emac,
                   uint32_t n_q, uint32_t *out_q, uint32_t *out_clump, uint32_t *out_count,
                   uint64_t cap, uint64_t *n_out);

BHIP_API int bhip_copy_hits_device(void *handle, void *dst_device, uint64_t cap_records, uint64_t *n_records);

BHIP_API int bhip_sync_hits(void *handle);

BHIP_API int bhip_sort_queries(int device, const uint8_t *codes, uint64_t codes_bytes, const uint64_t *start, const uint32_t *len,
                      uint64_t n, uint32_t max_len, uint32_t *perm, uint8_t *is_new);

BHIP_API int bhip_dna_marks(int device, const uint8_t *sym, uint64_t sym_len, const uint64_t *ref_start, const uint32_t *ref_len,
                            uint64_t n_refs, uint32_t W, uint64_t *max_chain, uint64_t *max_sh, uint8_t *flags, uint64_t *info);

typedef struct BhipCovLine { uint32_t ref, st, ed, w; } BhipCovLine;
BHIP_API int bhip_cov_begin(void *handle, uint32_t n_headers, const uint32_t *lengths, uint32_t pad);
BHIP_API int bhip_cov_add(void *handle, uint32_t sample, const BhipCovLine *lines, uint64_t n);
BHIP_API int bhip_cov_sample_stats(void *handle, uint32_t sample, uint64_t *shared, uint64_t *unique);
BHIP_API int bhip_cov_dataset_stats(void *handle, uint64_t *shared, uint64_t *unique);
BHIP_API int bhip_cov_info(void *handle, uint64_t info[8]);
BHIP_API int bhip_cov_end(void *handle);
BHIP_API int bhip_lane_extents(void *handle, uint32_t *extents);

BHIP_API int bhip_set_option(void *handle, const char *name, long long value);

BHIP_API int bhip_get_stats(void *handle, BhipStats *out);
BHIP_API int bhip_device_info(void *handle, char *name, int name_cap, int *n_cu, uint64_t *hbm_bytes);

BHIP_API void bhip_destroy(void *handle);
BHIP_API const char *bhip_last_error(void);
BHIP_API int bhip_abi_version(void);
#define BHIP_ABI_VERSION 8

#ifdef __cplusplus
}
#endif
#endif
```

Measured before the change: 601.8 million.

## Stage query and reference words in LDS for register rescore on short queries

Pads the packed-query stride to a multiple of four dwords so each query's packed words can be loaded as aligned uint4 vectors. A new STAGED variant of k_rescore_reg bulk-loads the query and the reference window into registers up front, then parks the later words in per-lane LDS slots. The inner DP loop reads those slots instead of issuing scattered global loads. It applies only when the longest query is at most 128 symbols, which covers these 100-bp reads, and it trades higher register and LDS use (with a waves-per-EU hint) for fewer dependent global memory accesses in the rescoring pass.

```diff
diff --git a/burst_amd/capi.py b/burst_amd/capi.py
--- a/burst_amd/capi.py
+++ b/burst_amd/capi.py
@@ -39,7 +39,7 @@
            "bhip_device_info", "bhip_destroy", "bhip_last_error", "bhip_abi_version", "bhip_set_ref_order", "bhip_copy_hits_device", "bhip_sync_hits",
            "bhip_comm_create", "bhip_comm_unique_id", "bhip_comm_create_rank", "bhip_comm_allreduce_min", "bhip_comm_fetch_gathered", "bhip_comm_gather_hits", "bhip_comm_stage_device", "bhip_comm_gather_staged", "bhip_comm_stage_reset", "bhip_comm_destroy", "bhip_acx_export", "bhip_reserve", "bhip_reserve_symbols", "bhip_sort_queries", "bhip_stage_spans", "bhip_alloc_host", "bhip_free_host", "bhip_host_register", "bhip_host_unregister", "bhip_set_enqueued_hook", "bhip_acx_export_entries",
            "bhip_build_accelerator_shared", "bhip_comm_share", "bhip_team_create", "bhip_team_destroy", "bhip_team_share", "bhip_device_copy", "bhip_dna_marks",
-           "bhip_cov_begin", "bhip_cov_add", "bhip_cov_sample_stats", "bhip_cov_dataset_stats", "bhip_cov_info", "bhip_cov_end", "bhip_lane_extents"]
+           "bhip_cov_begin", "bhip_cov_add", "bhip_cov_sample_stats", "bhip_cov_dataset_stats", "bhip_cov_info", "bhip_cov_end", "bhip_lane_extents", "bhip_qpack_stride"]
 
 COV_LINE_DTYPE = np.dtype([("ref", "<u4"), ("st", "<u4"), ("ed", "<u4"), ("w", "<u4")])
 assert COV_LINE_DTYPE.itemsize == 16
@@ -77,6 +77,8 @@
     lib.bhip_align_pairs.restype = i32
     lib.bhip_prefilter.argtypes = [vp, vp, vp, vp, u32, vp, vp, vp, u64, C.POINTER(u64)]
     lib.bhip_prefilter.restype = i32
+    lib.bhip_qpack_stride.argtypes = [u32]
+    lib.bhip_qpack_stride.restype = u32
     lib.bhip_set_option.argtypes = [vp, C.c_char_p, C.c_longlong]
     lib.bhip_set_option.restype = i32
     lib.bhip_get_stats.argtypes = [vp, C.POINTER(BhipStats)]
diff --git a/burst_amd/csrc/bhip_align.hip b/burst_amd/csrc/bhip_align.hip
--- a/burst_amd/csrc/bhip_align.hip
+++ b/burst_amd/csrc/bhip_align.hip
@@ -322,13 +322,13 @@
 	{
 		const uint32_t qb = 256u / (uint32_t)NW;
 		const uint32_t grid = (uint32_t)std::min<uint64_t>(((uint64_t)n_list + qb - 1) / qb, (uint64_t)h->n_cu * blocks_per_cu);
-		hipLaunchKernelGGL(k_build_peq, dim3(grid), dim3(256), 0, st, codes, off, d_qlist, n_list, NW, 0, h->mm, peq.as<uint32_t>(), pack, (S->st_maxlen + 7) / 8, h->peq_rows);
+		hipLaunchKernelGGL(k_build_peq, dim3(grid), dim3(256), 0, st, codes, off, d_qlist, n_list, NW, 0, h->mm, peq.as<uint32_t>(), pack, bhip_qstride(S->st_maxlen), h->peq_rows);
 		HIPCHK(hipGetLastError());
 	}
 	if (NWP) {
 		const uint32_t qb = 256u / (uint32_t)NWP;
 		const uint32_t grid = (uint32_t)std::min<uint64_t>(((uint64_t)n_list + qb - 1) / qb, (uint64_t)h->n_cu * blocks_per_cu);
-		hipLaunchKernelGGL(k_build_peq, dim3(grid), dim3(256), 0, st, codes, off, d_qlist, n_list, NWP, 32 * NWP, h->mm, peqp.as<uint32_t>(), pack, (S->st_maxlen + 7) / 8, h->peq_rows);
+		hipLaunchKernelGGL(k_build_peq, dim3(grid), dim3(256), 0, st, codes, off, d_qlist, n_list, NWP, 32 * NWP, h->mm, peqp.as<uint32_t>(), pack, bhip_qstride(S->st_maxlen), h->peq_rows);
 		HIPCHK(hipGetLastError());
 	}
 	return 0;
@@ -354,7 +354,7 @@
 	hipLaunchKernelGGL(k_seed_ranges, dim3(grid), dim3(256), 0, st,
 		junk ? S->qcodes_s.as<uint8_t>() : S->qcodes.as<uint8_t>(), junk ? S->qoff_s.as<uint64_t>() : S->qoff.as<uint64_t>(), d_qlist, n_list,
 		h->acx_view(), h->K, S->plan.as<uint32_t>(), W16, L->ranges_c[cls].as<uint2>(), L->hdr_c[cls].as<uint2>(),
-		junk ? S->qpack_s.as<uint32_t>() : S->qpack.as<uint32_t>(), (S->st_maxlen + 7) / 8, junk ? S->qemac_s.as<uint16_t>() : S->qemac.as<uint16_t>(), qm.as<uint4>(), S->st_has_six ? S->qsix.as<uint32_t>() : nullptr,
+		junk ? S->qpack_s.as<uint32_t>() : S->qpack.as<uint32_t>(), bhip_qstride(S->st_maxlen), junk ? S->qemac_s.as<uint16_t>() : S->qemac.as<uint16_t>(), qm.as<uint4>(), S->st_has_six ? S->qsix.as<uint32_t>() : nullptr,
 		seed_min_need_for(h, mean_words, W16), (uint32_t)h->opt_seed_drop_len, h->alt);
 	HIPCHK(hipGetLastError());
 	HIPCHK(hipEventRecord(ev[SPAN_DONE], st));
@@ -441,7 +441,7 @@
 	HIPCHK(hipSetDevice(h->device));
 	int rc;
 	if (getenv("BHIP_DEBUG")) { size_t f_ = 0, t_ = 0; if (hipMemGetInfo(&f_, &t_) == hipSuccess) fprintf(stderr, "[bhip] reserve for %u entries of up to %u symbols: %.2f GB of the device's %.2f free\n", n_entries, max_len, f_ / 1e9, t_ / 1e9); }
-	const size_t n = n_entries, nb = total_symbols ? (size_t)std::min<uint64_t>(total_symbols + 64, (uint64_t)n * max_len) : n * max_len, qw = (max_len + 7) / 8;
+	const size_t n = n_entries, nb = total_symbols ? (size_t)std::min<uint64_t>(total_symbols + 64, (uint64_t)n * max_len) : n * max_len, qw = bhip_qstride((uint32_t)max_len);
 	const size_t cw = (size_t)class_words(class_of_len(max_len), max_len);
 	const size_t peq_words = total_symbols ? std::min<size_t>(n * cw, 2 * (nb / 32 + n)) : n * cw;
 	for (StageSlot &S : h->slots) {
@@ -625,6 +625,8 @@
 	return 0;
 }
 
+static bool rescore_staged(const Handle *h) { return h->opt_rescore_stage && h->cur->st_maxlen && h->cur->st_maxlen <= BHIP_RESCORE_STAGE_MAXLEN; }
+
 static int enqueue_rescore(Handle *h, Lane *L, const BatchCall &b) {
 	hipStream_t po = h->post_stream;
 	Counters *dc = L->counters.as<Counters>();
@@ -640,19 +642,28 @@
 		if (s1 > s0) hipLaunchKernelGGL(k_junk_adjust_best, dim3(std::min<uint32_t>((s1 - s0 + 255) / 256, (uint32_t)h->n_cu * 4)), dim3(256), 0, po, h->best.as<uint32_t>(), h->cur->nx_six.as<uint8_t>(), s0, s1);
 		HIPCHK(hipGetLastError());
 	}
-	const uint32_t qw_g = (h->cur->st_maxlen + 7) / 8;
+	const uint32_t qw_g = bhip_qstride(h->cur->st_maxlen);
 	hipLaunchKernelGGL(k_rescore_classify, dim3((uint32_t)h->n_cu * 8), dim3(256), 0, po, L->raw.as<BhipRawHit>(), &dc->n_raw, (uint32_t)L->raw_cap,
 		h->best.as<uint32_t>(), b.all_hits, h->cur->qoff.as<uint64_t>(), six_or_null(h), rc_or_null(h),
 		R.len, h->out.as<BhipHit>(), &sc->n_out, (uint32_t)h->out_cap, L->rs_lists.as<uint32_t>(), dc->n_rs, L->wide.as<uint32_t>(), &dc->n_wide,
 		b.band_rows, h->opt_rescore_reg);
 	HIPCHK(hipGetLastError());
 	if (h->opt_rescore_reg) {
+		const bool staged = rescore_staged(h);
+		const uint32_t stg_q = staged ? (h->cur->st_maxlen + 7) / 8 : 0;
+		if (getenv("BHIP_DEBUG")) {
+			uint32_t li = 0;
+			for (uint32_t l = 0; l < h->lanes.size(); ++l) if (h->lanes[l] == L) li = l;
+			fprintf(stderr, "[bhip] lane %u: k_rescore_reg %s (longest query %u symbols)\n", li, staged ? "staged" : "streaming", h->cur->st_maxlen);
+		}
 		for_each_int(SetList{}, [&](auto set) {
 			constexpr int SET = decltype(set)::value;
-			const uint32_t grid = (uint32_t)h->n_cu * std::min<uint32_t>(32u, blocks_per_cu((const void *)k_rescore_reg<SET>, 64, 0)) * (uint32_t)h->opt_oversub;
-			hipLaunchKernelGGL(k_rescore_reg<SET>, dim3(grid), dim3(64), 0, po, L->raw.as<BhipRawHit>(), L->rs_lists.as<uint32_t>(), dc->n_rs, (uint32_t)L->raw_cap,
+			auto fn = staged ? k_rescore_reg<SET, true> : k_rescore_reg<SET, false>;
+			const size_t lds = staged ? (size_t)bhip_rs_stage_dwords(h->cur->st_maxlen) * 256 : 0;
+			const uint32_t grid = (uint32_t)h->n_cu * std::min<uint32_t>(32u, blocks_per_cu((const void *)fn, 64, lds)) * (uint32_t)h->opt_oversub;
+			hipLaunchKernelGGL(fn, dim3(grid), dim3(64), lds, po, L->raw.as<BhipRawHit>(), L->rs_lists.as<uint32_t>(), dc->n_rs, (uint32_t)L->raw_cap,
 				h->cur->qoff.as<uint64_t>(), rc_or_null(h), h->cur->qpack.as<uint32_t>(), qw_g,
-				R.bytes(), R.off, R.len, h->lut.as<uint8_t>(), h->out.as<BhipHit>(), &sc->n_out, (uint32_t)h->out_cap, &sc->err);
+				R.bytes(), R.off, R.len, h->lut.as<uint8_t>(), h->out.as<BhipHit>(), &sc->n_out, (uint32_t)h->out_cap, &sc->err, stg_q);
 		});
 		HIPCHK(hipGetLastError());
 	}
@@ -749,7 +760,7 @@
 }
 static int plan_batch(Handle *h, BatchCall &b) {
 	b.band_rows = std::min<uint32_t>(BHIP_RESCORE_WMAX, 2 * h->cur->st_maxE + 1 + 9);
-	b.qw = (h->cur->st_maxlen + 7) / 8; b.rw = (h->cur->st_maxlen + b.band_rows + 24) / 8 + 2;
+	b.qw = bhip_qstride(h->cur->st_maxlen); b.rw = (h->cur->st_maxlen + b.band_rows + 24) / 8 + 2;
 	if ((size_t)(b.band_rows + 1 + b.qw + b.rw) * 256 > 40 * 1024) { b.qw = 0; b.rw = 0; }
 	if (!b.sel_best) return BHIP_OK;
 	int rc;
@@ -1130,7 +1141,7 @@
 			std::vector<uint32_t> plan(n_q, 1u);
 			for (uint32_t i = 0; i < n_q; ++i) plan[i] = make_seed_plan(q_codes + q_off[i], (uint32_t)(q_off[i + 1] - q_off[i]), q_emac[i], (uint32_t)h->K, h->opt_prefilter_stride, h->alt);
 			if ((rc = upload_plan(h, n_q, plan))) return rc;
-			const uint32_t qw_g = (h->cur->st_maxlen + 7) / 8;
+			const uint32_t qw_g = bhip_qstride(h->cur->st_maxlen);
 			if ((rc = h->cur->qpack.reserve((size_t)n_q * qw_g * 4 + 16))) return rc;
 			const uint64_t total = (uint64_t)n_q * qw_g;
 			if (total) hipLaunchKernelGGL(k_pack_queries, dim3((uint32_t)std::min<uint64_t>((total + 255) / 256, (uint64_t)h->n_cu * 16)), dim3(256), 0, h->stream,
diff --git a/burst_amd/csrc/bhip_handle.h b/burst_amd/csrc/bhip_handle.h
--- a/burst_amd/csrc/bhip_handle.h
+++ b/burst_amd/csrc/bhip_handle.h
@@ -70,8 +70,8 @@
 	uint32_t *, uint8_t *, uint32_t *, BhipStageInfo *, BhipAlt);
 __global__ void k_rescore_classify(const BhipRawHit *, const uint32_t *, uint32_t, const uint32_t *, int, const uint64_t *, const uint32_t *, const uint8_t *,
 	const uint32_t *, BhipHit *, uint32_t *, uint32_t, uint32_t *, uint32_t *, uint32_t *, uint32_t *, uint32_t, int);
-template <int SET> __global__ void k_rescore_reg(const BhipRawHit *, const uint32_t *, const uint32_t *, uint32_t, const uint64_t *, const uint8_t *, const uint32_t *, uint32_t,
-	const uint8_t *, const uint64_t *, const uint32_t *, const uint8_t *, BhipHit *, uint32_t *, uint32_t, uint32_t *);
+template <int SET, bool STAGED> __global__ void k_rescore_reg(const BhipRawHit *, const uint32_t *, const uint32_t *, uint32_t, const uint64_t *, const uint8_t *, const uint32_t *, uint32_t,
+	const uint8_t *, const uint64_t *, const uint32_t *, const uint8_t *, BhipHit *, uint32_t *, uint32_t, uint32_t *, uint32_t);
 int bhip_fail_msg(int code, const char *fmt, ...) __attribute__((format(printf, 2, 3)));
 #define fail(...) bhip_fail_msg(__VA_ARGS__)
 inline bool bhip_trace_sync() { static const bool on = getenv("BHIP_TRACE_SYNC") != nullptr; return on; }
@@ -357,6 +357,7 @@
 	int opt_prune = 1;
 	int opt_lane_min = 32768;
 	int opt_rescore_reg = 1;
+	int opt_rescore_stage = 1;
 	int opt_pf_waves = 0;
 	int opt_pf_algo = -1;
 	int opt_pf_table = 0;
diff --git a/burst_amd/csrc/bhip_init.hip b/burst_amd/csrc/bhip_init.hip
--- a/burst_amd/csrc/bhip_init.hip
+++ b/burst_amd/csrc/bhip_init.hip
@@ -220,6 +220,7 @@
 	if (!strcmp(name, "band")) { h->opt_no_band = value == 0; return BHIP_OK; }
 	if (!strcmp(name, "prune")) { h->opt_prune = value != 0; return BHIP_OK; }
 	if (!strcmp(name, "rescore_reg")) { h->opt_rescore_reg = value != 0; return BHIP_OK; }
+	if (!strcmp(name, "rescore_stage")) { h->opt_rescore_stage = value != 0; return BHIP_OK; }
 	if (!strcmp(name, "seed_min_need")) { if (value < -1 || value > 255) return fail(BHIP_E_ARG, "seed_min_need must be -1 (by rule) or 0 .. 255"); h->opt_seed_min_need = (int)value; return BHIP_OK; }
 	if (!strcmp(name, "seed_drop_len")) { if (value < 0 || value > (1 << 24)) return fail(BHIP_E_ARG, "seed_drop_len must be 0 .. 2^24"); h->opt_seed_drop_len = (int)value; return BHIP_OK; }
 	if (!strcmp(name, "prefilter_waves")) { if (value < 0 || value > 16) return fail(BHIP_E_ARG, "prefilter_waves must be 0 .. 16"); h->opt_pf_waves = (int)value; return BHIP_OK; }
@@ -236,6 +237,8 @@
 	return fail(BHIP_E_ARG, "unknown option '%s'", name);
 }
 
+extern "C" uint32_t bhip_qpack_stride(uint32_t max_len) { return bhip_qstride(max_len); }
+
 extern "C" int bhip_get_stats(void *handle, BhipStats *out) {
 	Handle *h = (Handle *)handle;
 	if (!h || !out) return fail(BHIP_E_ARG, "null argument");
diff --git a/burst_amd/csrc/bhip_internal.h b/burst_amd/csrc/bhip_internal.h
--- a/burst_amd/csrc/bhip_internal.h
+++ b/burst_amd/csrc/bhip_internal.h
@@ -84,6 +84,10 @@
 
 #define BHIP_RESCORE_WMAX 48
 
+static inline uint32_t bhip_qstride(uint32_t max_len) { return (((max_len + 7u) / 8u) + 3u) & ~3u; }
+#define BHIP_RESCORE_STAGE_MAXLEN 128
+static inline uint32_t bhip_rs_stage_dwords(uint32_t max_len) { const uint32_t qn = (max_len + 7u) / 8u; return qn > 1 ? 2u * qn - 3u : 0u; }
+
 #define BHIP_ACX_LINE_WORDS 14u
 #define BHIP_REC_BYTES 4
 #define BHIP_REC_PAD 0xFFFFFFFFu
diff --git a/burst_amd/csrc/bhip_kernels.hip b/burst_amd/csrc/bhip_kernels.hip
--- a/burst_amd/csrc/bhip_kernels.hip
+++ b/burst_amd/csrc/bhip_kernels.hip
@@ -1168,9 +1168,9 @@
 	}
 }
 
-template <int WB>
+template <int WB, bool STAGED>
 __device__ __forceinline__ void rescore_reg_one(
-		const BhipRawHit *__restrict__ hp, bool live, uint32_t *s_mm, uint32_t fastq, uint32_t lane,
+		const BhipRawHit *__restrict__ hp, bool live, uint32_t *s_mm, uint32_t *s_st, uint32_t stg_q, uint32_t fastq, uint32_t lane,
 		const uint64_t *__restrict__ qoff, const uint8_t *__restrict__ qrc, const uint32_t *__restrict__ qpack, uint32_t qw,
 		const uint32_t *__restrict__ refw, const uint64_t *__restrict__ ref_off, const uint32_t *__restrict__ clump_len,
 		BhipHit *__restrict__ out, uint32_t *__restrict__ n_out, uint32_t out_cap, uint32_t *__restrict__ err_flags) {
@@ -1179,7 +1179,7 @@
 	const uint32_t INVALID = (512u << SS) | (255u << GS), Z0 = 255u << GS;
 	const uint32_t STEP_U = (1u << SS) + 1u + (1u << 8), STEP_L = (1u << SS) - (1u << GS) + (2u << 8);
 	uint32_t bkey = 0xFFFFFFFFu, bv = 0, fin = 0xFFFFFFFFu, m = 0, B = 0, hq = 0, hrefIx = 0;
-	if (live) {
+	if (live && (!STAGED || ((hp->m + 7u) >> 3) <= stg_q)) {
 		const uint32_t q = hp->q;
 		hq = q; hrefIx = hp->refIx;
 		B = hp->ed;
@@ -1190,27 +1190,67 @@
 		const int dlo = e1 - (int)m - (int)B, Wd = e2 - e1 + 2 * (int)B + 1;
 		const uint64_t rbase = hp->rbase;
 		const uint32_t LIM = (B + 1) << SS;
+		int p = dlo, j8 = dlo >> 3;
+		uint32_t d[NW];
+		int jn = j8 + NW;
+		uint4 ahead = make_uint4(0, 0, 0, 0);
+		const uint32_t *qp = qpack + (uint64_t)q * qw;
+		uint32_t qd, q_next, prev_sym;
+		const uint32_t qn = (m + 7) >> 3;
+		const int jlo = (p - 1) >> 3, jhi = ((dlo + (int)m - 1) >> 3) + NW - 1;
+		uint32_t *s_q = s_st + lane, *s_r = s_st + (stg_q > 2 ? stg_q - 2 : 0) * 64 + lane;
+		const int jb = jn + 1;
+		int r_left = 0;
+		if constexpr (STAGED) {
+			constexpr int QCH = BHIP_RESCORE_STAGE_MAXLEN / 32, RCH = (BHIP_RESCORE_STAGE_MAXLEN / 8 + NW + 6) / 4;
+			uint4 qv[QCH], rv[RCH];
+			#pragma unroll
+			for (int c = 0; c < QCH; ++c) qv[c] = (uint32_t)(4 * c) < qw ? ((const uint4 *)qp)[c] : make_uint4(0, 0, 0, 0);
+			const int t0 = jlo >> 2, t1 = jhi >> 2;
+			#pragma unroll
+			for (int c = 0; c < RCH; ++c) {
+				const int t = t0 + c < t1 ? t0 + c : t1;
+				const uint32_t tc = t < 0 || !nchunks ? 0u : (uint32_t)t < nchunks ? (uint32_t)t : nchunks - 1;
+				rv[c] = ((const uint4 *)refw)[rbase + tc];
+			}
+			#pragma unroll
+			for (int c = 0; c < RCH; ++c) { const int t = t0 + c; if (t < 0 || (uint32_t)t >= nchunks) rv[c] = make_uint4(0, 0, 0, 0); }
+			#pragma unroll
+			for (int i = 2; i < 4 * QCH; ++i) if ((uint32_t)i < qn && (uint32_t)i < stg_q) s_q[(i - 2) * 64] = pick4(qv[i >> 2], i & 3);
+			qd = qv[0].x; q_next = qv[0].y;
+			const int o = j8 - 4 * t0;
+			auto rdw = [&](int r) -> uint32_t { return pick4(rv[r >> 2], r & 3); };
+			auto at_o = [&](int i) -> uint32_t { return o == 0 ? rdw(i) : o == 1 ? rdw(i + 1) : o == 2 ? rdw(i + 2) : o == 3 ? rdw(i + 3) : rdw(i + 4); };
+			#pragma unroll
+			for (int i = 0; i < NW; ++i) d[i] = at_o(i);
+			ahead.x = jn <= jhi ? at_o(NW) : 0u;
+			prev_sym = (pick4(rv[0], (uint32_t)jlo & 3u) >> (4 * ((p - 1) & 7))) & 15u;
+			#pragma unroll
+			for (int r = NW + 1; r < 4 * RCH; ++r) { const int slot = r - o - NW - 1; if (slot >= 0 && slot <= jhi - jb && (uint32_t)slot + 1 < stg_q) s_r[slot * 64] = rdw(r); }
+			r_left = jhi - jb + 1;
+		} else {
+			#pragma unroll
+			for (int i = 0; i < NW; ++i) d[i] = ref_dword_at(refw, rbase, j8 + i, nchunks);
+			ahead = ref_chunk_at(refw, rbase, jn >> 2, nchunks);
+			qd = qp[0]; q_next = qw > 1 ? qp[1] : 0u;
+			prev_sym = (ref_dword_at(refw, rbase, (p - 1) >> 3, nchunks) >> (4 * ((p - 1) & 7))) & 15u;
+		}
 		uint32_t bd[WB + 1];
 		#pragma unroll
 		for (int k = 0; k < WB; ++k) { const int x = dlo + k; bd[k] = (k < Wd && x >= 0 && x <= (int)L) ? Z0 : INVALID; }
 		bd[WB] = INVALID;
-		int p = dlo, j8 = dlo >> 3;
-		uint32_t d[NW];
-		#pragma unroll
-		for (int i = 0; i < NW; ++i) d[i] = ref_dword_at(refw, rbase, j8 + i, nchunks);
 		auto all_acgt = [&]() { uint32_t bad = 0;
 			#pragma unroll
 			for (int i = 0; i < NW; ++i) bad |= (d[i] - 0x11111111u) & 0xCCCCCCCCu;
 			return bad == 0; };
 		bool dclean = all_acgt();
-		int jn = j8 + NW;
-		uint4 ahead = ref_chunk_at(refw, rbase, jn >> 2, nchunks);
-		const uint32_t *qp = qpack + (uint64_t)q * qw;
-		uint32_t qd = qp[0], q_next = qw > 1 ? qp[1] : 0u;
-		uint32_t prev_sym = (ref_dword_at(refw, rbase, (p - 1) >> 3, nchunks) >> (4 * ((p - 1) & 7))) & 15u;
 		for (int y = 1; y <= (int)m; ++y) {
 			const uint32_t qi = (uint32_t)(y - 1);
-			if ((qi & 7u) == 0 && qi) { qd = q_next; q_next = (qi >> 3) + 1 < qw ? qp[(qi >> 3) + 1] : 0u; }
+			if ((qi & 7u) == 0 && qi) {
+				qd = q_next;
+				if constexpr (STAGED) q_next = (qi >> 3) + 1 < qn ? s_q[((qi >> 3) - 1) * 64] : 0u;
+				else q_next = (qi >> 3) + 1 < qw ? qp[(qi >> 3) + 1] : 0u;
+			}
 			const uint32_t qc = (qd >> (4 * (qi & 7u))) & 15u;
 			const uint32_t col0 = (uint32_t)y <= B ? (((uint32_t)y << SS) | Z0 | (uint32_t)y) : INVALID;
 			const int x0 = y + dlo;
@@ -1281,10 +1321,11 @@
 			if ((p & 7) == 0) {
 				#pragma unroll
 				for (int i = 0; i < NW - 1; ++i) d[i] = d[i + 1];
-				d[NW - 1] = pick4(ahead, (uint32_t)jn & 3u);
+				d[NW - 1] = STAGED ? ahead.x : pick4(ahead, (uint32_t)jn & 3u);
 				dclean = all_acgt();
 				++j8; ++jn;
-				if ((jn & 3) == 0) ahead = ref_chunk_at(refw, rbase, jn >> 2, nchunks);
+				if constexpr (STAGED) { ahead.x = r_left > 0 ? *s_r : 0u; s_r += 64; --r_left; }
+				else if ((jn & 3) == 0) ahead = ref_chunk_at(refw, rbase, jn >> 2, nchunks);
 			}
 		}
 		#pragma unroll
@@ -1320,19 +1361,21 @@
 	}
 }
 
-template <int SET>
-__global__ __launch_bounds__(64) void k_rescore_reg(
+template <int SET, bool STAGED>
+__global__ __launch_bounds__(64) __attribute__((amdgpu_waves_per_eu(STAGED && SET == 0 ? 6 : 1))) void k_rescore_reg(
 		const BhipRawHit *__restrict__ raw, const uint32_t *__restrict__ lists, const uint32_t *__restrict__ counts, uint32_t raw_cap,
 		const uint64_t *__restrict__ qoff, const uint8_t *__restrict__ qrc, const uint32_t *__restrict__ qpack, uint32_t qw,
 		const uint8_t *__restrict__ refb, const uint64_t *__restrict__ ref_off, const uint32_t *__restrict__ clump_len,
 		const uint8_t *__restrict__ lut,
-		BhipHit *__restrict__ out, uint32_t *__restrict__ n_out, uint32_t out_cap, uint32_t *__restrict__ err_flags) {
+		BhipHit *__restrict__ out, uint32_t *__restrict__ n_out, uint32_t out_cap, uint32_t *__restrict__ err_flags, uint32_t stg_q) {
 	__shared__ uint32_t s_mm[16];
+	extern __shared__ __attribute__((aligned(16))) uint32_t smem[];
 	const uint32_t tid = threadIdx.x;
 	if (tid < 16) { uint32_t mm = 0; for (int r = 0; r < 16; ++r) mm |= (lut[16 * tid + r] == 0 ? 1u : 0u) << r | (lut[16 * tid + r] != 255 ? 1u : 0u) << (16 + r); s_mm[tid] = mm; }
 	__syncthreads();
 	uint32_t fastq = 0;
 	for (uint32_t qc = 1; qc <= 4; ++qc) if ((s_mm[qc] & 0x1Eu) == (1u << qc)) fastq |= 1u << qc;
+	if (STAGED) fastq = __builtin_amdgcn_readfirstlane(fastq);
 	const uint32_t *refw = (const uint32_t *)refb;
 #define BHIP_RS_RUN(b, WB) { \
 		uint32_t n = counts[b]; if (n > raw_cap) n = raw_cap; \
@@ -1340,7 +1383,7 @@
 		const uint32_t n_round = (n + 63u) & ~63u; \
 		for (uint32_t i = blockIdx.x * 64 + tid; i < n_round; i += gridDim.x * 64) { \
 			const bool live = i < n; \
-			rescore_reg_one<WB>(raw + (live ? lst[i] : 0u), live, s_mm, fastq, tid, qoff, qrc, qpack, qw, refw, ref_off, clump_len, out, n_out, out_cap, err_flags); \
+			rescore_reg_one<WB, STAGED>(raw + (live ? lst[i] : 0u), live, s_mm, STAGED ? smem : nullptr, stg_q, fastq, tid, qoff, qrc, qpack, qw, refw, ref_off, clump_len, out, n_out, out_cap, err_flags); \
 		} }
 	if (SET == 0) { BHIP_RS_RUN(0, 4) BHIP_RS_RUN(1, 6) BHIP_RS_RUN(2, 8) }
 	else if (SET == 3) { BHIP_RS_RUN(3, 12) }
@@ -1348,14 +1391,11 @@
 	else { BHIP_RS_RUN(6, 32) BHIP_RS_RUN(7, 40) BHIP_RS_RUN(8, 48) }
 #undef BHIP_RS_RUN
 }
-template __global__ void k_rescore_reg<0>(const BhipRawHit *, const uint32_t *, const uint32_t *, uint32_t, const uint64_t *, const uint8_t *, const uint32_t *, uint32_t,
-	const uint8_t *, const uint64_t *, const uint32_t *, const uint8_t *, BhipHit *, uint32_t *, uint32_t, uint32_t *);
-template __global__ void k_rescore_reg<1>(const BhipRawHit *, const uint32_t *, const uint32_t *, uint32_t, const uint64_t *, const uint8_t *, const uint32_t *, uint32_t,
-	const uint8_t *, const uint64_t *, const uint32_t *, const uint8_t *, BhipHit *, uint32_t *, uint32_t, uint32_t *);
-template __global__ void k_rescore_reg<2>(const BhipRawHit *, const uint32_t *, const uint32_t *, uint32_t, const uint64_t *, const uint8_t *, const uint32_t *, uint32_t,
-	const uint8_t *, const uint64_t *, const uint32_t *, const uint8_t *, BhipHit *, uint32_t *, uint32_t, uint32_t *);
-template __global__ void k_rescore_reg<3>(const BhipRawHit *, const uint32_t *, const uint32_t *, uint32_t, const uint64_t *, const uint8_t *, const uint32_t *, uint32_t,
-	const uint8_t *, const uint64_t *, const uint32_t *, const uint8_t *, BhipHit *, uint32_t *, uint32_t, uint32_t *);
+#define BHIP_RS_INST(SET, STAGED) template __global__ void k_rescore_reg<SET, STAGED>(const BhipRawHit *, const uint32_t *, const uint32_t *, uint32_t, const uint64_t *, const uint8_t *, \
+	const uint32_t *, uint32_t, const uint8_t *, const uint64_t *, const uint32_t *, const uint8_t *, BhipHit *, uint32_t *, uint32_t, uint32_t *, uint32_t);
+BHIP_RS_INST(0, false) BHIP_RS_INST(1, false) BHIP_RS_INST(2, false) BHIP_RS_INST(3, false)
+BHIP_RS_INST(0, true) BHIP_RS_INST(1, true) BHIP_RS_INST(2, true) BHIP_RS_INST(3, true)
+#undef BHIP_RS_INST
 
 template __global__ void k_rescore<false>(const BhipRawHit *, const uint32_t *, uint32_t, const uint32_t *, const uint32_t *, const uint32_t *, int,
 	const uint8_t *, const uint64_t *, const uint32_t *, const uint8_t *, const uint8_t *, const uint64_t *, const uint32_t *, const uint8_t *,
diff --git a/burst_amd/csrc/bhip_stage.hip b/burst_amd/csrc/bhip_stage.hip
--- a/burst_amd/csrc/bhip_stage.hip
+++ b/burst_amd/csrc/bhip_stage.hip
@@ -85,7 +85,7 @@
 	}
 	if (max_len > BHIP_MAX_QLEN) return fail(BHIP_E_QUERYLEN, "queries of up to %u symbols (max %d)", max_len, BHIP_MAX_QLEN);
 	S->st_maxlen = max_len;
-	const uint32_t qw = (max_len + 7) / 8;
+	const uint32_t qw = bhip_qstride(max_len);
 	if (all_packed2) all_packed = false;
 	if ((all_packed || all_packed2) && (rc = S->qcodes4.reserve(nb / 2 + 2 * (size_t)n_spans + 64))) return rc;
 	if (all_len && (rc = S->qlen16.reserve(((size_t)n_q + n_spans + 1) * 2 + 64))) return rc;
@@ -315,7 +315,7 @@
 		HIPCHK(hipMemcpyAsync(S->qemac_s.p, emac_s.data(), (size_t)n_q * 2, hipMemcpyHostToDevice, st));
 		HIPCHK(hipMemcpyAsync(S->nx.p, nxv.data(), n_q, hipMemcpyHostToDevice, st));
 		HIPCHK(hipMemcpyAsync(S->nx_six.p, nxs.data(), nsh, hipMemcpyHostToDevice, st));
-		const uint32_t qw_g = (S->st_maxlen + 7) / 8;
+		const uint32_t qw_g = bhip_qstride(S->st_maxlen);
 		if ((rc = S->qpack_s.reserve((size_t)n_q * qw_g * 4 + 64))) return rc;
 		const uint64_t total = (uint64_t)n_q * qw_g;
 		if (total) hipLaunchKernelGGL(k_pack_queries, dim3((uint32_t)std::min<uint64_t>((total + 255) / 256, (uint64_t)h->n_cu * 16)), dim3(256), 0, st,
diff --git a/include/burst_hip.h b/include/burst_hip.h
--- a/include/burst_hip.h
+++ b/include/burst_hip.h
@@ -151,6 +151,8 @@
 
 BHIP_API int bhip_set_option(void *handle, const char *name, long long value);
 
+BHIP_API uint32_t bhip_qpack_stride(uint32_t max_len);
+
 BHIP_API int bhip_get_stats(void *handle, BhipStats *out);
 BHIP_API int bhip_device_info(void *handle, char *name, int name_cap, int *n_cu, uint64_t *hbm_bytes);
 
```

New measurement: 573.8 million. 4.6% lower.
